# malak29/video-text-detection-system

Hardware: AMD Instinct MI355X
Metric: frames/sec (detect+recognize) @720p, 1/2/4/8 MI355X; box IoU vs CPU ref (higher is better)
Workload: dtype f16

## Files before the change

include/vtd.h:

```cpp
#ifndef VTD_H
#define VTD_H

#include <stddef.h>
#include <stdint.h>

#ifdef __cplusplus
extern "C" {
#endif

typedef struct vtd_detector vtd_detector;
typedef struct vtd_recognizer vtd_recognizer;
typedef struct vtd_postproc vtd_postproc;
typedef void* vtd_stream;

typedef struct vtd_detection {
    int32_t bbox[4];
    int32_t polygon[8];
    float confidence;
    float area;
    int32_t first_x, first_y;
} vtd_detection;

const char* vtd_version(void);
const char* vtd_strerror(int code);
int vtd_device_count(void);

int vtd_detector_create(const char* backbone, int max_batch, vtd_detector** out);
void vtd_detector_destroy(vtd_detector* d);
int vtd_detector_set_tensor(vtd_detector* d, const char* key, const float* host_data, int64_t numel);
int vtd_detector_set_option(vtd_detector* d, const char* name, int value);
int vtd_detector_finalize(vtd_detector* d, vtd_stream stream);
int vtd_detector_preprocess(vtd_detector* d, const uint8_t* frames_dev, int n, int height, int width, vtd_stream stream);
int vtd_detector_set_input_nchw(vtd_detector* d, const float* x_dev, int n, vtd_stream stream);
int vtd_detector_forward(vtd_detector* d, int n, float* prob_dev, float* thresh_dev, vtd_stream stream);
int vtd_detector_read_tap(vtd_detector* d, const char* name, int n, float* host_out, int64_t capacity, vtd_stream stream);
int64_t vtd_detector_macs_per_frame(const vtd_detector* d);
int vtd_detector_set_profiling(vtd_detector* d, int enable);
int vtd_detector_num_ops(const vtd_detector* d);
int vtd_detector_get_profile(vtd_detector* d, int op_index, char* name, int name_cap, double* total_ms, int64_t* calls,
                             double* total_macs, vtd_stream stream);

int vtd_detector_set_tuning(vtd_detector* d, const char* table_text);
int64_t vtd_detector_get_tuning(const vtd_detector* d, char* buf, int64_t capacity);
int vtd_detector_tuning_measured(const vtd_detector* d);

int vtd_postproc_create(int max_batch, int map_h, int map_w, int max_out, vtd_postproc** out);
void vtd_postproc_destroy(vtd_postproc* pp);
int vtd_postproc_run(vtd_postproc* pp, const float* prob_dev, int n, const int32_t* orig_w_host, const int32_t* orig_h_host,
                     float threshold, vtd_detection* out_dev, int32_t* counts_dev, vtd_stream stream);
int vtd_copy_to_pinned_host(const void* src_dev, void* dst_pinned_host, int64_t bytes, vtd_stream stream);

int64_t vtd_dbloss_workspace_bytes(void);
int vtd_dbloss_forward(const float* prob_dev, const float* thresh_dev, const float* prob_target_dev, const float* thresh_target_dev, int64_t numel,
                       float smooth, void* workspace_dev, float* out4_dev, double* sums5_dev, vtd_stream stream);
int vtd_dbloss_backward(const float* prob_dev, const float* thresh_dev, const float* prob_target_dev, const float* thresh_target_dev, int64_t numel,
                        float smooth, const double* sums5_dev, const float* grad_out4_dev, float* grad_prob_dev, float* grad_thresh_dev,
                        vtd_stream stream);
int vtd_binary_counts_accumulate(const float* pred_dev, const float* target_dev, int64_t numel, float threshold, int64_t* counts4_dev,
                                 vtd_stream stream);

typedef struct vtd_dbhead_branch {
    float *conv_w, *conv_b, *bn1_w, *bn1_b, *bn1_mean, *bn1_var, *ct1_w, *ct1_b, *bn2_w, *bn2_b, *bn2_mean, *bn2_var, *ct2_w, *ct2_b;
} vtd_dbhead_branch;
typedef struct vtd_dbhead_params {
    vtd_dbhead_branch branch[2];
} vtd_dbhead_params;
int vtd_detector_forward_features(vtd_detector* d, int n, void* feats_dev, vtd_stream stream);
int vtd_dbhead_pack_features(const void* x_dev, int dtype, int n, int height, int width, void* feats_dev, vtd_stream stream);
int64_t vtd_dbhead_train_workspace_bytes(int n, int height, int width, int backward);
int vtd_dbhead_train_forward(const void* feats_dev, int n, int height, int width, const vtd_dbhead_params* params, int training, float momentum,
                             float eps, void* workspace_dev, float* prob_dev, float* thresh_dev, float* stats_dev, vtd_stream stream);
int vtd_dbhead_train_backward(const void* feats_dev, int n, int height, int width, const vtd_dbhead_params* params, int training,
                              const void* workspace_dev, const float* prob_dev, const float* thresh_dev, const float* grad_prob_dev,
                              const float* grad_thresh_dev, const vtd_dbhead_params* grads, void* scratch_dev, vtd_stream stream);
int vtd_dbhead_train_backward_input(int n, int height, int width, const vtd_dbhead_params* params, void* scratch_dev, float* dfeats_dev,
                                    float* dscale_dev, vtd_stream stream);
int vtd_dbhead_unpack_input_grad(const float* dfeats_dev, const float* dscale_dev, int n, int height, int width, float* grad_nchw_dev,
                                 vtd_stream stream);

typedef struct vtd_fpn_params {
    float *inner_w[4], *inner_b[4];
    float *layer_w, *layer_b;
} vtd_fpn_params;
int vtd_detector_forward_trunk(vtd_detector* d, int n, void* c2_dev, void* c3_dev, void* c4_dev, void* c5_dev, vtd_stream stream);
int vtd_detector_forward_pool(vtd_detector* d, int n, void* pool_dev, vtd_stream stream);
int vtd_fpn_train_pack_tap(const void* x_dev, int dtype, int n, int channels, int height, int width, void* tap_dev, vtd_stream stream);
int64_t vtd_fpn_train_workspace_bytes(int n, int h5, int w5, int c5_channels, int mode);
int vtd_fpn_train_forward(const void* const* taps, int n, int h5, int w5, int c5_channels, const vtd_fpn_params* params, void* workspace_dev,
                          void* p2_dev, vtd_stream stream);
int vtd_fpn_train_unpack_p2(const void* p2_dev, int n, int height, int width, float* p2_nchw_dev, vtd_stream stream);
int vtd_fpn_train_pack_grad(const float* grad_nchw_dev, int n, int height, int width, float* dp2_dev, vtd_stream stream);
int vtd_fpn_train_backward(const void* const* taps, int n, int h5, int w5, int c5_channels, const vtd_fpn_params* params, const void* workspace_dev,
                           const float* dp2_dev, const float* dscale_dev, const vtd_fpn_params* grads, void* scratch_dev, vtd_stream stream);
int64_t vtd_fpn_train_input_workspace_bytes(int n, int h5, int w5, int c5_channels);
int vtd_fpn_train_backward_input(int n, int h5, int w5, int c5_channels, const vtd_fpn_params* params, void* scratch_dev, int level_mask,
                                 float* const* dtaps_dev, float* dscale_dev, vtd_stream stream);
int vtd_fpn_train_unpack_tap_grad(const float* dtap_dev, const float* dscale_dev, int n, int channels, int height, int width, float* grad_nchw_dev,
                                  vtd_stream stream);

typedef struct vtd_basicblock_params {
    float *conv1_w, *bn1_w, *bn1_b, *bn1_mean, *bn1_var;
    float *conv2_w, *bn2_w, *bn2_b, *bn2_mean, *bn2_var;
    float *ds_w, *ds_bn_w, *ds_bn_b, *ds_bn_mean, *ds_bn_var;
} vtd_basicblock_params;
int64_t vtd_basicblock_train_workspace_bytes(int n, int h_in, int w_in, int cin, int width, int stride, int mode);
int vtd_basicblock_train_forward(const void* x_dev, int n, int h_in, int w_in, int cin, int width, int stride, const vtd_basicblock_params* params,
                                 float eps, void* workspace_dev, void* y_dev, vtd_stream stream);
int vtd_basicblock_train_backward(const void* x_dev, int n, int h_in, int w_in, int cin, int width, int stride, const vtd_basicblock_params* params,
                                  float eps, const void* workspace_dev, const void* y_dev, const float* dy_dev, const float* dscale_dev,
                                  const vtd_basicblock_params* grads, void* scratch_dev, float* dx_dev, float* dxscale_dev, vtd_stream stream);

int64_t vtd_resblock_train_workspace_bytes(int n, int h_in, int w_in, int cin, int width, int stride, int mode);
int vtd_resblock_train_forward(const void* x_dev, int n, int h_in, int w_in, int cin, int width, int stride, const vtd_basicblock_params* params,
                               float eps, void* workspace_dev, void* y_dev, vtd_stream stream);
int vtd_resblock_train_backward(const void* x_dev, int n, int h_in, int w_in, int cin, int width, int stride, const vtd_basicblock_params* params,
                                float eps, const void* workspace_dev, const void* y_dev, const float* dy_dev, const float* dscale_dev,
                                const vtd_basicblock_params* grads, void* scratch_dev, float* dx_dev, float* dxscale_dev, vtd_stream stream);
int vtd_resblock_train_combine(float* a_dev, const float* ascale_dev, const float* b_dev, const float* bscale_dev, int64_t numel, float* outscale_dev,
                               vtd_stream stream);

int64_t vtd_block64_train_workspace_bytes(int n, int h_in, int w_in, int cin, int width, int stride, int mode);
int vtd_block64_train_forward(const void* x_dev, int n, int h_in, int w_in, int cin, int width, int stride, const vtd_basicblock_params* params,
                              float eps, void* workspace_dev, void* y_dev, vtd_stream stream);
int vtd_block64_train_backward(const void* x_dev, int n, int h_in, int w_in, int cin, int width, int stride, const vtd_basicblock_params* params,
                               float eps, const void* workspace_dev, const void* y_dev, const float* dy_dev, const float* dscale_dev,
                               const vtd_basicblock_params* grads, void* scratch_dev, float* dx_dev, float* dxscale_dev, vtd_stream stream);

typedef struct vtd_stem_params {
    float *w, *gamma, *beta, *mean, *var;
} vtd_stem_params;
int vtd_stem_train_pack_input(const void* x_dev, int dtype, int n, int height, int width, void* tap_dev, vtd_stream stream);
int64_t vtd_stem_train_workspace_bytes(int n, int height, int width, int mode);
int vtd_stem_train_forward(const void* x_tap_dev, int n, int height, int width, const vtd_stem_params* params, float eps, void* workspace_dev,
                           void* pool_tap_dev, void* idx_dev, vtd_stream stream);
int vtd_stem_train_backward(const void* x_tap_dev, int n, int height, int width, const vtd_stem_params* params, float eps, const void* workspace_dev,
                            const void* pool_tap_dev, const void* idx_dev, const float* dpool_dev, const float* dscale_dev, const vtd_stem_params* grads,
                            void* scratch_dev, vtd_stream stream);

int vtd_recognizer_create(int vocab_size, int max_crops, vtd_recognizer** out);
void vtd_recognizer_destroy(vtd_recognizer* r);
int vtd_recognizer_set_tensor(vtd_recognizer* r, const char* key, const float* host_data, int64_t numel);
int vtd_recognizer_set_option(vtd_recognizer* r, const char* name, int value);
int vtd_recognizer_finalize(vtd_recognizer* r, vtd_stream stream);
int vtd_recognizer_crop_resize(vtd_recognizer* r, const uint8_t* frames_dev, int n_frames, int height, int width,
                               const int32_t* boxes_dev, int ncrops, vtd_stream stream);
int vtd_recognizer_set_input_nchw(vtd_recognizer* r, const float* x_dev, int ncrops, vtd_stream stream);
int vtd_recognizer_forward(vtd_recognizer* r, int ncrops, float* logits_dev, vtd_stream stream);
int vtd_recognizer_read_tap(vtd_recognizer* r, const char* name, int ncrops, float* host_out, int64_t capacity, vtd_stream stream);
int64_t vtd_recognizer_macs_per_crop(const vtd_recognizer* r);
int vtd_recognizer_set_tuning(vtd_recognizer* r, const char* table_text);
int64_t vtd_recognizer_get_tuning(const vtd_recognizer* r, char* buf, int64_t capacity);
int vtd_recognizer_tuning_measured(const vtd_recognizer* r);
int vtd_ctc_greedy_decode(const float* logits_dev, int n, int T, int V, const int32_t* id2char_dev, int blank_id, int apply_softmax,
                          int32_t* out_dev, vtd_stream stream);

typedef struct vtd_trocr vtd_trocr;
typedef struct vtd_trocr_config {
    int32_t image_size, patch_size;
    int32_t enc_hidden, enc_layers, enc_heads, enc_ffn;
    int32_t enc_qkv_bias;
    float enc_ln_eps;
    int32_t dec_hidden, dec_layers, dec_heads, dec_ffn;
    int32_t vocab_size, max_positions;
    float dec_ln_eps;
    int32_t decoder_start_token_id, eos_token_id, pad_token_id;
    int32_t max_length;
} vtd_trocr_config;
int vtd_trocr_create(const vtd_trocr_config* cfg, int max_crops, vtd_trocr** out);
void vtd_trocr_destroy(vtd_trocr* t);
int vtd_trocr_set_option(vtd_trocr* t, const char* name, int value);
int vtd_trocr_get_option(const vtd_trocr* t, const char* name, int* value);
int vtd_trocr_set_tensor(vtd_trocr* t, const char* key, const float* host_data, int64_t numel);
int vtd_trocr_finalize(vtd_trocr* t, vtd_stream stream);
int vtd_trocr_encode_crops(vtd_trocr* t, const uint8_t* frames_dev, int n_frames, int height, int width, const int32_t* boxes_host, int ncrops,
                           vtd_stream stream);
int vtd_trocr_encode_pixels(vtd_trocr* t, const float* pixel_values_dev, int ncrops, vtd_stream stream);
int vtd_trocr_generate(vtd_trocr* t, int ncrops, int max_length, const int32_t* forced_ids_dev, int forced_len, int32_t* ids_dev, float* logits_dev,
                       vtd_stream stream);
int vtd_trocr_num_slots(const vtd_trocr* t);
int vtd_trocr_encode_crops_slot(vtd_trocr* t, int slot, const uint8_t* frames_dev, int n_frames, int height, int width, const int32_t* boxes_host,
                                int ncrops, vtd_stream stream);
int vtd_trocr_encode_pixels_slot(vtd_trocr* t, int slot, const float* pixel_values_dev, int ncrops, vtd_stream stream);
int vtd_trocr_stage_crops_slot(vtd_trocr* t, int slot, const uint8_t* frames_dev, int n_frames, int height, int width, const int32_t* boxes_host,
                               int ncrops, int row_offset, vtd_stream stream);
int vtd_trocr_encode_staged_slot(vtd_trocr* t, int slot, int ncrops, vtd_stream stream);
int vtd_trocr_generate_slot(vtd_trocr* t, int slot, int ncrops, int max_length, const int32_t* forced_ids_dev, int forced_len, int32_t* ids_dev,
                            float* logits_dev, vtd_stream stream);
// ... 17 lines not shown
```

video-text-detection-system_amd/csrc/detector_misc.hip:

```cpp
#include "vtd_common.h"

namespace {

constexpr int PRE_TY = 16;
constexpr int PRE_OUT = 640;
constexpr int PRE_CHUNK = 4;
#ifndef VTD_PRE_NT
#define VTD_PRE_NT 640
#endif
constexpr int PRE_NT = VTD_PRE_NT;
constexpr int PRE_COLS = (PRE_OUT + PRE_NT - 1) / PRE_NT;

struct PreParams {
    const uint8_t* frames;
    half_t* out;
    const int* xb;
    const int* xk;
    const int* yb;
    const int* yk;
    int H, W, ksx, ksy;
    int max_rows;
    unsigned quads_magic;
};

__device__ __forceinline__ uint8_t clip8_22(int v) {
    v >>= 22;
    return (uint8_t)(v < 0 ? 0 : (v > 255 ? 255 : v));
}

__global__ __launch_bounds__(256) void preprocess_kernel(const PreParams p) {
    extern __shared__ __attribute__((aligned(16))) uint8_t rows[];
    const int oy0 = blockIdx.x * PRE_TY;
    const int img = blockIdx.y;
    const int y_first = p.yb[2 * oy0];
    const int oy_last = min(oy0 + PRE_TY, PRE_OUT) - 1;
    const int y_end = p.yb[2 * oy_last] + p.yb[2 * oy_last + 1];
    const int nrows = y_end - y_first;
    const int row_bytes = p.W * 3;
    const int row_pad = (row_bytes + 15) & ~15;
    uint8_t* raw = rows + ((p.max_rows * PRE_OUT * 3 + 15) & ~15);
    const uint8_t* src = p.frames + (int64_t)img * p.H * row_bytes;

    for (int r0 = 0; r0 < nrows; r0 += PRE_CHUNK) {
        const int nr = min(PRE_CHUNK, nrows - r0);
        if ((row_bytes & 15) == 0) {
            const int vec_per_row = row_bytes >> 4;
            for (int i = threadIdx.x; i < nr * vec_per_row; i += 256) {
                const int rr = i / vec_per_row, v = i - rr * vec_per_row;
                *(uint4*)(raw + rr * row_pad + v * 16) = *(const uint4*)(src + (int64_t)(y_first + r0 + rr) * row_bytes + v * 16);
            }
        } else {
            for (int i = threadIdx.x; i < nr * row_bytes; i += 256) {
                const int rr = i / row_bytes, v = i - rr * row_bytes;
                raw[rr * row_pad + v] = src[(int64_t)(y_first + r0 + rr) * row_bytes + v];
            }
        }
        __syncthreads();
        for (int idx = threadIdx.x; idx < nr * PRE_OUT; idx += 256) {
            const int rr = idx / PRE_OUT, ox = idx - rr * PRE_OUT;
            const uint8_t* row = raw + rr * row_pad;
            const int xmin = p.xb[2 * ox], cnt = p.xb[2 * ox + 1];
            const int* k = p.xk + ox * p.ksx;
            int s0 = 1 << 21, s1 = 1 << 21, s2 = 1 << 21;
            for (int t = 0; t < cnt; ++t) {
                const int kv = k[t];
                const uint8_t* px = row + (xmin + t) * 3;
                s0 += px[0] * kv;
                s1 += px[1] * kv;
                s2 += px[2] * kv;
            }
            uint8_t* d = rows + ((r0 + rr) * PRE_OUT + ox) * 3;
            d[0] = clip8_22(s0);
            d[1] = clip8_22(s1);
            d[2] = clip8_22(s2);
        }
        __syncthreads();
    }

    const float mean[3] = {0.485f, 0.456f, 0.406f};
    const float stdv[3] = {0.229f, 0.224f, 0.225f};
    for (int idx = threadIdx.x; idx < PRE_TY * PRE_OUT; idx += 256) {
        const int ty = idx / PRE_OUT, ox = idx - ty * PRE_OUT;
        const int oy = oy0 + ty;
        if (oy >= PRE_OUT) break;
        const int ymin = p.yb[2 * oy] - y_first, cnt = p.yb[2 * oy + 1];
        const int* k = p.yk + oy * p.ksy;
        int s0 = 1 << 21, s1 = 1 << 21, s2 = 1 << 21;
        for (int t = 0; t < cnt; ++t) {
            const int kv = k[t];
            const uint8_t* px = rows + ((ymin + t) * PRE_OUT + ox) * 3;
            s0 += px[0] * kv;
            s1 += px[1] * kv;
            s2 += px[2] * kv;
        }
        const float b = (float)clip8_22(s0), g = (float)clip8_22(s1), r = (float)clip8_22(s2);
        half4 o;
        o[0] = (half_t)((r / 255.0f - mean[0]) / stdv[0]);
        o[1] = (half_t)((g / 255.0f - mean[1]) / stdv[1]);
        o[2] = (half_t)((b / 255.0f - mean[2]) / stdv[2]);
        o[3] = (half_t)0.f;
        *(half4*)(p.out + (((int64_t)img * 646 + oy + 3) * 646 + ox + 3) * 4) = o;
    }
}

template <int KSX, int KSY>
__global__ __launch_bounds__(PRE_NT) void preprocess_fast_kernel(const PreParams p) {
    extern __shared__ __attribute__((aligned(16))) uint8_t lds[];
    uint32_t* const rows = (uint32_t*)lds;
    const int raw_pitch = p.W + KSX;
    uint32_t* const raw = rows + p.max_rows * PRE_OUT;
    int* const ytab = (int*)(raw + PRE_CHUNK * raw_pitch);
    half_t* const lut = (half_t*)(ytab + PRE_TY * (2 + KSY));
    const int oy0 = blockIdx.x * PRE_TY;
    const int img = blockIdx.y;
    const int y_first = p.yb[2 * oy0];
    const int oy_last = min(oy0 + PRE_TY, PRE_OUT) - 1;
    const int y_end = p.yb[2 * oy_last] + p.yb[2 * oy_last + 1];
    const int nrows = y_end - y_first;
    const int row_bytes = p.W * 3;
    const uint8_t* src = p.frames + (int64_t)img * p.H * row_bytes;
    const int tid = threadIdx.x;

    int xmin[PRE_COLS], kx[PRE_COLS][KSX];
#pragma unroll
    for (int s = 0; s < PRE_COLS; ++s) {
        const int ox = min(tid + PRE_NT * s, PRE_OUT - 1);
        xmin[s] = p.xb[2 * ox];
#pragma unroll
        for (int t = 0; t < KSX; ++t) kx[s][t] = p.xk[ox * KSX + t];
    }
    for (int i = tid; i < PRE_TY * (2 + KSY); i += PRE_NT) {
        const int ty = i / (2 + KSY), e = i - ty * (2 + KSY);
        const int oy = min(oy0 + ty, PRE_OUT - 1);
        ytab[i] = e < 2 ? p.yb[2 * oy + e] : p.yk[oy * KSY + (e - 2)];
    }
    for (int i = tid; i < PRE_CHUNK * KSX; i += PRE_NT) raw[(i / KSX) * raw_pitch + p.W + (i % KSX)] = 0u;
    {
        const float mean[3] = {0.485f, 0.456f, 0.406f};
        const float stdv[3] = {0.229f, 0.224f, 0.225f};
        if (tid < 256) {
#pragma unroll
            for (int c = 0; c < 3; ++c) lut[c * 256 + tid] = (half_t)(((float)tid / 255.0f - mean[c]) / stdv[c]);
        }
    }

    const int quads = p.W >> 2;
    constexpr int MAXIT = (PRE_CHUNK * 512 + PRE_NT - 1) / PRE_NT;
    uint32_t stg0[MAXIT][3], stg1[MAXIT][3];
    auto fetch = [&](int r0, uint32_t (&stg)[MAXIT][3]) {
        const int nr = min(PRE_CHUNK, nrows - r0);
#pragma unroll
        for (int it = 0; it < MAXIT; ++it) {
            const int i = tid + it * PRE_NT;
            if (i < nr * quads) {
                const int rr = (int)__umulhi((unsigned)i, p.quads_magic), q = i - rr * quads;
                const uint32_t* g = (const uint32_t*)(src + (int64_t)(y_first + r0 + rr) * row_bytes) + q * 3;
                stg[it][0] = g[0]; stg[it][1] = g[1]; stg[it][2] = g[2];
            }
        }
    };
    auto chunk = [&](int r0, uint32_t (&stg)[MAXIT][3]) {
        const int nr = min(PRE_CHUNK, nrows - r0);
#pragma unroll
        for (int it = 0; it < MAXIT; ++it) {
            const int i = tid + it * PRE_NT;
            if (i < nr * quads) {
                const int rr = (int)__umulhi((unsigned)i, p.quads_magic), q = i - rr * quads;
                const uint32_t d0 = stg[it][0], d1 = stg[it][1], d2 = stg[it][2];
                uint4 px;
                px.x = d0 & 0xffffffu;
                px.y = ((d0 >> 24) | (d1 << 8)) & 0xffffffu;
                px.z = ((d1 >> 16) | (d2 << 16)) & 0xffffffu;
                px.w = d2 >> 8;
                *(uint4*)(raw + rr * raw_pitch + q * 4) = px;
            }
        }
        __syncthreads();
        if (r0 + 2 * PRE_CHUNK < nrows) fetch(r0 + 2 * PRE_CHUNK, stg);
        for (int rr = 0; rr < nr; ++rr) {
            const uint32_t* row = raw + rr * raw_pitch;
#pragma unroll
            for (int s = 0; s < PRE_COLS; ++s) {
                const int ox = tid + PRE_NT * s;
                if (ox < PRE_OUT) {
                    uint32_t s0 = 1u << 21, s1 = 1u << 21, s2 = 1u << 21;
#pragma unroll
                    for (int t = 0; t < KSX; ++t) {
                        const uint32_t px = row[xmin[s] + t];
                        const uint32_t kt = (uint32_t)kx[s][t];
                        s0 = __umul24(px & 0xffu, kt) + s0;
                        s1 = __umul24((px >> 8) & 0xffu, kt) + s1;
                        s2 = __umul24(px >> 16, kt) + s2;
                    }
                    rows[(r0 + rr) * PRE_OUT + ox] = (uint32_t)clip8_22((int)s0) | ((uint32_t)clip8_22((int)s1) << 8) | ((uint32_t)clip8_22((int)s2) << 16);
                }
            }
        }
        __syncthreads();
    };
    fetch(0, stg0);
    if (PRE_CHUNK < nrows) fetch(PRE_CHUNK, stg1);
    for (int r0 = 0; r0 < nrows; r0 += 2 * PRE_CHUNK) {
        chunk(r0, stg0);
        if (r0 + PRE_CHUNK < nrows) chunk(r0 + PRE_CHUNK, stg1);
    }

    for (int idx = tid; idx < PRE_TY * (PRE_OUT / 4); idx += PRE_NT) {
        const int ty = idx / (PRE_OUT / 4), g = idx - ty * (PRE_OUT / 4);
        const int oy = oy0 + ty;
        if (oy >= PRE_OUT) break;
        const int* yt = ytab + ty * (2 + KSY);
        const int ymin = yt[0] - y_first;
        uint32_t acc[4][3];
#pragma unroll
        for (int q = 0; q < 4; ++q)
#pragma unroll
            for (int c = 0; c < 3; ++c) acc[q][c] = 1u << 21;
#pragma unroll
        for (int t = 0; t < KSY; ++t) {
            const uint32_t kv = (uint32_t)yt[2 + t];
            const int r = min(ymin + t, nrows - 1);
            const uint4 px = *(const uint4*)(rows + r * PRE_OUT + g * 4);
            const uint32_t pv[4] = {px.x, px.y, px.z, px.w};
#pragma unroll
            for (int q = 0; q < 4; ++q) {
                acc[q][0] = __umul24(pv[q] & 0xffu, kv) + acc[q][0];
                acc[q][1] = __umul24((pv[q] >> 8) & 0xffu, kv) + acc[q][1];
                acc[q][2] = __umul24(pv[q] >> 16, kv) + acc[q][2];
            }
        }
        half8 o01, o23;
#pragma unroll
        for (int q = 0; q < 4; ++q) {
            const half_t h0 = lut[clip8_22((int)acc[q][2])];
            const half_t h1 = lut[256 + clip8_22((int)acc[q][1])];
            const half_t h2 = lut[512 + clip8_22((int)acc[q][0])];
            if (q < 2) { o01[q * 4] = h0; o01[q * 4 + 1] = h1; o01[q * 4 + 2] = h2; o01[q * 4 + 3] = (half_t)0.f; }
            else { o23[(q - 2) * 4] = h0; o23[(q - 2) * 4 + 1] = h1; o23[(q - 2) * 4 + 2] = h2; o23[(q - 2) * 4 + 3] = (half_t)0.f; }
        }
        half_t* dst = p.out + (((int64_t)img * 646 + oy + 3) * 646 + g * 4 + 3) * 4;
        *(half4*)(dst) = half4{o01[0], o01[1], o01[2], o01[3]};
        *(half4*)(dst + 4) = half4{o01[4], o01[5], o01[6], o01[7]};
        *(half4*)(dst + 8) = half4{o23[0], o23[1], o23[2], o23[3]};
        *(half4*)(dst + 12) = half4{o23[4], o23[5], o23[6], o23[7]};
    }
}

__global__ void nchw_to_input_kernel(const float* __restrict__ x, half_t* __restrict__ out, int n) {
    const int64_t idx = (int64_t)blockIdx.x * blockDim.x + threadIdx.x;
    const int64_t total = (int64_t)n * 640 * 640;
    if (idx >= total) return;
    const int img = (int)(idx / (640 * 640));
    const int rem = (int)(idx - (int64_t)img * 640 * 640);
    const int y = rem / 640, xx = rem - y * 640;
    const float* base = x + (int64_t)img * 3 * 640 * 640 + rem;
    half4 o = {(half_t)base[0], (half_t)base[640 * 640], (half_t)base[2 * 640 * 640], (half_t)0.f};
    *(half4*)(out + (((int64_t)img * 646 + y + 3) * 646 + xx + 3) * 4) = o;
}

struct PoolParams {
    const half_t* in;
    half_t* out;
    int n, c, ho, wo;
    int in_hp, in_wp, in_y0, in_x0;
    int out_hp, out_wp, out_ring;
    int kh, kw, sh, sw;
};

__global__ void maxpool_kernel(const PoolParams p) {
    const int cg = p.c >> 3;
    const int64_t total = (int64_t)p.n * p.ho * p.wo * cg;
    for (int64_t idx = (int64_t)blockIdx.x * blockDim.x + threadIdx.x; idx < total; idx += (int64_t)gridDim.x * blockDim.x) {
        const int g = (int)(idx % cg);
        int64_t t = idx / cg;
        const int ox = (int)(t % p.wo);
        t /= p.wo;
        const int oy = (int)(t % p.ho);
        const int img = (int)(t / p.ho);
        half8 m;
#pragma unroll
        for (int e = 0; e < 8; ++e) m[e] = (half_t)(-65504.f);
        for (int r = 0; r < p.kh; ++r)
            for (int s = 0; s < p.kw; ++s) {
                const half8 v = *(const half8*)(p.in + (((int64_t)img * p.in_hp + oy * p.sh + p.in_y0 + r) * p.in_wp +
                                                         ox * p.sw + p.in_x0 + s) * p.c + g * 8);
#pragma unroll
                for (int e = 0; e < 8; ++e) m[e] = v[e] > m[e] ? v[e] : m[e];
            }
        *(half8*)(p.out + (((int64_t)img * p.out_hp + oy + p.out_ring) * p.out_wp + ox + p.out_ring) * p.c + g * 8) = m;
    }
}

}

int vtd_launch_preprocess(const uint8_t* frames, int n, int H, int W, half_t* out, const int* xb, const int* xk, int ksx,
                          const int* yb, const int* yk, int ksy, int max_rows, hipStream_t stream) {
    PreParams p{frames, out, xb, xk, yb, yk, H, W, ksx, ksy, max_rows, 0u};
    if ((W & 3) == 0 && W <= 2048 && ksy == 5 && (ksx == 5 || ksx == 7)) {
        const int lds_fast = (max_rows * PRE_OUT + PRE_CHUNK * (W + ksx) + PRE_TY * (2 + ksy)) * 4 + 3 * 256 * 2;
        p.quads_magic = (unsigned)(((1ull << 32) + (W / 4) - 1) / (W / 4));
        if (lds_fast <= 160 * 1024) {
            static bool attr5 = false, attr7 = false;
            if (ksx == 5) {
                if (!attr5) {
                    VTD_HIP_CHECK(hipFuncSetAttribute((const void*)preprocess_fast_kernel<5, 5>, hipFuncAttributeMaxDynamicSharedMemorySize, 160 * 1024));
                    attr5 = true;
                }
                hipLaunchKernelGGL((preprocess_fast_kernel<5, 5>), dim3(PRE_OUT / PRE_TY, n), dim3(PRE_NT), lds_fast, stream, p);
            } else {
                if (!attr7) {
                    VTD_HIP_CHECK(hipFuncSetAttribute((const void*)preprocess_fast_kernel<7, 5>, hipFuncAttributeMaxDynamicSharedMemorySize, 160 * 1024));
                    attr7 = true;
                }
                hipLaunchKernelGGL((preprocess_fast_kernel<7, 5>), dim3(PRE_OUT / PRE_TY, n), dim3(PRE_NT), lds_fast, stream, p);
            }
            return -(int)hipGetLastError();
        }
    }
    const int lds = ((max_rows * PRE_OUT * 3 + 15) & ~15) + PRE_CHUNK * ((W * 3 + 15) & ~15);
    if (lds > 160 * 1024) return -1010;
    static bool attr_done = false;
    if (!attr_done) {
        VTD_HIP_CHECK(hipFuncSetAttribute((const void*)preprocess_kernel, hipFuncAttributeMaxDynamicSharedMemorySize, 160 * 1024));
        attr_done = true;
    }
    hipLaunchKernelGGL(preprocess_kernel, dim3(PRE_OUT / PRE_TY, n), dim3(256), lds, stream, p);
    return -(int)hipGetLastError();
}

int vtd_launch_nchw_to_input(const float* x, half_t* out, int n, hipStream_t stream) {
    const int64_t total = (int64_t)n * 640 * 640;
    hipLaunchKernelGGL(nchw_to_input_kernel, dim3((unsigned)((total + 255) / 256)), dim3(256), 0, stream, x, out, n);
    return -(int)hipGetLastError();
}

int vtd_launch_maxpool(const TensorDesc& in, const TensorDesc& out, int n, int kh, int kw, int sh, int sw, int pad_h, int pad_w,
                       hipStream_t stream) {
    if (in.c != out.c || (in.c & 7)) return -1020;
    if (in.ring < pad_h || in.ring < pad_w) return -1021;
    if ((out.h - 1) * sh - pad_h + kh > in.h + (in.hp - in.h - in.ring) || (out.w - 1) * sw - pad_w + kw > in.w + (in.wp - in.w - in.ring))
        return -1022;
    PoolParams p{in.ptr, out.ptr, n, in.c, out.h, out.w, in.hp, in.wp, in.ring - pad_h, in.ring - pad_w,
                 out.hp, out.wp, out.ring, kh, kw, sh, sw};
    const int64_t total = (int64_t)n * out.h * out.w * (in.c >> 3);
    const int blocks = (int)((total + 255) / 256 < 256 * 16 ? (total + 255) / 256 : 256 * 16);
    hipLaunchKernelGGL(maxpool_kernel, dim3(blocks), dim3(256), 0, stream, p);
    return -(int)hipGetLastError();
}
```

video-text-detection-system_amd/csrc/stem_pool.hip:

```cpp
#include <cstdlib>
#include "vtd_common.h"

namespace {

constexpr int SP_PT_ROWS = 7, SP_PT_COLS = 8;
constexpr int SP_CT_COLS = 17;
constexpr int SP_PATCH_COLS = 40;
constexpr int SP_PIECES = 12;
constexpr int SP_PATCH_BYTES = SP_PIECES * 1024;
constexpr int SP_NST = 3;
constexpr int SP_CT_PITCH = 144;
constexpr int SP_LDS = SP_NST * SP_PATCH_BYTES + 256 * SP_CT_PITCH + 256;

struct StemPoolParams {
    const half_t* in;
    const half_t* w;
    const float* bias;
    half_t* out;
    int n, in_hp, in_wp, conv_h, conv_w, pool_h, pool_w, out_hp, out_wp, out_ring;
    int tiles_x, tiles_y, total_tiles;
};

typedef short short4v __attribute__((ext_vector_type(4)));
typedef short short8v __attribute__((ext_vector_type(8)));
__device__ __forceinline__ half8 sp_max(half8 a, half8 b) {
    return __builtin_bit_cast(half8, __builtin_elementwise_max(__builtin_bit_cast(short8v, a), __builtin_bit_cast(short8v, b)));
}

__host__ __device__ constexpr int sp_chan(int tile, int row) { return 32 * (tile >> 1) + 8 * (row >> 2) + 4 * (tile & 1) + (row & 3); }

template <int N>
__device__ __forceinline__ void sp_wait_vmcnt() { asm volatile("s_waitcnt vmcnt(%0)" ::"n"(N) : "memory"); }
__device__ __forceinline__ void sp_lds_barrier() {
    asm volatile("s_waitcnt lgkmcnt(0)" ::: "memory");
    __builtin_amdgcn_s_barrier();
}

__device__ __forceinline__ void sp_tile_coords(const StemPoolParams& p, int tile, int& img, int& py0, int& px0) {
    const int per_img = p.tiles_x * p.tiles_y;
    img = tile / per_img;
    const int r = tile - img * per_img;
    const int ty = r / p.tiles_x;
    py0 = ty * SP_PT_ROWS;
    px0 = (r - ty * p.tiles_x) * SP_PT_COLS;
}

template <int DBG>
__global__ __launch_bounds__(256, 2) void stem_pool_kernel(const StemPoolParams p) {
    extern __shared__ __attribute__((aligned(16))) unsigned char sp_smem[];
    unsigned char* const ring = sp_smem;
    unsigned char* const ctile = sp_smem + SP_NST * SP_PATCH_BYTES;
    float* const bias_lds = (float*)(ctile + 256 * SP_CT_PITCH);
    const int tid = threadIdx.x, lane = tid & 63;
    const int wv = __builtin_amdgcn_readfirstlane(tid >> 6);
    const int fr = lane & 15, fq = lane >> 4;

    int first, stride, last;
    if ((gridDim.x & 7) == 0) {
        const int xcd = blockIdx.x & 7, per = gridDim.x >> 3;
        const int lo = (int)(((int64_t)p.total_tiles * xcd) >> 3);
        last = (int)(((int64_t)p.total_tiles * (xcd + 1)) >> 3);
        first = lo + (blockIdx.x >> 3);
        stride = per;
    } else {
        first = blockIdx.x; stride = gridDim.x; last = p.total_tiles;
    }
    if (first >= last) return;
    const int nt = (last - first + stride - 1) / stride;

    half8 wreg[7][4];
#pragma unroll
    for (int ky = 0; ky < 7; ++ky)
#pragma unroll
        for (int i = 0; i < 4; ++i) wreg[ky][i] = *(const half8*)(p.w + ((ky * 4 + i) * 64 + lane) * 8);
    if (tid < 64) bias_lds[tid] = p.bias[tid];
    int a_off[4];
#pragma unroll
    for (int j = 0; j < 4; ++j) {
        const int pix = wv * 64 + j * 16 + fr;
        const int c_row = pix / SP_CT_COLS, c_col = pix - c_row * SP_CT_COLS;
        a_off[j] = ((2 * c_row) * SP_PATCH_COLS + 2 * c_col + 2 * fq) * 8;
    }
    int u_row[3], u_col[3];
#pragma unroll
    for (int k = 0; k < 3; ++k) {
        int u = (wv + 4 * k) * 64 + lane;
        u = u < 700 ? u : 699;
        u_row[k] = u / 20;
        u_col[k] = 2 * (u - u_row[k] * 20);
    }
    auto issue = [&](int tile, int stage) {
        if constexpr (DBG == 4) return;
        int img, py0, px0;
        sp_tile_coords(p, __builtin_amdgcn_readfirstlane(tile), img, py0, px0);
        const half_t* base = p.in + (int64_t)img * p.in_hp * p.in_wp * 4;
#pragma unroll
        for (int k = 0; k < 3; ++k) {
            int iy = 4 * py0 - 2 + u_row[k], ix = 4 * px0 - 2 + u_col[k];
            iy = iy < 0 ? 0 : iy > p.in_hp - 1 ? p.in_hp - 1 : iy;
            ix = ix < 0 ? 0 : ix > p.in_wp - 2 ? p.in_wp - 2 : ix;
            __builtin_amdgcn_global_load_lds((const VTD_AS1 void*)(base + (iy * p.in_wp + ix) * 4),
                                             (VTD_AS3 void*)(ring + stage * SP_PATCH_BYTES + (wv + 4 * k) * 1024), 16, 0, 0);
        }
    };

    if constexpr (DBG == 7 || DBG == 8) {
        if (((blockIdx.x >> 3) & 32) != 0) { __builtin_amdgcn_s_sleep(60); }
    }
    issue(first, 0);
    if (nt > 1) { issue(first + stride, 1); sp_wait_vmcnt<3>(); } else sp_wait_vmcnt<0>();
    sp_lds_barrier();

    int st = 0;
    for (int k = 0; k < nt; ++k) {
        const int tile = first + k * stride;
        int img, py0, px0;
        sp_tile_coords(p, __builtin_amdgcn_readfirstlane(tile), img, py0, px0);
        if (k + 2 < nt) issue(tile + 2 * stride, st == 0 ? SP_NST - 1 : st - 1);

        floatx4 acc[4][4];
#pragma unroll
        for (int i = 0; i < 4; ++i)
#pragma unroll
            for (int j = 0; j < 4; ++j) acc[i][j] = *(const floatx4*)(bias_lds + sp_chan(i, fq * 4));
        const unsigned char* pb = ring + st * SP_PATCH_BYTES;
        half8 af[2][4];
#pragma unroll
        for (int j = 0; j < 4; ++j) af[0][j] = *(const half8*)(pb + a_off[j]);
        if constexpr (DBG == 6 || DBG == 7) __builtin_amdgcn_s_setprio(3);
#pragma unroll
        for (int ky = 0; ky < 7; ++ky) {
            if (ky < 6) {
#pragma unroll
                for (int j = 0; j < 4; ++j) af[(ky + 1) & 1][j] = *(const half8*)(pb + a_off[j] + (ky + 1) * (SP_PATCH_COLS * 8));
            }
            if (DBG == 3 && ky > 0) { for (int j = 0; j < 4; ++j) asm volatile("" ::"v"(af[ky & 1][j])); continue; }
#pragma unroll
            for (int j = 0; j < 4; ++j)
#pragma unroll
                for (int i = 0; i < 4; ++i) acc[i][j] = __builtin_amdgcn_mfma_f32_16x16x32_f16(wreg[ky][i], af[ky & 1][j], acc[i][j], 0, 0, 0);
            if (ky < 6) __builtin_amdgcn_sched_group_barrier(0x100, 4, 0);
            __builtin_amdgcn_sched_group_barrier(0x008, 16, 0);
            __builtin_amdgcn_sched_barrier(0);
        }

        if constexpr (DBG == 6 || DBG == 7) __builtin_amdgcn_s_setprio(0);
        if constexpr (DBG == 2) {
            float t = 0.f;
            for (int i = 0; i < 4; ++i) for (int j = 0; j < 4; ++j) t += acc[i][j][0] + acc[i][j][1] + acc[i][j][2] + acc[i][j][3];
            if (t == 123.456f) p.out[0] = (half_t)t;
            if (k + 2 < nt) sp_wait_vmcnt<3>(); else sp_wait_vmcnt<0>();
            sp_lds_barrier();
            st = st + 1 == SP_NST ? 0 : st + 1;
            continue;
        }
#pragma unroll
        for (int j = 0; j < 4; ++j) {
            const int pix = wv * 64 + j * 16 + fr;
            const int c_row = pix / SP_CT_COLS, c_col = pix - c_row * SP_CT_COLS;
            const int cy = 2 * py0 - 1 + c_row, cx = 2 * px0 - 1 + c_col;
            const bool valid = cy >= 0 && cy < p.conv_h && cx >= 0 && cx < p.conv_w;
            unsigned char* dst = ctile + pix * SP_CT_PITCH + fq * 16;
#pragma unroll
            for (int k = 0; k < 2; ++k) {
                typedef float float2v __attribute__((ext_vector_type(2)));
                typedef _Float16 half2v __attribute__((ext_vector_type(2)));
                const floatx4 a = acc[2 * k][j], b = acc[2 * k + 1][j];
                const half2v h0 = __builtin_convertvector((float2v{a[0], a[1]}), half2v);
                const half2v h1 = __builtin_convertvector((float2v{a[2], a[3]}), half2v);
                const half2v h2 = __builtin_convertvector((float2v{b[0], b[1]}), half2v);
                const half2v h3 = __builtin_convertvector((float2v{b[2], b[3]}), half2v);
                half8 hv = half8{h0[0], h0[1], h1[0], h1[1], h2[0], h2[1], h3[0], h3[1]};
                hv = __builtin_bit_cast(half8, __builtin_elementwise_max(__builtin_bit_cast(short8v, hv), short8v{0, 0, 0, 0, 0, 0, 0, 0}));
                if (!valid) hv = half8{0, 0, 0, 0, 0, 0, 0, 0};
                *(half8*)(dst + k * 64) = hv;
            }
        }
        sp_lds_barrier();

        if constexpr (DBG != 1) {
            const int cg = (lane >> 2) & 7;
            const int qx = ((lane >> 5) & 1) | ((lane & 3) << 1);
            const bool two = wv < 3;
            const unsigned char* src0 = ctile + ((2 * wv) * SP_CT_COLS + 2 * qx) * SP_CT_PITCH + cg * 16;
            const int px = px0 + qx;
#pragma unroll
            for (int it = 0; it < 2; ++it) {
                if (it == 1 && !two) break;
                const unsigned char* src = src0 + it * (8 * SP_CT_COLS * SP_CT_PITCH);
                half8 v[9];
#pragma unroll
                for (int r = 0; r < 3; ++r)
#pragma unroll
                    for (int c = 0; c < 3; ++c) v[r * 3 + c] = *(const half8*)(src + (r * SP_CT_COLS + c) * SP_CT_PITCH);
                __builtin_amdgcn_sched_group_barrier(0x100, 9, 0);
                half8 m = sp_max(v[0], v[1]);
#pragma unroll
                for (int q = 2; q < 9; ++q) m = sp_max(m, v[q]);
                const int py = py0 + wv + 4 * it;
                if (DBG == 5) asm volatile("" ::"v"(m));
                else if (py < p.pool_h && px < p.pool_w)
                    *(half8*)(p.out + (((int64_t)img * p.out_hp + py + p.out_ring) * p.out_wp + px + p.out_ring) * 64 + cg * 8) = m;
            }
        }
        if (k + 2 < nt) sp_wait_vmcnt<3>(); else sp_wait_vmcnt<0>();
        sp_lds_barrier();
        st = st + 1 == SP_NST ? 0 : st + 1;
    }
}

}

void vtd_stem_pool_pack_weights(const float* w_folded , half_t* packed ) {
    for (int ky = 0; ky < 7; ++ky)
        for (int i = 0; i < 4; ++i)
            for (int lane = 0; lane < 64; ++lane) {
                const int fr = lane & 15, fq = lane >> 4, co = sp_chan(i, fr);
                for (int e = 0; e < 8; ++e) {
                    const int kx = 2 * fq + (e >> 2), c = e & 3;
                    float v = 0.f;
                    if (kx < 7 && c < 3) v = w_folded[((co * 3 + c) * 7 + ky) * 7 + kx];
                    packed[((ky * 4 + i) * 64 + lane) * 8 + e] = (half_t)v;
                }
            }
}

int vtd_launch_stem_pool(const TensorDesc& in, const TensorDesc& out, const half_t* w_packed, const float* bias, int n,
                         hipStream_t stream) {
    if (in.c != 4 || in.ring != 3 || out.c != 64 || (in.h & 3) || (in.w & 3) || out.h != in.h / 4 || out.w != in.w / 4 ||
        in.hp != in.h + 6 || in.wp != in.w + 6 || (in.wp & 1) || n <= 0 || n > in.n || n > out.n)
        return -2001;
    if (out.w % SP_PT_COLS) return -2002;
    StemPoolParams p;
    p.in = in.ptr; p.w = w_packed; p.bias = bias; p.out = out.ptr;
    p.n = n; p.in_hp = in.hp; p.in_wp = in.wp; p.conv_h = in.h / 2; p.conv_w = in.w / 2; p.pool_h = out.h; p.pool_w = out.w;
    p.out_hp = out.hp; p.out_wp = out.wp; p.out_ring = out.ring;
    p.tiles_x = out.w / SP_PT_COLS;
    p.tiles_y = (out.h + SP_PT_ROWS - 1) / SP_PT_ROWS;
    p.total_tiles = n * p.tiles_x * p.tiles_y;
    const int grid = p.total_tiles < 512 ? p.total_tiles : 512;
    void (*kern)(const StemPoolParams) = stem_pool_kernel<0>;
#ifdef VTD_STEM_EXPERIMENT
    if (const char* e = getenv("VTD_STEM_DEBUG")) {
        switch (atoi(e)) {
            case 1: kern = stem_pool_kernel<1>; break;
            case 2: kern = stem_pool_kernel<2>; break;
            case 3: kern = stem_pool_kernel<3>; break;
            case 4: kern = stem_pool_kernel<4>; break;
            case 5: kern = stem_pool_kernel<5>; break;
            case 6: kern = stem_pool_kernel<6>; break;
            case 7: kern = stem_pool_kernel<7>; break;
            case 8: kern = stem_pool_kernel<8>; break;
            default: break;
        }
    }
    {
        hipError_t ea = hipFuncSetAttribute((const void*)kern, hipFuncAttributeMaxDynamicSharedMemorySize, SP_LDS);
        if (ea != hipSuccess) return -(int)ea;
    }
#else
    static bool attr_set = false;
    if (!attr_set) {
        hipError_t ea = hipFuncSetAttribute((const void*)kern, hipFuncAttributeMaxDynamicSharedMemorySize, SP_LDS);
        if (ea != hipSuccess) return -(int)ea;
        attr_set = true;
    }
#endif
    hipLaunchKernelGGL(kern, dim3(grid), dim3(256), SP_LDS, stream, p);
    hipError_t e = hipGetLastError();
    return e == hipSuccess ? 0 : -(int)e;
}
```

video-text-detection-system_amd/csrc/vtd_api.cpp:

```cpp
#include <algorithm>
#include <cmath>
#include <cstdio>
#include <cstdlib>
#include <cstring>
#include <map>
#include <memory>
#include <string>
#include <vector>

#include "../../include/vtd.h"
#include "vtd_common.h"

int vtd_launch_conv(const ConvParams& p, int cfg, hipStream_t stream);
int vtd_conv_num_configs();
bool vtd_conv_config_valid(const ConvParams& p, int cfg);
int vtd_launch_preprocess(const uint8_t* frames, int n, int H, int W, half_t* out, const int* xb, const int* xk, int ksx,
                          const int* yb, const int* yk, int ksy, int max_rows, hipStream_t stream);
int vtd_launch_nchw_to_input(const float* x, half_t* out, int n, hipStream_t stream);
int vtd_launch_maxpool(const TensorDesc& in, const TensorDesc& out, int n, int kh, int kw, int sh, int sw, int pad_h, int pad_w,
                       hipStream_t stream);
void vtd_stem_pool_pack_weights(const float* w_folded, half_t* packed);
int vtd_launch_stem_pool(const TensorDesc& in, const TensorDesc& out, const half_t* w_packed, const float* bias, int n, hipStream_t stream);
extern "C" int vtd_head_entry_halo_steps(int py, int px, int nch1, int* out);
int vtd_launch_head_entry_halo(const ConvParams& c, const int* steps_dev, int nsteps, int big_tiles, hipStream_t stream);
#ifdef VTD_EXPERIMENTAL_CANDIDATES
extern "C" int vtd_head_entry_half_schedule(const int* steps, int nsteps, int* out);
int vtd_launch_head_entry_half(const ConvParams& c, const int* sched_dev, int nsteps, hipStream_t stream);
int vtd_head_entry_pair_tables(int py, int px, int c2ch, int* half_steps, int* plan);
int vtd_launch_head_entry_pair(const ConvParams& c, const int* half_steps_dev, const int* plan_dev, int nh, hipStream_t stream);
#endif
bool vtd_conv_halo_supported(const ConvParams& c, int* bn_out, int* tw_out);
bool vtd_conv_halo_c64_supported(const ConvParams& c, int tw);
int vtd_launch_conv_halo(const ConvParams& c, int bn, int tw, hipStream_t stream);
bool vtd_pointwise128_supported(const ConvParams& c);
int vtd_launch_pointwise128(const ConvParams& c, hipStream_t stream);
void vtd_head_tail_pack_w1(const half_t* w1_gemm, half_t* packed);
void vtd_head_tail_pack_w2(const float* w2, half_t* packed);
int vtd_launch_head_tail(const TensorDesc& in, const half_t* w1, const float* bias1, const half_t* w2, float b2, float* out, int n,
                         hipStream_t stream);

int vtd_launch_crop_resize(const uint8_t* frames, int H, int W, const int32_t* boxes, int ncrops, uint8_t* out, hipStream_t s);
int vtd_launch_crnn_conv1(const uint8_t* in_u8, const float* in_f32, const half_t* w, const float* bias, half_t* out, int n, hipStream_t s);
int vtd_launch_lstm(const half_t* xs, const half_t* whh, half_t* hout, int D, int T, hipStream_t s);
int vtd_launch_ctc_greedy(const float* logits, int n, int T, int V, int ld, const int32_t* id2char, int blank, int apply_softmax,
                          int32_t* out, hipStream_t s);
int vtd_launch_compact_rows(const float* in, float* out, int64_t rows, int V, int ld, hipStream_t s);
int vtd_dbloss_ws_bytes();
int vtd_launch_dbloss(const float* prob, const float* thresh, const float* prob_t, const float* thresh_t, int64_t n, float smooth, double* workspace,
                      float* out4, double* sums5, hipStream_t stream);
int vtd_launch_dbloss_backward(const float* prob, const float* thresh, const float* prob_t, const float* thresh_t, int64_t n, float smooth,
                               const double* sums5, const float* grad_out4, float* grad_prob, float* grad_thresh, hipStream_t stream);
int vtd_launch_binary_counts(const float* pred, const float* target, int64_t n, float threshold, int64_t* counts4, hipStream_t stream);
int64_t vtd_dbhead_ws_bytes(int n, int H, int W, int backward);
int vtd_launch_dbhead_pack(const void* x, int dtype, int n, int H, int W, void* feats, hipStream_t s);
int vtd_launch_dbhead_forward(const void* feats, int n, int H, int W, const vtd_dbhead_params* params, int training, float momentum, float eps,
                              void* ws, float* prob, float* thresh, float* stats_out, hipStream_t s);
int vtd_launch_dbhead_backward_input(int n, int H, int W, const vtd_dbhead_params* params, void* scratch, float* dfeats, float* dscale, hipStream_t s);
int vtd_launch_dbhead_unpack_input_grad(const float* dfeats, const float* dscale, int n, int H, int W, float* out, hipStream_t s);
int64_t vtd_fpn_ws_bytes(int n, int h5, int w5, int c5, int mode);
int vtd_launch_fpn_pack_tap(const void* x, int dtype, int n, int channels, int H, int W, void* out, hipStream_t s);
int vtd_launch_fpn_unpack_p2(const void* p2, int n, int H, int W, float* out, hipStream_t s);
int vtd_launch_fpn_pack_grad(const float* g, int n, int H, int W, float* out, hipStream_t s);
int vtd_launch_fpn_forward(const void* const* taps, int n, int h5, int w5, int c5, const vtd_fpn_params* params, void* ws, void* p2_out, hipStream_t s);
int vtd_launch_fpn_backward(const void* const* taps, int n, int h5, int w5, int c5, const vtd_fpn_params* params, const void* ws, const float* dp2,
                            const float* dscale, const vtd_fpn_params* grads, void* scratch, hipStream_t s);
int64_t vtd_fpn_input_ws_bytes(int n, int h5, int w5, int c5);
int vtd_launch_fpn_backward_input(int n, int h5, int w5, int c5, const vtd_fpn_params* params, void* scratch, int mask, float* const* dtaps,
                                  float* dscale, hipStream_t s);
int64_t vtd_basicblock_ws_bytes(int n, int hin, int win, int cin, int width, int stride, int mode);
int vtd_launch_basicblock_forward(const void* x, int n, int hin, int win, int cin, int width, int stride, const vtd_basicblock_params* P, float eps,
                                  void* ws, void* y, hipStream_t s);
int vtd_launch_basicblock_backward(const void* x, int n, int hin, int win, int cin, int width, int stride, const vtd_basicblock_params* P, float eps,
                                   const void* ws, const void* y, const float* dy, const float* dscale, const vtd_basicblock_params* Gp, void* scratch,
                                   float* dx, float* dxscale, hipStream_t s);
int64_t vtd_resblock_ws_bytes(int n, int hin, int win, int cin, int width, int stride, int mode);
int64_t vtd_block64_ws_bytes(int n, int hin, int win, int cin, int width, int stride, int mode);
int vtd_launch_block64_forward(const void* x, int n, int hin, int win, int cin, int width, int stride, const vtd_basicblock_params* P, float eps, void* ws,
                               void* y, hipStream_t s);
int vtd_launch_block64_backward(const void* x, int n, int hin, int win, int cin, int width, int stride, const vtd_basicblock_params* P, float eps,
                                const void* ws, const void* y, const float* dy, const float* dscale, const vtd_basicblock_params* Gp, void* scratch,
                                float* dx, float* dxscale, hipStream_t s);
int vtd_launch_resblock_combine(float* a, const float* asc, const float* b, const float* bsc, int64_t numel, float* osc, hipStream_t s);
int vtd_launch_stem_pack_input(const void* x, int dtype, int n, int H, int W, void* tap, hipStream_t s);
int64_t vtd_stem_ws_bytes(int n, int H, int W, int mode);
int vtd_launch_stem_forward(const void* x, int n, int H, int W, const vtd_stem_params* P, float eps, void* ws, void* pool, void* idx, hipStream_t s);
int vtd_launch_stem_backward(const void* x, int n, int H, int W, const vtd_stem_params* P, float eps, const void* ws, const void* pool, const void* idx,
                             const float* dpool, const float* dscale, const vtd_stem_params* Gp, void* scratch, hipStream_t s);
int vtd_launch_resblock_forward(const void* x, int n, int hin, int win, int cin, int width, int stride, const vtd_basicblock_params* P, float eps, void* ws,
                                void* y, hipStream_t s);
int vtd_launch_resblock_backward(const void* x, int n, int hin, int win, int cin, int width, int stride, const vtd_basicblock_params* P, float eps,
                                 const void* ws, const void* y, const float* dy, const float* dscale, const vtd_basicblock_params* Gp, void* scratch,
                                 float* dx, float* dxscale, hipStream_t s);
int vtd_launch_fpn_unpack_tap_grad(const float* g, const float* sc, int n, int channels, int H, int W, float* out, hipStream_t s);
int vtd_launch_dbhead_backward(const void* feats, int n, int H, int W, const vtd_dbhead_params* params, int training, const void* ws,
                               const float* prob, const float* thresh, const float* gprob, const float* gthresh, const vtd_dbhead_params* grads,
                               void* scratch, hipStream_t s);

namespace vtd {

enum : int {
    ERR_ARG = -1100,
    ERR_UNKNOWN_KEY = -1101,
    ERR_SHAPE = -1102,
    ERR_MISSING_KEY = -1103,
    ERR_NOT_FINALIZED = -1104,
    ERR_BATCH = -1105,
    ERR_GEOMETRY = -1106,
    ERR_CAPACITY = -1107,
};

using StateDict = std::map<std::string, std::vector<float>>;

struct DeviceArena {
    std::vector<void*> blocks;
    size_t total = 0;
    int alloc(void** out, size_t bytes, bool zero) {
        void* p = nullptr;
        bytes = (bytes + 255) & ~size_t(255);
        hipError_t e = hipMalloc(&p, bytes);
        if (e != hipSuccess) return -(int)e;
        if (zero) {
            e = hipMemset(p, 0, bytes);
            if (e != hipSuccess) return -(int)e;
        }
        blocks.push_back(p);
        total += bytes;
        *out = p;
        return 0;
    }
    ~DeviceArena() {
        for (void* p : blocks) (void)hipFree(p);
    }
};

static TensorDesc make_desc(int n, int h, int w, int c, int ring, int ring_br) {
    TensorDesc t;
    t.ptr = nullptr;
    t.n = n; t.h = h; t.w = w; t.c = c; t.ring = ring;
    t.hp = h + ring + ring_br;
    t.wp = w + ring + ring_br;
    return t;
}

struct ConvOp {
    TensorDesc in, out, res;
    bool has_res = false;
    half_t* w = nullptr;
    half_t* w_panel = nullptr;
    float* bias = nullptr;
    int k_hi_step = 32, cin_steps = 1, kw = 1, s_step = 0, r_step = 0;
    int K = 0, cout = 0, cout_pad = 0, stride = 1, in_y0 = 0, in_x0 = 0, flags = 0, ps_cout = 0, res_shift = 0;
    int ho = 0, wo = 0;
    int64_t macs_per_image = 0;
    void* out_f32 = nullptr;
    int ldc = 0;
    int seg_cols = 0;
    void* seg_out[3] = {nullptr, nullptr, nullptr};
    int seg_ldc[3] = {0, 0, 0};
    const float* head_w = nullptr;
    float head_b = 0.f;
    const uint32_t* plist = nullptr;
    const int* tile_combo = nullptr;
    const uint32_t* plist_b = nullptr;
    const int* tile_combo_border = nullptr;
    int tiles_border = 0;
    const int* he_steps = nullptr;
    int he_nsteps = 0;
    const int* hh_sched = nullptr;
    const int* hp_half_steps = nullptr;
    const int* hp_plan = nullptr;
    int hp_nh = 0;
    const int* tile_combo_b = nullptr;
    int tiles_per_img_b = 0;
    int tiles_per_img = 0, seg1_steps = 0, cin_steps2 = 0, kw2 = 0, s_step2 = 0, r_step2 = 0, img_h = 0, img_w = 0;
    TensorDesc in2;
    const float* bias_tab = nullptr;
    bool dual = false;
    int in2_mul = 1, in2_shr = 0;
    int pool_pw = 0;
};

struct Op {
    enum Kind { CONV, POOL, FINAL, STEMPOOL, HEADTAIL, BORDER } kind;
    ConvOp conv;
    TensorDesc pin, pout;
    int pk[6] = {0, 0, 0, 0, 0, 0};
    const float* fw = nullptr;
    float fbias = 0.f;
    int final_slot = 0;
    const half_t* spw = nullptr;
    const float* spb = nullptr;
    const half_t* htw1 = nullptr;
    const half_t* htw2 = nullptr;
};

static void fill_conv_params(const ConvOp& c, int n, ConvParams& p) {
    std::memset(&p, 0, sizeof(p));
    p.in = c.in.ptr; p.wgt = c.w; p.k_hi_step = c.k_hi_step; p.cin_steps = c.cin_steps; p.kw = c.kw; p.s_step = c.s_step; p.r_step = c.r_step; p.bias = c.bias;
    p.res = c.has_res ? c.res.ptr : nullptr;
    p.out = (c.flags & (EPI_OUT_F32 | EPI_OUT_F16)) ? c.out_f32 : (void*)c.out.ptr;
    p.M = n * c.ho * c.wo; p.K = c.K; p.cout = c.cout; p.cout_pad = c.cout_pad;
    p.ho = c.ho; p.wo = c.wo;
    p.in_hp = c.in.hp; p.in_wp = c.in.wp; p.in_c = c.in.c; p.in_y0 = c.in_y0; p.in_x0 = c.in_x0; p.stride = c.stride;
    p.out_hp = c.out.hp; p.out_wp = c.out.wp; p.out_c = c.out.c; p.out_ring = c.out.ring;
    p.res_hp = c.res.hp; p.res_wp = c.res.wp; p.res_ring = c.res.ring; p.res_shift = c.res_shift;
    p.ps_cout = c.ps_cout; p.flags = c.flags; p.ldc = c.ldc;
    p.seg_cols = c.seg_cols;
    for (int i = 0; i < 3; ++i) { p.seg_out[i] = c.seg_out[i]; p.seg_ldc[i] = c.seg_ldc[i]; }
    p.head_w = c.head_w; p.head_b = c.head_b; p.prob_out = (float*)c.out_f32;
    if (c.plist) {
        p.plist = c.plist; p.tile_combo = c.tile_combo; p.tiles_per_img = c.tiles_per_img;
        p.plist_b = c.plist_b; p.tile_combo_b = c.tile_combo_b; p.tiles_per_img_b = c.tiles_per_img_b;
        p.in2 = c.in2.ptr; p.in2_hp = c.in2.hp; p.in2_wp = c.in2.wp; p.in2_c = c.in2.c; p.in2_ring = c.in2.ring;
        p.seg1_steps = c.seg1_steps; p.cin_steps2 = c.cin_steps2; p.kw2 = c.kw2; p.s_step2 = c.s_step2; p.r_step2 = c.r_step2;
        p.bias_tab = c.bias_tab; p.img_h = c.img_h; p.img_w = c.img_w;
        p.M = n * c.tiles_per_img * 128;
    }
    p.pool_pw = c.pool_pw;
    if (c.dual) {
        p.in2 = c.in2.ptr; p.in2_hp = c.in2.hp; p.in2_wp = c.in2.wp; p.in2_c = c.in2.c; p.in2_ring = c.in2.ring;
        p.in2_mul = c.in2_mul; p.in2_shr = c.in2_shr;
        p.seg1_steps = c.seg1_steps; p.cin_steps2 = c.cin_steps2; p.kw2 = 1; p.s_step2 = 0; p.r_step2 = 0;
    }
}

static const int kHaloCfg = 100;
static const int kHaloC64Cfg = 101;
static const int kHalo64Cfg = 104;
static const int kHeadEntryHalo256Cfg = 103;
static const int kHeadEntryPairCfg = 105;
static const int kPointwiseCfg = 106;
static const int kHeadEntryHalfCfg = 107;
static const int kHeadEntryHaloCfg = 102;
static bool halo_enabled() {
    const char* e = std::getenv("VTD_HALO_CONV");
    return !(e && e[0] == '0');
}

static int pick_tile_height(const ConvParams& p, int table_cfg) {
    if (const char* e = std::getenv("VTD_TILE_HEIGHT_MODEL"); e && e[0] == '0') return table_cfg;
    if (std::getenv("VTD_FORCE_CONV_CFG")) return table_cfg;
    static const struct { int cfg, bm, bn; double eff; } family[5] = {{0, 256, 128, 1.0}, {14, 256, 128, 1.04}, {13, 272, 128, 0.92}, {12, 208, 128, 0.80},
                                                                      {15, 256, 256, 1.07}};
    auto cost_of = [&](int cfg) -> double {
        for (const auto& k : family)
            if (k.cfg == cfg) {
                if (!vtd_conv_config_valid(p, k.cfg)) return 0.0;
                const int64_t tiles = (int64_t)((p.M + k.bm - 1) / k.bm) * (p.cout_pad / k.bn);
                return (double)((tiles + 255) / 256) * k.bm * k.bn / k.eff;
            }
        return 0.0;
    };
    int best = table_cfg;
    double best_cost = cost_of(table_cfg);
    if (best_cost == 0.0) return table_cfg;
    const double keep = best_cost * 0.94;
    double other_cost = keep;
    for (const auto& k : family) {
        if (k.cfg == table_cfg) continue;
        const double c = cost_of(k.cfg);
        if (c > 0.0 && c < other_cost) { other_cost = c; best = k.cfg; }
// ... 32 lines not shown
    return vtd_launch_conv(p, cfg, s);
}

static int launch_border_tiles(const ConvOp& c, int n, hipStream_t s) {
    if (!c.tile_combo_border || c.tiles_border <= 0) return ERR_GEOMETRY;
    ConvParams pb;
    fill_conv_params(c, n, pb);
    pb.tile_combo = c.tile_combo_border; pb.tiles_per_img = c.tiles_border; pb.M = n * c.tiles_border * 128;
    pb.plist_b = nullptr; pb.tile_combo_b = nullptr; pb.tiles_per_img_b = 0;
    return vtd_launch_conv(pb, 9, s);
}

static int autotune_conv(const ConvOp& c, int n, hipStream_t s, int* best_cfg) {
    ConvParams p;
    fill_conv_params(c, n, p);
    hipEvent_t e0, e1;
    VTD_HIP_CHECK(hipEventCreate(&e0));
    VTD_HIP_CHECK(hipEventCreate(&e1));
    float best = 1e30f;
    int best_id = -1, rc = 0;
    if (p.plist) {
        const char* fc = std::getenv("VTD_FORCE_CLASSED_CFG");
        if (fc && (vtd_conv_config_valid(p, std::atoi(fc)) || ((std::atoi(fc) == kHeadEntryHaloCfg || std::atoi(fc) == kHeadEntryHalo256Cfg) && c.he_steps) ||
                   (std::atoi(fc) == kHeadEntryHalfCfg && c.hh_sched) ||
                   (std::atoi(fc) == kHeadEntryPairCfg && c.hp_half_steps))) {
            (void)hipEventDestroy(e0);
            (void)hipEventDestroy(e1);
            *best_cfg = std::atoi(fc);
            return 0;
        }
    }
    for (int cfg = 0; cfg < vtd_conv_num_configs() && !rc; ++cfg) {
        if (!vtd_conv_config_valid(p, cfg)) continue;
        if ((rc = vtd_launch_conv(p, cfg, s))) break;
        (void)hipEventRecord(e0, s);
        for (int rep = 0; rep < 3 && !rc; ++rep) rc = vtd_launch_conv(p, cfg, s);
        (void)hipEventRecord(e1, s);
        if (hipEventSynchronize(e1) != hipSuccess) { rc = ERR_ARG; break; }
        float ms = 0.f;
        (void)hipEventElapsedTime(&ms, e0, e1);
        if (ms < best) { best = ms; best_id = cfg; }
    }
    if (!rc && p.plist && c.he_steps && halo_enabled()) {
        const float best_gathered = best;
        for (int variant = 0; variant < 4 && !rc; ++variant) {
            if (variant == 2 && !c.hp_half_steps) continue;
            if (variant == 3 && !c.hh_sched) continue;
            const int vcfg = variant == 3 ? kHeadEntryHalfCfg : variant == 2 ? kHeadEntryPairCfg : variant ? kHeadEntryHalo256Cfg : kHeadEntryHaloCfg;
            auto both = [&]() { int r = launch_conv_op(c, n, s, vcfg); return r ? r : launch_border_tiles(c, n, s); };
            if ((rc = both())) break;
            float ms = 1e30f;
            for (int round = 0; round < 2 && !rc; ++round) {
                (void)hipEventRecord(e0, s);
                for (int rep = 0; rep < 4 && !rc; ++rep) rc = both();
                (void)hipEventRecord(e1, s);
                if (hipEventSynchronize(e1) != hipSuccess) rc = ERR_ARG;
                float t = 0.f;
                (void)hipEventElapsedTime(&t, e0, e1);
                ms = t * 0.75f < ms ? t * 0.75f : ms;
            }
            if (const char* v = std::getenv("VTD_AUTOTUNE_VERBOSE"); v && v[0] == '1')
                std::fprintf(stderr, "[autotune] head entry variant %d: %.1f us per launch incl. border tiles (best so far %.1f, cfg %d)\n", vcfg,
                             ms / 3.f * 1e3f, best / 3.f * 1e3f, best_id);
            (void)best_gathered;
            if (!rc && ms < best) { best = ms; best_id = vcfg; }
        }
    }
    if (!rc && vtd_pointwise128_supported(p)) {
        if (!(rc = vtd_launch_pointwise128(p, s))) {
            (void)hipEventRecord(e0, s);
            for (int rep = 0; rep < 3 && !rc; ++rep) rc = vtd_launch_pointwise128(p, s);
            (void)hipEventRecord(e1, s);
            if (hipEventSynchronize(e1) != hipSuccess) rc = ERR_ARG;
            float ms = 0.f;
            (void)hipEventElapsedTime(&ms, e0, e1);
            if (!rc && ms < best) { best = ms; best_id = kPointwiseCfg; }
        }
    }
    int hbn = 0, htw = 0;
    if (!rc && halo_enabled() && vtd_conv_halo_supported(p, &hbn, &htw)) {
        const char* force = std::getenv("VTD_FORCE_HALO");
        if (force && (force[0] == '1' || force[0] == '2' || force[0] == '3')) best = 1e30f;
        bool pinned = false;
        for (int variant = 0; variant < 3 && !rc; ++variant) {
            if (variant == 1 && !vtd_conv_halo_c64_supported(p, htw)) continue;
            const int bn = variant == 1 ? 1 : variant == 2 ? 2 : hbn;
            if ((rc = vtd_launch_conv_halo(p, bn, htw, s))) break;
            (void)hipEventRecord(e0, s);
            for (int rep = 0; rep < 3 && !rc; ++rep) rc = vtd_launch_conv_halo(p, bn, htw, s);
            (void)hipEventRecord(e1, s);
            if (hipEventSynchronize(e1) != hipSuccess) rc = ERR_ARG;
            float ms = 0.f;
            (void)hipEventElapsedTime(&ms, e0, e1);
            const int vid = variant == 1 ? kHaloC64Cfg : variant == 2 ? kHalo64Cfg : kHaloCfg;
            const bool pin = (variant == 1 && force && force[0] == '2') || (variant == 2 && force && force[0] == '3');
            if (!rc && !pinned && (ms < best || pin)) { best = ms; best_id = vid; pinned = pin; }
        }
    }
    (void)hipEventDestroy(e0);
    (void)hipEventDestroy(e1);
    *best_cfg = best_id;
    if (const char* v = std::getenv("VTD_AUTOTUNE_VERBOSE"); v && v[0] == '1')
        std::fprintf(stderr, "[autotune] M=%d N=%d K=%d%s -> cfg %d (%.1f us per launch)\n", p.M, p.cout, p.K, p.plist ? " classed" : "", best_id,
                     best / 3.f * 1e3f);
    return rc;
}

static bool autotune_enabled() {
    const char* e = std::getenv("VTD_AUTOTUNE");
    return !(e && e[0] == '0');
}

struct ResampleAxis {
    int ksize = 0;
    std::vector<int> bounds, kk;
};
static ResampleAxis pillow_axis(int in_size, int out_size) {
    ResampleAxis a;
    const double scale = (double)in_size / out_size;
    const double fscale = scale < 1.0 ? 1.0 : scale;
    const double support = fscale;
    a.ksize = (int)std::ceil(support) * 2 + 1;
    a.bounds.assign(2 * (size_t)out_size, 0);
    a.kk.assign((size_t)out_size * a.ksize, 0);
    std::vector<double> pre(a.ksize);
    for (int xx = 0; xx < out_size; ++xx) {
        const double center = (xx + 0.5) * scale, ss = 1.0 / fscale;
        int xmin = (int)(center - support + 0.5);
        if (xmin < 0) xmin = 0;
        int xmax = (int)(center + support + 0.5);
        if (xmax > in_size) xmax = in_size;
        xmax -= xmin;
        double ww = 0.0;
        for (int x = 0; x < xmax; ++x) {
            double t = (x + xmin - center + 0.5) * ss;
            if (t < 0) t = -t;
            const double wv = t < 1.0 ? 1.0 - t : 0.0;
            pre[x] = wv;
            ww += wv;
        }
        for (int x = 0; x < xmax; ++x) {
            const double v = ww != 0.0 ? pre[x] / ww : pre[x];
            a.kk[(size_t)xx * a.ksize + x] = v < 0 ? (int)(-0.5 + v * (1 << 22)) : (int)(0.5 + v * (1 << 22));
        }
        a.bounds[2 * xx] = xmin;
        a.bounds[2 * xx + 1] = xmax;
    }
    return a;
}

struct PreTables {
    int *xb = nullptr, *xk = nullptr, *yb = nullptr, *yk = nullptr;
    int ksx = 0, ksy = 0, max_rows = 0;
};

}

using namespace vtd;

namespace vtd {
struct ModelBase {
    StateDict sd;
    DeviceArena arena;
    std::map<std::string, int> tuning;
    bool tuning_measured = false;
    int alloc_tensor(TensorDesc& t) {
        void* p = nullptr;
        int rc = arena.alloc(&p, (size_t)tensor_elems(t) * sizeof(half_t), true);
        t.ptr = (half_t*)p;
        return rc;
    }
    const std::vector<float>* get(const std::string& k, size_t numel) const {
        auto it = sd.find(k);
        if (it == sd.end() || it->second.size() != numel) return nullptr;
        return &it->second;
    }
};

static std::string conv_signature(const ConvOp& c) {
    char buf[192];
    int len = std::snprintf(buf, sizeof buf, "conv|in%dx%dx%d|out%dx%d|co%d|K%d|s%d|f%x|r%d|c%d", c.in.h, c.in.w, c.in.c, c.ho, c.wo, c.cout, c.K,
                            c.stride, (unsigned)c.flags, c.has_res ? 1 + c.res_shift : 0, c.plist ? 1 : 0);
    if (c.dual) len += std::snprintf(buf + len, sizeof buf - len, "|x%dm%ds%d", c.in2.c, c.in2_mul, c.in2_shr);
    if (c.pool_pw) std::snprintf(buf + len, sizeof buf - len, "|p2x%d", c.pool_pw);
    return buf;
}

static bool config_valid_for(const ConvOp& c, int n, int cfg) {
    ConvParams p;
    fill_conv_params(c, n, p);
    if (cfg == kHeadEntryPairCfg) return p.plist && c.hp_half_steps && c.tile_combo_border;
    if (cfg == kHeadEntryHalfCfg) return p.plist && c.hh_sched && c.tile_combo_border;
    if (cfg == kHeadEntryHaloCfg || cfg == kHeadEntryHalo256Cfg) return p.plist && c.he_steps && c.tile_combo_border;
    if (cfg == kHaloCfg || cfg == kHaloC64Cfg || cfg == kHalo64Cfg) {
        int bn = 0, tw = 0;
        if (!vtd_conv_halo_supported(p, &bn, &tw)) return false;
        return cfg != kHaloC64Cfg || vtd_conv_halo_c64_supported(p, tw);
    }
    if (cfg == kPointwiseCfg) return vtd_pointwise128_supported(p);
    return cfg >= 0 && cfg < vtd_conv_num_configs() && vtd_conv_config_valid(p, cfg);
}

static int choose_config(ModelBase* m, const ConvOp& c, int n, hipStream_t s, int* cfg) {
    const std::string key = conv_signature(c) + "|n" + std::to_string(n);
    auto it = m->tuning.find(key);
    const bool forced = std::getenv("VTD_FORCE_CLASSED_CFG") || std::getenv("VTD_FORCE_HALO");
    if (const char* fc = std::getenv("VTD_FORCE_CONV_CFG"); fc && !c.plist && config_valid_for(c, n, std::atoi(fc))) {
        *cfg = std::atoi(fc);
        return 0;
    }
    if (const char* fp = std::getenv("VTD_FORCE_POINTWISE"); fp && fp[0] == '1' && config_valid_for(c, n, kPointwiseCfg)) {
        *cfg = kPointwiseCfg;
        return 0;
    }
    if (!forced && it != m->tuning.end() && config_valid_for(c, n, it->second)) {
        *cfg = it->second;
        return 0;
    }
    *cfg = -1;
    if (!autotune_enabled()) return 0;
    int rc = autotune_conv(c, n, s, cfg);
    if (!rc && *cfg >= 0) {
        m->tuning[key] = *cfg;
        m->tuning_measured = true;
    }
    return rc;
}

static int set_tuning_text(ModelBase* m, const char* text) {
    if (!m || !text) return ERR_ARG;
    const char* p = text;
    while (*p) {
        const char* eol = std::strchr(p, '\n');
        std::string line = eol ? std::string(p, eol) : std::string(p);
        p = eol ? eol + 1 : p + line.size();
        if (line.empty() || line[0] == '#') continue;
        const size_t sp = line.find_last_of(" \t");
        if (sp == std::string::npos || sp + 1 >= line.size()) return ERR_ARG;
        char* end = nullptr;
        const long v = std::strtol(line.c_str() + sp + 1, &end, 10);
        if (!end || *end != 0) return ERR_ARG;
        size_t ke = sp;
        while (ke > 0 && (line[ke - 1] == ' ' || line[ke - 1] == '\t')) --ke;
        m->tuning[line.substr(0, ke)] = (int)v;
    }
    return 0;
}

static int64_t get_tuning_text(const ModelBase* m, char* buf, int64_t cap) {
    if (!m) return ERR_ARG;
    std::string out;
    for (const auto& kv : m->tuning) out += kv.first + " " + std::to_string(kv.second) + "\n";
    if (buf && cap > 0) {
        const size_t ncopy = std::min((size_t)cap - 1, out.size());
        std::memcpy(buf, out.data(), ncopy);
        buf[ncopy] = 0;
    }
    return (int64_t)out.size() + 1;
}

static int batch_bucket(int n, int cap) {
    int b = 1;
    while (b < n) b <<= 1;
    return std::min(b, cap);
}

}

struct vtd_detector : vtd::ModelBase {
    std::string backbone;
    int max_batch = 0;
    bool finalized = false;
    std::vector<Op> ops;
    TensorDesc input;
    std::map<std::string, TensorDesc> taps;
    std::map<std::pair<int, int>, PreTables> pre;
    int64_t macs = 0;
    float* final_out[2] = {nullptr, nullptr};
    std::map<int, std::vector<int>> tuned;
    bool head_tail_kernel = true;
    bool fuse_stem_pool = true;
    bool fuse_fpn_head = true;
    bool fuse_downsample = true;
    size_t pool_ops = 0;
    size_t trunk_ops = 0;
    size_t p2_ops = 0;
    bool profiling = false;
    int prof_only = -1;
    std::vector<hipEvent_t> ev_pool;
    size_t ev_used = 0;
    std::vector<std::pair<int, std::pair<hipEvent_t, hipEvent_t>>> ev_spans;
    std::vector<double> prof_ms;
    std::vector<int64_t> prof_calls;
    std::vector<double> prof_macs;
    hipEvent_t take_event() {
        if (ev_used == ev_pool.size()) {
            hipEvent_t e;
            if (hipEventCreate(&e) != hipSuccess) return nullptr;
            ev_pool.push_back(e);
        }
        return ev_pool[ev_used++];
    }
    ~vtd_detector() {
        for (hipEvent_t e : ev_pool) (void)hipEventDestroy(e);
    }
};


struct vtd_recognizer : vtd::ModelBase {
    int vocab = 0, max_crops = 0;
    bool finalized = false;
    bool fuse_pools = true;
    uint8_t* resized = nullptr;
    half_t* w1 = nullptr;
    float* b1 = nullptr;
    TensorDesc t1;
    std::vector<Op> ops;
    TensorDesc t7, h0, h1;
    ConvOp xs_gemm[2], cls_gemm;
    half_t* whh[2] = {nullptr, nullptr};
    half_t* xs = nullptr;
    float* logits_pad = nullptr;
    std::map<std::string, TensorDesc> taps;
    int64_t macs = 0;
    std::map<int, std::vector<int>> tuned;
};

namespace vtd {

struct Fold {
    std::vector<double> scale, shift;
};

static inline half_t half_of(double v) {
    volatile float f = (float)v;
    return (half_t)f;
}

static int fold_bn(const ModelBase* d, const std::string& bn, const std::string& bias_key, int cout, Fold& f) {
    f.scale.assign(cout, 1.0);
    f.shift.assign(cout, 0.0);
    const std::vector<float>* b = nullptr;
    if (!bias_key.empty()) {
        b = d->get(bias_key, cout);
        if (!b) return ERR_MISSING_KEY;
    }
    if (!bn.empty()) {
        auto g = d->get(bn + ".weight", cout), be = d->get(bn + ".bias", cout), mu = d->get(bn + ".running_mean", cout),
             var = d->get(bn + ".running_var", cout);
        if (!g || !be || !mu || !var) return ERR_MISSING_KEY;
        for (int c = 0; c < cout; ++c) {
            const double s = (double)(*g)[c] / std::sqrt((double)(*var)[c] + 1e-5);
            f.scale[c] = s;
            f.shift[c] = (double)(*be)[c] + ((b ? (double)(*b)[c] : 0.0) - (double)(*mu)[c]) * s;
        }
    } else if (b) {
        for (int c = 0; c < cout; ++c) f.shift[c] = (*b)[c];
    }
    return 0;
}

static int upload(DeviceArena& arena, const void* host, size_t bytes, void** dev) {
    int rc = arena.alloc(dev, bytes, false);
    if (rc) return rc;
    hipError_t e = hipMemcpy(*dev, host, bytes, hipMemcpyHostToDevice);
    return e == hipSuccess ? 0 : -(int)e;
}

struct HostConv {
    std::vector<half_t> w;
    std::vector<float> bias;
    int K = 0, cout_pad = 0;
    bool host_only = false;
};

static int build_conv(ModelBase* d, ConvOp& op, const TensorDesc& in, TensorDesc& out, const std::string& wkey,
                      const Fold& f, int cin, int cout, int kh, int kw, int stride, int pad, int flags, HostConv* keep = nullptr) {
    auto w = d->get(wkey, (size_t)cout * cin * kh * kw);
    if (!w) return ERR_MISSING_KEY;
    if (in.c != cin || (cin & 63) || in.ring < pad) return ERR_GEOMETRY;
    const int ho = (in.h + 2 * pad - kh) / stride + 1, wo = (in.w + 2 * pad - kw) / stride + 1;
    if (out.h != ho || out.w != wo || out.c != cout) return ERR_GEOMETRY;
    const int K = kh * kw * cin;
    const int cout_pad = (cout + 63) / 64 * 64;
    std::vector<half_t> wp((size_t)cout_pad * K, (half_t)0.f);
    for (int co = 0; co < cout; ++co)
        for (int c = 0; c < cin; ++c)
            for (int r = 0; r < kh; ++r)
                for (int s = 0; s < kw; ++s)
                    wp[(size_t)co * K + (size_t)(r * kw + s) * cin + c] =
                        half_of((double)(*w)[(((size_t)co * cin + c) * kh + r) * kw + s] * f.scale[co]);
    std::vector<float> bias(cout_pad, 0.f);
    for (int co = 0; co < cout; ++co) bias[co] = (float)f.shift[co];
    op.cin_steps = cin / 64; op.kw = kw; op.s_step = in.c; op.r_step = in.wp * in.c; op.k_hi_step = 32;
    int rc;
    if (!keep || !keep->host_only) {
        if ((rc = upload(d->arena, wp.data(), wp.size() * sizeof(half_t), (void**)&op.w))) return rc;
        if ((rc = upload(d->arena, bias.data(), bias.size() * sizeof(float), (void**)&op.bias))) return rc;
    }
    if (keep) { keep->w = wp; keep->bias = bias; keep->K = K; keep->cout_pad = cout_pad; }
    op.in = in; op.out = out; op.K = K; op.cout = cout; op.cout_pad = cout_pad; op.stride = stride;
    op.in_y0 = in.ring - pad; op.in_x0 = in.ring - pad; op.flags = flags; op.ho = ho; op.wo = wo;
    op.macs_per_image = (int64_t)ho * wo * cout * K;
    if ((ho - 1) * stride + op.in_y0 + kh - 1 >= in.hp || (wo - 1) * stride + op.in_x0 + kw - 1 >= in.wp) return ERR_GEOMETRY;
    return 0;
}

static int attach_second_segment(ModelBase* d, ConvOp& op, const HostConv& first, const ConvOp& sec_op, const HostConv& second,
                                 int mul, int shr) {
    if (first.cout_pad != second.cout_pad || first.K != op.K || second.K != sec_op.K || sec_op.kw != 1 || sec_op.K != sec_op.cin_steps * 64 ||
        sec_op.cout != op.cout || sec_op.ho != op.ho || sec_op.wo != op.wo || (first.K & 63) || (second.K & 63))
        return ERR_GEOMETRY;
    if (((op.ho - 1) * mul >> shr) >= sec_op.in.h || ((op.wo - 1) * mul >> shr) >= sec_op.in.w) return ERR_GEOMETRY;
    const int K = first.K + second.K;
    std::vector<half_t> wp((size_t)first.cout_pad * K);
    std::vector<float> bias(first.cout_pad);
    for (int co = 0; co < first.cout_pad; ++co) {
        std::memcpy(&wp[(size_t)co * K], &first.w[(size_t)co * first.K], (size_t)first.K * sizeof(half_t));
        std::memcpy(&wp[(size_t)co * K + first.K], &second.w[(size_t)co * second.K], (size_t)second.K * sizeof(half_t));
        bias[co] = (float)((double)first.bias[co] + (double)second.bias[co]);
    }
    int rc;
    if ((rc = upload(d->arena, wp.data(), wp.size() * sizeof(half_t), (void**)&op.w))) return rc;
    if ((rc = upload(d->arena, bias.data(), bias.size() * sizeof(float), (void**)&op.bias))) return rc;
    op.dual = true;
    op.in2 = sec_op.in; op.in2_mul = mul; op.in2_shr = shr;
    op.seg1_steps = first.K / 64; op.cin_steps2 = second.K / 64;
    op.K = K;
    op.macs_per_image += sec_op.macs_per_image;
    return 0;
}

static int build_stem(ModelBase* d, ConvOp& op, const TensorDesc& in, TensorDesc& out, const std::string& wkey, const Fold& f) {
    auto w = d->get(wkey, (size_t)64 * 3 * 7 * 7);
    if (!w) return ERR_MISSING_KEY;
// ... 436 lines not shown
                push_conv(c3);
            }
            x = y;
            cin = cout;
        }
        tapsC[st] = x;
        d->taps["c" + std::to_string(st + 2)] = x;
    }
    d->trunk_ops = d->ops.size();

    TensorDesc last;
    for (int i = 0; i < (fuse ? 3 : 4); ++i) {
        const TensorDesc& feat = tapsC[3 - i];
        TensorDesc lat;
        if ((rc = new_tensor(feat.h, feat.w, 256, lat))) return rc;
        Fold f;
        const std::string k = "fpn.inner_blocks." + std::to_string(i);
        if ((rc = fold_bn(d, "", k + ".bias", 256, f))) return rc;
        ConvOp c;
        if ((rc = build_conv(d, c, feat, lat, k + ".weight", f, feat.c, 256, 1, 1, 1, 0, i ? EPI_RESIDUAL : 0))) return rc;
        if (i) { c.has_res = true; c.res = last; c.res_shift = 1; }
        push_conv(c);
        last = lat;
    }
    TensorDesc p2;
    if (!fuse) {
        if ((rc = new_tensor(160, 160, 256, p2))) return rc;
        Fold f;
        if ((rc = fold_bn(d, "", "fpn.layer_blocks.3.bias", 256, f))) return rc;
        ConvOp c;
        if ((rc = build_conv(d, c, last, p2, "fpn.layer_blocks.3.weight", f, 256, 256, 3, 3, 1, 1, 0))) return rc;
        push_conv(c);
        d->taps["p2"] = p2;
        d->p2_ops = d->ops.size();
    } else if (!d->get("fpn.inner_blocks.3.weight", (size_t)256 * tapsC[0].c) || !d->get("fpn.layer_blocks.3.weight", (size_t)256 * 256 * 9)) {
        return ERR_MISSING_KEY;
    }
    for (int i = 0; i < 3; ++i) {
        const std::string k = "fpn.layer_blocks." + std::to_string(i);
        if (!d->get(k + ".weight", (size_t)256 * 256 * 9) || !d->get(k + ".bias", 256)) return ERR_MISSING_KEY;
    }

    const char* branch[2] = {"head.probability_head.", "head.threshold_head."};
    for (int br = 0; br < 2; ++br) {
        const std::string hp = branch[br];
        TensorDesc h1;
        if ((rc = new_tensor(160, 160, 64, h1))) return rc;
        Fold f1, f2;
        ConvOp c1;
        if (fuse) {
            if ((rc = build_classed_head_entry(d, c1, tapsC[0], last, h1, hp))) return rc;
        } else {
            if ((rc = fold_bn(d, hp + "1", hp + "0.bias", 64, f1))) return rc;
            if ((rc = build_conv(d, c1, p2, h1, hp + "0.weight", f1, 256, 64, 3, 3, 1, 1, EPI_RELU))) return rc;
        }
        if ((rc = fold_bn(d, hp + "4", hp + "3.bias", 64, f2))) return rc;
        ConvOp c2;
        TensorDesc h2 = make_desc(B, 320, 320, 64, 1, 1);
        std::vector<half_t> w1_host;
        if ((rc = build_convt(d, c2, h1, h2, hp + "3.weight", f2, 64, 64, EPI_RELU, &w1_host))) return rc;
        auto w6 = d->get(hp + "6.weight", 64 * 4), b6 = d->get(hp + "6.bias", 1);
        if (!w6 || !b6) return ERR_MISSING_KEY;
        std::vector<float> wf(4 * 64);
        for (int blk = 0; blk < 4; ++blk)
            for (int ci = 0; ci < 64; ++ci) wf[blk * 64 + ci] = (*w6)[ci * 4 + blk];
        float* wdev = nullptr;
        if ((rc = upload(d->arena, wf.data(), wf.size() * sizeof(float), (void**)&wdev))) return rc;
        c2.flags = EPI_HEAD_FINAL;
        c2.head_w = wdev;
        c2.head_b = (*b6)[0];
        Op o1, o2;
        o1.kind = Op::CONV; o1.conv = c1; o1.final_slot = br;
        o2.kind = Op::FINAL; o2.conv = c2; o2.final_slot = br;
        if (d->head_tail_kernel) {
            std::vector<half_t> p1((size_t)4 * 4 * 2 * 64 * 8), p2((size_t)2 * 64 * 8);
            vtd_head_tail_pack_w1(w1_host.data(), p1.data());
            vtd_head_tail_pack_w2(wf.data(), p2.data());
            if ((rc = upload(d->arena, p1.data(), p1.size() * sizeof(half_t), (void**)&o2.htw1))) return rc;
            if ((rc = upload(d->arena, p2.data(), p2.size() * sizeof(half_t), (void**)&o2.htw2))) return rc;
            o2.kind = Op::HEADTAIL;
        }
        d->ops.push_back(o1);
        if (fuse) {
            Op ob;
            ob.kind = Op::BORDER; ob.conv = c1; ob.final_slot = br;
            ob.conv.macs_per_image = (int64_t)c1.tiles_border * 128 * 64 * c1.K;
            d->ops.push_back(ob);
        }
        d->ops.push_back(o2);
        if (br == 0) {
            const int64_t px = (int64_t)160 * 160;
            const int64_t ref_entry = fuse ? px * 256 * tapsC[0].c + px * 256 * 2304 + px * 64 * 2304 : c1.macs_per_image;
            d->macs += ref_entry + c2.macs_per_image + (int64_t)320 * 320 * 4 * 64;
            d->taps["head1"] = h1;
        }
    }
    return 0;
}

static int read_tensor_nchw(const TensorDesc& t, int n, int creal, float* host_out, hipStream_t stream) {
    hipError_t e = hipStreamSynchronize(stream);
    if (e != hipSuccess) return -(int)e;
    std::vector<half_t> tmp((size_t)n * t.hp * t.wp * t.c);
    e = hipMemcpy(tmp.data(), t.ptr, tmp.size() * sizeof(half_t), hipMemcpyDeviceToHost);
    if (e != hipSuccess) return -(int)e;
    for (int img = 0; img < n; ++img)
        for (int c = 0; c < creal; ++c)
            for (int y = 0; y < t.h; ++y)
                for (int x = 0; x < t.w; ++x)
                    host_out[(((size_t)img * creal + c) * t.h + y) * t.w + x] =
                        (float)tmp[(((size_t)img * t.hp + y + t.ring) * t.wp + x + t.ring) * t.c + c];
    return 0;
}

static int build_linear(ModelBase* d, ConvOp& op, const TensorDesc& in, const std::vector<float>& W, const std::vector<float>& bias,
                        int N, int K, void* out_f32, int ldc, int out_flag = EPI_OUT_F32) {
    if (in.c != K || (K & 63) || (int)W.size() != N * K || (int)bias.size() != N || (ldc & 3) || ldc < N) return ERR_GEOMETRY;
    const int cout_pad = (N + 63) / 64 * 64;
    std::vector<half_t> wp((size_t)cout_pad * K, (half_t)0.f);
    for (size_t i = 0; i < (size_t)N * K; ++i) wp[i] = (half_t)W[i];
    std::vector<float> b(cout_pad, 0.f);
    for (int i = 0; i < N; ++i) b[i] = bias[i];
    op.cin_steps = K / 64; op.kw = 1; op.s_step = 0; op.r_step = 0; op.k_hi_step = 32;
    int rc;
    if ((rc = upload(d->arena, wp.data(), wp.size() * sizeof(half_t), (void**)&op.w))) return rc;
    if ((rc = upload(d->arena, b.data(), b.size() * sizeof(float), (void**)&op.bias))) return rc;
    op.in = in; op.out = in; op.K = K; op.cout = N; op.cout_pad = cout_pad; op.stride = 1;
    op.in_y0 = in.ring; op.in_x0 = in.ring; op.flags = out_flag; op.ho = in.h; op.wo = in.w;
    op.out_f32 = out_f32; op.ldc = ldc;
    op.macs_per_image = (int64_t)in.h * in.w * N * K;
    return 0;
}

static bool known_detector_key(const std::string& k) {
    return k.rfind("backbone.", 0) == 0 || k.rfind("fpn.", 0) == 0 || k.rfind("head.", 0) == 0;
}

static int get_pre_tables(vtd_detector* d, int H, int W, PreTables& out) {
    auto key = std::make_pair(H, W);
    auto it = d->pre.find(key);
    if (it != d->pre.end()) {
        out = it->second;
        return 0;
    }
    ResampleAxis ax = pillow_axis(W, 640), ay = pillow_axis(H, 640);
    PreTables t;
    t.ksx = ax.ksize; t.ksy = ay.ksize;
    int max_rows = 0;
    for (int oy0 = 0; oy0 < 640; oy0 += 16) {
        const int last = std::min(oy0 + 16, 640) - 1;
        max_rows = std::max(max_rows, ay.bounds[2 * last] + ay.bounds[2 * last + 1] - ay.bounds[2 * oy0]);
    }
    t.max_rows = max_rows;
    int rc;
    if ((rc = upload(d->arena, ax.bounds.data(), ax.bounds.size() * sizeof(int), (void**)&t.xb))) return rc;
    if ((rc = upload(d->arena, ax.kk.data(), ax.kk.size() * sizeof(int), (void**)&t.xk))) return rc;
    if ((rc = upload(d->arena, ay.bounds.data(), ay.bounds.size() * sizeof(int), (void**)&t.yb))) return rc;
    if ((rc = upload(d->arena, ay.kk.data(), ay.kk.size() * sizeof(int), (void**)&t.yk))) return rc;
    d->pre[key] = t;
    out = t;
    return 0;
}

}

extern "C" {

const char* vtd_version(void) {
#ifdef VTD_EXPERIMENTAL_CANDIDATES
    return "vtd_hip 0.3 (gfx950) +experimental";
#else
    return "vtd_hip 0.3 (gfx950)";
#endif
}

const char* vtd_strerror(int code) {
    static thread_local char buf[128];
    switch (code) {
        case 0: return "ok";
        case ERR_ARG: return "invalid argument";
        case ERR_UNKNOWN_KEY: return "unknown state-dict key";
        case ERR_SHAPE: return "tensor has the wrong number of elements";
        case ERR_MISSING_KEY: return "state dict incomplete (missing or mis-sized key)";
        case ERR_NOT_FINALIZED: return "handle not finalized";
        case ERR_BATCH: return "batch exceeds the handle's max_batch";
        case ERR_GEOMETRY: return "layer geometry check failed";
        case ERR_CAPACITY: return "output capacity too small";
        case -2801: return "feature export needs a detector finalized with fuse_fpn_head=0 (the fused head entry never forms P2)";
        case -2802: return "DB head training: invalid argument or shape";
        case -2803: return "DB head training: misaligned buffer";
        case -2901: return "trunk export needs a detector finalized with fuse_fpn_head=0 (the fused graph pads C2 for the composed head entry)";
        case -2902: return "FPN training: invalid argument or shape";
        case -2903: return "FPN training: misaligned buffer";
        case -3001: return "BasicBlock training: invalid argument or unsupported geometry (built: 256 -> 512 stride 2 with even extents, 512 -> 512 stride 1)";
        case -3002: return "BasicBlock training: misaligned buffer";
        case -3003: return "BasicBlock training: the input gradient of the stride-2 block is not built (it needs a strided dgrad)";
        case -3101: return "ResNet block training: invalid argument or unsupported geometry (built: 128 -> 256 and 256 -> 512 stride 2 with even "
                           "extents, 256 -> 256 and 512 -> 512 stride 1)";
        case -3102: return "ResNet block training: misaligned buffer";
        case -3201: return "64-wide block training: invalid argument or unsupported geometry (built: 64 -> 64 stride 1, ResNet-18's layer1)";
        case -3202: return "64-wide block training: misaligned buffer";
        case -3301: return "stem training: invalid argument or unsupported geometry (built: n >= 1, even image height and width >= 2)";
        case -3302: return "stem training: misaligned buffer";
        default: break;
    }
    if (code <= -1000) {
        std::snprintf(buf, sizeof(buf), "vtd validation error %d", code);
        return buf;
    }
    if (code < 0) return hipGetErrorString((hipError_t)(-code));
    return "unknown";
}

int64_t vtd_dbloss_workspace_bytes(void) { return vtd_dbloss_ws_bytes(); }

int vtd_dbloss_forward(const float* prob_dev, const float* thresh_dev, const float* prob_target_dev, const float* thresh_target_dev, int64_t numel,
                       float smooth, void* workspace_dev, float* out4_dev, double* sums5_dev, vtd_stream stream) {
    if (!prob_dev || !prob_target_dev || !workspace_dev || !out4_dev || numel <= 0) return ERR_ARG;
    if ((thresh_dev == nullptr) != (thresh_target_dev == nullptr)) return ERR_ARG;
    return vtd_launch_dbloss(prob_dev, thresh_dev, prob_target_dev, thresh_target_dev, numel, smooth, (double*)workspace_dev, out4_dev, sums5_dev,
                             (hipStream_t)stream);
}

int vtd_dbloss_backward(const float* prob_dev, const float* thresh_dev, const float* prob_target_dev, const float* thresh_target_dev, int64_t numel,
                        float smooth, const double* sums5_dev, const float* grad_out4_dev, float* grad_prob_dev, float* grad_thresh_dev,
                        vtd_stream stream) {
    return vtd_launch_dbloss_backward(prob_dev, thresh_dev, prob_target_dev, thresh_target_dev, numel, smooth, sums5_dev, grad_out4_dev,
                                      grad_prob_dev, grad_thresh_dev, (hipStream_t)stream);
}

int vtd_binary_counts_accumulate(const float* pred_dev, const float* target_dev, int64_t numel, float threshold, int64_t* counts4_dev,
                                 vtd_stream stream) {
    return vtd_launch_binary_counts(pred_dev, target_dev, numel, threshold, counts4_dev, (hipStream_t)stream);
}

int vtd_dbhead_pack_features(const void* x_dev, int dtype, int n, int height, int width, void* feats_dev, vtd_stream stream) {
    return vtd_launch_dbhead_pack(x_dev, dtype, n, height, width, feats_dev, (hipStream_t)stream);
}

int64_t vtd_dbhead_train_workspace_bytes(int n, int height, int width, int backward) { return vtd_dbhead_ws_bytes(n, height, width, backward); }

int vtd_dbhead_train_forward(const void* feats_dev, int n, int height, int width, const vtd_dbhead_params* params, int training, float momentum,
                             float eps, void* workspace_dev, float* prob_dev, float* thresh_dev, float* stats_dev, vtd_stream stream) {
    return vtd_launch_dbhead_forward(feats_dev, n, height, width, params, training, momentum, eps, workspace_dev, prob_dev, thresh_dev, stats_dev,
                                     (hipStream_t)stream);
}

int vtd_dbhead_train_backward(const void* feats_dev, int n, int height, int width, const vtd_dbhead_params* params, int training,
                              const void* workspace_dev, const float* prob_dev, const float* thresh_dev, const float* grad_prob_dev,
                              const float* grad_thresh_dev, const vtd_dbhead_params* grads, void* scratch_dev, vtd_stream stream) {
    return vtd_launch_dbhead_backward(feats_dev, n, height, width, params, training, workspace_dev, prob_dev, thresh_dev, grad_prob_dev,
                                      grad_thresh_dev, grads, scratch_dev, (hipStream_t)stream);
}

int vtd_dbhead_train_backward_input(int n, int height, int width, const vtd_dbhead_params* params, void* scratch_dev, float* dfeats_dev,
                                    float* dscale_dev, vtd_stream stream) {
    return vtd_launch_dbhead_backward_input(n, height, width, params, scratch_dev, dfeats_dev, dscale_dev, (hipStream_t)stream);
}

int vtd_fpn_train_pack_tap(const void* x_dev, int dtype, int n, int channels, int height, int width, void* tap_dev, vtd_stream stream) {
    return vtd_launch_fpn_pack_tap(x_dev, dtype, n, channels, height, width, tap_dev, (hipStream_t)stream);
}

int64_t vtd_fpn_train_workspace_bytes(int n, int h5, int w5, int c5_channels, int mode) { return vtd_fpn_ws_bytes(n, h5, w5, c5_channels, mode); }

int vtd_fpn_train_forward(const void* const* taps, int n, int h5, int w5, int c5_channels, const vtd_fpn_params* params, void* workspace_dev,
                          void* p2_dev, vtd_stream stream) {
    return vtd_launch_fpn_forward(taps, n, h5, w5, c5_channels, params, workspace_dev, p2_dev, (hipStream_t)stream);
}

int vtd_fpn_train_unpack_p2(const void* p2_dev, int n, int height, int width, float* p2_nchw_dev, vtd_stream stream) {
    return vtd_launch_fpn_unpack_p2(p2_dev, n, height, width, p2_nchw_dev, (hipStream_t)stream);
}

int vtd_fpn_train_pack_grad(const float* grad_nchw_dev, int n, int height, int width, float* dp2_dev, vtd_stream stream) {
    return vtd_launch_fpn_pack_grad(grad_nchw_dev, n, height, width, dp2_dev, (hipStream_t)stream);
}

int vtd_fpn_train_backward(const void* const* taps, int n, int h5, int w5, int c5_channels, const vtd_fpn_params* params, const void* workspace_dev,
                           const float* dp2_dev, const float* dscale_dev, const vtd_fpn_params* grads, void* scratch_dev, vtd_stream stream) {
    return vtd_launch_fpn_backward(taps, n, h5, w5, c5_channels, params, workspace_dev, dp2_dev, dscale_dev, grads, scratch_dev, (hipStream_t)stream);
}

int64_t vtd_basicblock_train_workspace_bytes(int n, int h_in, int w_in, int cin, int width, int stride, int mode) {
    return vtd_basicblock_ws_bytes(n, h_in, w_in, cin, width, stride, mode);
}

int vtd_basicblock_train_forward(const void* x_dev, int n, int h_in, int w_in, int cin, int width, int stride, const vtd_basicblock_params* params,
                                 float eps, void* workspace_dev, void* y_dev, vtd_stream stream) {
    return vtd_launch_basicblock_forward(x_dev, n, h_in, w_in, cin, width, stride, params, eps, workspace_dev, y_dev, (hipStream_t)stream);
}

int vtd_basicblock_train_backward(const void* x_dev, int n, int h_in, int w_in, int cin, int width, int stride, const vtd_basicblock_params* params,
                                  float eps, const void* workspace_dev, const void* y_dev, const float* dy_dev, const float* dscale_dev,
                                  const vtd_basicblock_params* grads, void* scratch_dev, float* dx_dev, float* dxscale_dev, vtd_stream stream) {
    return vtd_launch_basicblock_backward(x_dev, n, h_in, w_in, cin, width, stride, params, eps, workspace_dev, y_dev, dy_dev, dscale_dev, grads,
                                          scratch_dev, dx_dev, dxscale_dev, (hipStream_t)stream);
}

int64_t vtd_resblock_train_workspace_bytes(int n, int h_in, int w_in, int cin, int width, int stride, int mode) {
    return vtd_resblock_ws_bytes(n, h_in, w_in, cin, width, stride, mode);
}

int vtd_resblock_train_forward(const void* x_dev, int n, int h_in, int w_in, int cin, int width, int stride, const vtd_basicblock_params* params,
                               float eps, void* workspace_dev, void* y_dev, vtd_stream stream) {
    return vtd_launch_resblock_forward(x_dev, n, h_in, w_in, cin, width, stride, params, eps, workspace_dev, y_dev, (hipStream_t)stream);
}

int vtd_resblock_train_backward(const void* x_dev, int n, int h_in, int w_in, int cin, int width, int stride, const vtd_basicblock_params* params,
                                float eps, const void* workspace_dev, const void* y_dev, const float* dy_dev, const float* dscale_dev,
                                const vtd_basicblock_params* grads, void* scratch_dev, float* dx_dev, float* dxscale_dev, vtd_stream stream) {
    return vtd_launch_resblock_backward(x_dev, n, h_in, w_in, cin, width, stride, params, eps, workspace_dev, y_dev, dy_dev, dscale_dev, grads,
                                        scratch_dev, dx_dev, dxscale_dev, (hipStream_t)stream);
}

int vtd_resblock_train_combine(float* a_dev, const float* ascale_dev, const float* b_dev, const float* bscale_dev, int64_t numel, float* outscale_dev,
                               vtd_stream stream) {
    return vtd_launch_resblock_combine(a_dev, ascale_dev, b_dev, bscale_dev, numel, outscale_dev, (hipStream_t)stream);
}

int64_t vtd_block64_train_workspace_bytes(int n, int h_in, int w_in, int cin, int width, int stride, int mode) {
    return vtd_block64_ws_bytes(n, h_in, w_in, cin, width, stride, mode);
}

int vtd_block64_train_forward(const void* x_dev, int n, int h_in, int w_in, int cin, int width, int stride, const vtd_basicblock_params* params,
                              float eps, void* workspace_dev, void* y_dev, vtd_stream stream) {
    return vtd_launch_block64_forward(x_dev, n, h_in, w_in, cin, width, stride, params, eps, workspace_dev, y_dev, (hipStream_t)stream);
}

int vtd_block64_train_backward(const void* x_dev, int n, int h_in, int w_in, int cin, int width, int stride, const vtd_basicblock_params* params,
                               float eps, const void* workspace_dev, const void* y_dev, const float* dy_dev, const float* dscale_dev,
                               const vtd_basicblock_params* grads, void* scratch_dev, float* dx_dev, float* dxscale_dev, vtd_stream stream) {
    return vtd_launch_block64_backward(x_dev, n, h_in, w_in, cin, width, stride, params, eps, workspace_dev, y_dev, dy_dev, dscale_dev, grads,
                                       scratch_dev, dx_dev, dxscale_dev, (hipStream_t)stream);
}

int vtd_stem_train_pack_input(const void* x_dev, int dtype, int n, int height, int width, void* tap_dev, vtd_stream stream) {
    return vtd_launch_stem_pack_input(x_dev, dtype, n, height, width, tap_dev, (hipStream_t)stream);
}

int64_t vtd_stem_train_workspace_bytes(int n, int height, int width, int mode) { return vtd_stem_ws_bytes(n, height, width, mode); }

int vtd_stem_train_forward(const void* x_tap_dev, int n, int height, int width, const vtd_stem_params* params, float eps, void* workspace_dev,
                           void* pool_tap_dev, void* idx_dev, vtd_stream stream) {
    return vtd_launch_stem_forward(x_tap_dev, n, height, width, params, eps, workspace_dev, pool_tap_dev, idx_dev, (hipStream_t)stream);
}

int vtd_stem_train_backward(const void* x_tap_dev, int n, int height, int width, const vtd_stem_params* params, float eps, const void* workspace_dev,
                            const void* pool_tap_dev, const void* idx_dev, const float* dpool_dev, const float* dscale_dev, const vtd_stem_params* grads,
                            void* scratch_dev, vtd_stream stream) {
    return vtd_launch_stem_backward(x_tap_dev, n, height, width, params, eps, workspace_dev, pool_tap_dev, idx_dev, dpool_dev, dscale_dev, grads,
                                    scratch_dev, (hipStream_t)stream);
}

int64_t vtd_fpn_train_input_workspace_bytes(int n, int h5, int w5, int c5_channels) { return vtd_fpn_input_ws_bytes(n, h5, w5, c5_channels); }

int vtd_fpn_train_backward_input(int n, int h5, int w5, int c5_channels, const vtd_fpn_params* params, void* scratch_dev, int level_mask,
                                 float* const* dtaps_dev, float* dscale_dev, vtd_stream stream) {
    return vtd_launch_fpn_backward_input(n, h5, w5, c5_channels, params, scratch_dev, level_mask, dtaps_dev, dscale_dev, (hipStream_t)stream);
}

int vtd_fpn_train_unpack_tap_grad(const float* dtap_dev, const float* dscale_dev, int n, int channels, int height, int width, float* grad_nchw_dev,
                                  vtd_stream stream) {
    return vtd_launch_fpn_unpack_tap_grad(dtap_dev, dscale_dev, n, channels, height, width, grad_nchw_dev, (hipStream_t)stream);
}

int vtd_dbhead_unpack_input_grad(const float* dfeats_dev, const float* dscale_dev, int n, int height, int width, float* grad_nchw_dev,
                                 vtd_stream stream) {
    return vtd_launch_dbhead_unpack_input_grad(dfeats_dev, dscale_dev, n, height, width, grad_nchw_dev, (hipStream_t)stream);
}

int vtd_device_count(void) {
    int n = 0;
    hipError_t e = hipGetDeviceCount(&n);
    return e == hipSuccess ? n : -(int)e;
}

int vtd_detector_create(const char* backbone, int max_batch, vtd_detector** out) {
    if (!backbone || !out || max_batch <= 0) return ERR_ARG;
    const std::string b = backbone;
    if (b != "resnet18" && b != "resnet50") return ERR_ARG;
    auto* d = new vtd_detector();
    d->backbone = b;
    d->max_batch = max_batch;
    *out = d;
    return 0;
}

void vtd_detector_destroy(vtd_detector* d) { delete d; }

int vtd_detector_set_tensor(vtd_detector* d, const char* key, const float* host_data, int64_t numel) {
    if (!d || !key || !host_data || numel < 0) return ERR_ARG;
    const std::string k = key;
    if (!known_detector_key(k)) return ERR_UNKNOWN_KEY;
    if (k.size() > 19 && k.compare(k.size() - 19, 19, "num_batches_tracked") == 0) return 0;
    d->sd[k].assign(host_data, host_data + numel);
    return 0;
}

int vtd_detector_set_option(vtd_detector* d, const char* name, int value) {
    if (!d || !name || d->finalized) return ERR_ARG;
    if (std::string(name) == "fuse_fpn_head") { d->fuse_fpn_head = value != 0; return 0; }
    if (std::string(name) == "fuse_stem_pool") { d->fuse_stem_pool = value != 0; return 0; }
    if (std::string(name) == "head_tail_kernel") { d->head_tail_kernel = value != 0; return 0; }
    if (std::string(name) == "fuse_downsample") { d->fuse_downsample = value != 0; return 0; }
    return ERR_UNKNOWN_KEY;
}

int vtd_detector_finalize(vtd_detector* d, vtd_stream stream) {
    if (!d) return ERR_ARG;
    if (d->finalized) return ERR_ARG;
    int rc = build_detector_graph(d);
    if (rc) return rc;
    hipError_t e = hipStreamSynchronize((hipStream_t)stream);
    if (e != hipSuccess) return -(int)e;
    d->sd.clear();
    d->finalized = true;
    return 0;
}

int vtd_detector_preprocess(vtd_detector* d, const uint8_t* frames_dev, int n, int height, int width, vtd_stream stream) {
    if (!d || !frames_dev || height <= 0 || width <= 0) return ERR_ARG;
    if (!d->finalized) return ERR_NOT_FINALIZED;
    if (n <= 0 || n > d->max_batch) return ERR_BATCH;
    PreTables t;
    int rc = get_pre_tables(d, height, width, t);
    if (rc) return rc;
    return vtd_launch_preprocess(frames_dev, n, height, width, d->input.ptr, t.xb, t.xk, t.ksx, t.yb, t.yk, t.ksy, t.max_rows,
                                 (hipStream_t)stream);
}

int vtd_detector_set_input_nchw(vtd_detector* d, const float* x_dev, int n, vtd_stream stream) {
    if (!d || !x_dev) return ERR_ARG;
    if (!d->finalized) return ERR_NOT_FINALIZED;
    if (n <= 0 || n > d->max_batch) return ERR_BATCH;
    return vtd_launch_nchw_to_input(x_dev, d->input.ptr, n, (hipStream_t)stream);
}

static int run_detector_ops(vtd_detector* d, int n, float* prob_dev, float* thresh_dev, hipStream_t s, size_t op_end) {
    float* outs[2] = {prob_dev, thresh_dev};
    const int bucket = batch_bucket(n, d->max_batch);
    auto tit = d->tuned.find(bucket);
    if (tit == d->tuned.end()) {
        std::vector<int> cfgs(d->ops.size(), -1);
        for (size_t oi = 0; oi < d->ops.size(); ++oi)
            if (d->ops[oi].kind == Op::CONV) {
                int rc = choose_config(d, d->ops[oi].conv, bucket, s, &cfgs[oi]);
                if (rc) return rc;
            }
        tit = d->tuned.emplace(bucket, std::move(cfgs)).first;
    }
    const std::vector<int>& cfgs = tit->second;
    for (size_t oi = 0; oi < op_end; ++oi) {
        const Op& o = d->ops[oi];
        int rc = 0;
        if (o.final_slot == 1 && !thresh_dev) continue;
        if (o.kind == Op::BORDER && (oi == 0 || (cfgs[oi - 1] != kHeadEntryHaloCfg && cfgs[oi - 1] != kHeadEntryHalo256Cfg && cfgs[oi - 1] != kHeadEntryPairCfg && cfgs[oi - 1] != kHeadEntryHalfCfg)))
            continue;
        hipEvent_t e0 = nullptr, e1 = nullptr;
        const bool prof = d->profiling && (d->prof_only < 0 || d->prof_only == (int)oi);
        if (prof) {
            e0 = d->take_event();
            e1 = d->take_event();
            if (!e0 || !e1) return ERR_ARG;
            VTD_HIP_CHECK(hipEventRecord(e0, s));
        }
        switch (o.kind) {
            case Op::CONV: rc = launch_conv_op(o.conv, n, s, cfgs[oi]); break;
            case Op::POOL: rc = vtd_launch_maxpool(o.pin, o.pout, n, o.pk[0], o.pk[1], o.pk[2], o.pk[3], o.pk[4], o.pk[5], s); break;
            case Op::FINAL: rc = launch_conv_op(o.conv, n, s, 7, outs[o.final_slot]); break;
            case Op::HEADTAIL:
                rc = vtd_launch_head_tail(o.conv.in, o.htw1, o.conv.bias, o.htw2, o.conv.head_b, outs[o.final_slot], n, s);
                break;
            case Op::BORDER: rc = launch_border_tiles(o.conv, n, s); break;
            case Op::STEMPOOL: rc = vtd_launch_stem_pool(o.pin, o.pout, o.spw, o.spb, n, s); break;
        }
        if (rc) return rc;
        if (prof) {
            VTD_HIP_CHECK(hipEventRecord(e1, s));
            d->ev_spans.push_back({(int)oi, {e0, e1}});
            d->prof_macs[oi] += (o.kind != Op::POOL) ? (double)o.conv.macs_per_image * n : 0.0;
        }
    }
    return 0;
}

int vtd_detector_forward(vtd_detector* d, int n, float* prob_dev, float* thresh_dev, vtd_stream stream) {
    if (!d || !prob_dev) return ERR_ARG;
    if (!d->finalized) return ERR_NOT_FINALIZED;
    if (n <= 0 || n > d->max_batch) return ERR_BATCH;
    return run_detector_ops(d, n, prob_dev, thresh_dev, (hipStream_t)stream, d->ops.size());
}

int vtd_detector_forward_features(vtd_detector* d, int n, void* feats_dev, vtd_stream stream) {
    if (!d || !feats_dev) return ERR_ARG;
    if (!d->finalized) return ERR_NOT_FINALIZED;
    if (n <= 0 || n > d->max_batch) return ERR_BATCH;
    if (d->fuse_fpn_head || !d->p2_ops || !d->taps.count("p2")) return -2801;
    if ((uintptr_t)feats_dev & 15) return -2803;
    hipStream_t s = (hipStream_t)stream;
    int rc = run_detector_ops(d, n, nullptr, nullptr, s, d->p2_ops);
    if (rc) return rc;
    const TensorDesc& p2 = d->taps["p2"];
    VTD_HIP_CHECK(hipMemcpyAsync(feats_dev, p2.ptr, (size_t)n * p2.hp * p2.wp * p2.c * sizeof(half_t), hipMemcpyDeviceToDevice, s));
    return 0;
}

int vtd_detector_forward_trunk(vtd_detector* d, int n, void* c2_dev, void* c3_dev, void* c4_dev, void* c5_dev, vtd_stream stream) {
    void* dst[4] = {c2_dev, c3_dev, c4_dev, c5_dev};
    if (!d || !c2_dev || !c3_dev || !c4_dev || !c5_dev) return ERR_ARG;
    if (!d->finalized) return ERR_NOT_FINALIZED;
    if (n <= 0 || n > d->max_batch) return ERR_BATCH;
    if (d->fuse_fpn_head || !d->trunk_ops) return -2901;
    const char* names[4] = {"c2", "c3", "c4", "c5"};
    for (int i = 0; i < 4; ++i) {
        if ((uintptr_t)dst[i] & 15) return -2903;
        auto it = d->taps.find(names[i]);
        if (it == d->taps.end() || it->second.ring != 1) return -2901;
    }
    hipStream_t s = (hipStream_t)stream;
    int rc = run_detector_ops(d, n, nullptr, nullptr, s, d->trunk_ops);
    if (rc) return rc;
    for (int i = 0; i < 4; ++i) {
        const TensorDesc& t = d->taps[names[i]];
        VTD_HIP_CHECK(hipMemcpyAsync(dst[i], t.ptr, (size_t)n * t.hp * t.wp * t.c * sizeof(half_t), hipMemcpyDeviceToDevice, s));
    }
    return 0;
}

int vtd_detector_forward_pool(vtd_detector* d, int n, void* pool_dev, vtd_stream stream) {
    if (!d || !pool_dev) return ERR_ARG;
    if (!d->finalized) return ERR_NOT_FINALIZED;
    if (n <= 0 || n > d->max_batch) return ERR_BATCH;
    auto it = d->taps.find("pool");
    if (!d->pool_ops || it == d->taps.end() || it->second.ring != 1) return -2901;
    if ((uintptr_t)pool_dev & 15) return -2903;
    hipStream_t s = (hipStream_t)stream;
    int rc = run_detector_ops(d, n, nullptr, nullptr, s, d->pool_ops);
    if (rc) return rc;
    const TensorDesc& t = it->second;
    VTD_HIP_CHECK(hipMemcpyAsync(pool_dev, t.ptr, (size_t)n * t.hp * t.wp * t.c * sizeof(half_t), hipMemcpyDeviceToDevice, s));
    return 0;
}

int vtd_detector_set_profiling(vtd_detector* d, int enable) {
    if (!d || !d->finalized) return ERR_ARG;
    d->profiling = enable != 0;
    d->prof_only = enable >= 2 ? enable - 2 : -1;
    if (d->prof_only >= (int)d->ops.size()) return ERR_ARG;
    d->ev_spans.clear();
    d->ev_used = 0;
    d->prof_ms.assign(d->ops.size(), 0.0);
    d->prof_calls.assign(d->ops.size(), 0);
    d->prof_macs.assign(d->ops.size(), 0.0);
    return 0;
}

int vtd_detector_num_ops(const vtd_detector* d) { return d ? (int)d->ops.size() : 0; }

int vtd_detector_set_tuning(vtd_detector* d, const char* table_text) {
    if (!d) return ERR_ARG;
    int rc = set_tuning_text(d, table_text);
    if (!rc) d->tuned.clear();
    return rc;
}

int64_t vtd_detector_get_tuning(const vtd_detector* d, char* buf, int64_t capacity) { return get_tuning_text(d, buf, capacity); }

int vtd_detector_tuning_measured(const vtd_detector* d) { return d && d->tuning_measured ? 1 : 0; }

int vtd_detector_get_profile(vtd_detector* d, int op_index, char* name, int name_cap, double* total_ms, int64_t* calls,
                             double* total_macs, vtd_stream stream) {
    if (!d || op_index < 0 || op_index >= (int)d->ops.size() || !name || name_cap < 32 || !total_ms || !calls || !total_macs)
        return ERR_ARG;
    if (!d->ev_spans.empty()) {
        hipError_t e = hipStreamSynchronize((hipStream_t)stream);
        if (e != hipSuccess) return -(int)e;
        for (auto& sp : d->ev_spans) {
            float ms = 0.f;
            e = hipEventElapsedTime(&ms, sp.second.first, sp.second.second);
            if (e != hipSuccess) return -(int)e;
            d->prof_ms[sp.first] += ms;
            d->prof_calls[sp.first] += 1;
        }
        d->ev_spans.clear();
        d->ev_used = 0;
    }
    const Op& o = d->ops[op_index];
    if (o.kind == Op::CONV) {
        const ConvOp& c = o.conv;
        static const char* kTile[] = {"256,128,s3", "128,128,s2", "128,128,s3", "256,64,s2", "256,64,s3", "128,64,s2", "128,64,s3",
                                      "64,256,s2", "128,64,s2,classed", "128,64,s3,classed", "256,64,s2,classed", "256,64,s3,classed", "208,128,s3", "272,128,s3", "256,128,s3,16w", "256,256,s2", "128,64,s6"};
        int cfg = -1;
        if (!d->tuned.empty()) cfg = d->tuned.rbegin()->second[op_index];
        if (cfg == kHeadEntryPairCfg)
            std::snprintf(name, name_cap, "head_entry_pair M/img=%d N=%d K=%d (lateral+smooth+head conv composed; border classes in the "
                          "next slot)", c.ho * c.wo, c.cout, c.K);
        else if (cfg == kHeadEntryHalfCfg)
            std::snprintf(name, name_cap, "head_entry_half M/img=%d N=%d K=%d (lateral+smooth+head conv composed, half halos two steps ahead; border classes in the "
                          "next slot)", c.ho * c.wo, c.cout, c.K);
        else if (cfg == kHeadEntryHalo256Cfg)
            std::snprintf(name, name_cap, "head_entry_halo256 M/img=%d N=%d K=%d (lateral+smooth+head conv composed; border classes in the "
                          "next slot)", c.ho * c.wo, c.cout, c.K);
        else if (cfg == kHeadEntryHaloCfg)
            std::snprintf(name, name_cap, "head_entry_halo M/img=%d N=%d K=%d (lateral+smooth+head conv composed; border classes in the "
                          "next slot)", c.ho * c.wo, c.cout, c.K);
        else if (cfg == kPointwiseCfg)
            std::snprintf(name, name_cap, "pointwise128 1x1%s streaming M/img=%d N=%d K=%d", c.has_res ? "+top-down add" : "", c.ho * c.wo, c.cout, c.K);
        else if (cfg == kHaloCfg || cfg == kHaloC64Cfg || cfg == kHalo64Cfg)
            std::snprintf(name, name_cap, "conv_halo%s 3x3 M/img=%d N=%d K=%d", cfg == kHaloC64Cfg ? "_c64_persistent" : cfg == kHalo64Cfg ? "64" : "",
                          c.ho * c.wo, c.cout, c.K);
        else
            std::snprintf(name, name_cap, "conv_igemm<%s> M/img=%d N=%d K=%d%s", (cfg >= 0 && cfg < 17) ? kTile[cfg] : "default",
                          c.ho * c.wo, c.cout, c.K, c.plist ? " (lateral+smooth+head conv composed)" : "");
    } else if (o.kind == Op::POOL) {
        std::snprintf(name, name_cap, "maxpool %dx%d/s%d", o.pk[0], o.pk[1], o.pk[2]);
    } else if (o.kind == Op::BORDER) {
        std::snprintf(name, name_cap, "conv_igemm<128,64,s3,classed> border classes of the composed head entry (%d tiles/img)", o.conv.tiles_border);
    } else if (o.kind == Op::HEADTAIL) {
        std::snprintf(name, name_cap, "head_tail ConvT1+BN+ReLU+ConvT2+sigmoid fused M/img=%d N=256 K=64", o.conv.ho * o.conv.wo);
    } else if (o.kind == Op::STEMPOOL) {
        std::snprintf(name, name_cap, "stem_pool conv7x7/s2+BN+ReLU+maxpool3x3/s2 fused M/img=%d N=64 K=147", 320 * 320);
    } else {
        std::snprintf(name, name_cap, "conv_igemm<64,256,s2> ConvT1+ConvT2+sigmoid fused M/img=%d", o.conv.ho * o.conv.wo);
    }
    const bool have = d->prof_ms.size() == d->ops.size();
    *total_ms = have ? d->prof_ms[op_index] : 0.0;
    *calls = have ? d->prof_calls[op_index] : 0;
    *total_macs = have ? d->prof_macs[op_index] : 0.0;
    return 0;
}

int vtd_detector_read_tap(vtd_detector* d, const char* name, int n, float* host_out, int64_t capacity, vtd_stream stream) {
    if (!d || !name || !host_out) return ERR_ARG;
    if (!d->finalized) return ERR_NOT_FINALIZED;
    auto it = d->taps.find(name);
    if (it == d->taps.end()) return ERR_UNKNOWN_KEY;
    const TensorDesc& t = it->second;
    if (n <= 0 || n > t.n) return ERR_BATCH;
    const int creal = (std::string(name) == "input") ? 3 : t.c;
    if (capacity < (int64_t)n * creal * t.h * t.w) return ERR_CAPACITY;
    return read_tensor_nchw(t, n, creal, host_out, (hipStream_t)stream);
}

int64_t vtd_detector_macs_per_frame(const vtd_detector* d) { return d ? d->macs : 0; }

}

namespace vtd {

static int build_recognizer_graph(vtd_recognizer* r) {
    const int D = r->max_crops;
    int rc;
    auto new_tensor = [&](int h, int w, int c, int ring, TensorDesc& t) {
        t = make_desc(D, h, w, c, ring, ring);
        return r->alloc_tensor(t);
    };
    void* p = nullptr;
    if ((rc = r->arena.alloc(&p, (size_t)D * 32 * 128 * 3, true))) return rc;
    r->resized = (uint8_t*)p;
    {
        Fold f;
        if ((rc = fold_bn(r, "cnn.1", "cnn.0.bias", 64, f))) return rc;
        auto w = r->get("cnn.0.weight", 64 * 3 * 3 * 3);
        if (!w) return ERR_MISSING_KEY;
        std::vector<half_t> wp(64 * 32, (half_t)0.f);
        std::vector<float> bp(64);
        for (int co = 0; co < 64; ++co) {
            bp[co] = (float)f.shift[co];
            for (int c = 0; c < 3; ++c)
                for (int rr = 0; rr < 3; ++rr)
                    for (int ss = 0; ss < 3; ++ss)
                        wp[co * 32 + (rr * 3 + ss) * 3 + c] = half_of((double)(*w)[((co * 3 + c) * 3 + rr) * 3 + ss] * f.scale[co]);
        }
        if ((rc = upload(r->arena, wp.data(), wp.size() * sizeof(half_t), (void**)&r->w1))) return rc;
        if ((rc = upload(r->arena, bp.data(), bp.size() * 4, (void**)&r->b1))) return rc;
        if ((rc = new_tensor(16, 64, 64, 1, r->t1))) return rc;
        r->macs += (int64_t)32 * 128 * 64 * 27;
    }
    struct Spec { int conv, bn, cin, cout, k, pad, ph, pw; };
    const Spec specs[6] = {{4, 5, 64, 128, 3, 1, 2, 2},  {8, 9, 128, 256, 3, 1, 0, 0},   {11, 12, 256, 256, 3, 1, 2, 1},
                           {15, 16, 256, 512, 3, 1, 0, 0}, {18, 19, 512, 512, 3, 1, 2, 1}, {22, 23, 512, 512, 2, 0, 0, 0}};
    TensorDesc x = r->t1;
    for (const Spec& sp : specs) {
        const int ho = x.h + 2 * sp.pad - sp.k + 1, wo = x.w + 2 * sp.pad - sp.k + 1;
        TensorDesc y;
        const bool pooled = sp.ph == 2 && r->fuse_pools && !(ho & 1) && wo % sp.pw == 0;
        if (pooled) y = make_desc(D, ho, wo, sp.cout, 1, 1);
        else if ((rc = new_tensor(ho, wo, sp.cout, 1, y))) return rc;
        Fold f;
        const std::string ck = "cnn." + std::to_string(sp.conv), bk = "cnn." + std::to_string(sp.bn);
        if ((rc = fold_bn(r, bk, ck + ".bias", sp.cout, f))) return rc;
        Op o;
        o.kind = Op::CONV;
        if ((rc = build_conv(r, o.conv, x, y, ck + ".weight", f, sp.cin, sp.cout, sp.k, sp.k, 1, sp.pad, EPI_RELU))) return rc;
        if (pooled) {
            TensorDesc z;
            if ((rc = new_tensor(ho / 2, wo / sp.pw, sp.cout, 1, z))) return rc;
            o.conv.out = z;
            o.conv.pool_pw = sp.pw;
            y = z;
        }
        r->ops.push_back(o);
        r->macs += o.conv.macs_per_image;
        x = y;
        if (sp.ph && !pooled) {
            TensorDesc z;
            if ((rc = new_tensor(x.h / sp.ph, x.w / sp.pw, x.c, 1, z))) return rc;
            Op po;
            po.kind = Op::POOL;
            po.pin = x; po.pout = z;
            const int pk[6] = {sp.ph, sp.pw, sp.ph, sp.pw, 0, 0};
            std::memcpy(po.pk, pk, sizeof(pk));
            r->ops.push_back(po);
            x = z;
        }
    }
    if (x.h != 1 || x.w != 31 || x.c != 512) return ERR_GEOMETRY;
    r->t7 = x;
    r->taps["cnn"] = x;
    const int T = 31;
    if ((rc = r->arena.alloc(&p, (size_t)D * T * 2048 * sizeof(half_t), true))) return rc;
    r->xs = (half_t*)p;
    if ((rc = r->arena.alloc(&p, (size_t)D * T * 128 * 4, true))) return rc;
    r->logits_pad = (float*)p;
    r->h0 = make_desc(D, 1, T, 512, 0, 0);
    r->h1 = make_desc(D, 1, T, 512, 0, 0);
    if ((rc = r->alloc_tensor(r->h0)) || (rc = r->alloc_tensor(r->h1))) return rc;
    r->taps["h0"] = r->h0;
    r->taps["h1"] = r->h1;
    for (int layer = 0; layer < 2; ++layer) {
        std::vector<float> W((size_t)2048 * 512), B(2048);
        std::vector<half_t> whh((size_t)2 * 1024 * 256);
        for (int dir = 0; dir < 2; ++dir) {
            const std::string suf = "_l" + std::to_string(layer) + (dir ? "_reverse" : "");
            auto wih = r->get("rnn.weight_ih" + suf, (size_t)1024 * 512), wh = r->get("rnn.weight_hh" + suf, (size_t)1024 * 256);
            auto bih = r->get("rnn.bias_ih" + suf, 1024), bhh = r->get("rnn.bias_hh" + suf, 1024);
            if (!wih || !wh || !bih || !bhh) return ERR_MISSING_KEY;
            std::copy(wih->begin(), wih->end(), W.begin() + (size_t)dir * 1024 * 512);
            for (int i = 0; i < 1024; ++i) B[dir * 1024 + i] = (*bih)[i] + (*bhh)[i];
            for (size_t i = 0; i < (size_t)1024 * 256; ++i) whh[(size_t)dir * 1024 * 256 + i] = (half_t)(*wh)[i];
        }
        if ((rc = build_linear(r, r->xs_gemm[layer], layer ? r->h0 : r->t7, W, B, 2048, 512, r->xs, 2048, EPI_OUT_F16))) return rc;
        if ((rc = upload(r->arena, whh.data(), whh.size() * sizeof(half_t), (void**)&r->whh[layer]))) return rc;
        r->macs += r->xs_gemm[layer].macs_per_image + (int64_t)2 * T * 1024 * 256;
    }
    {
        auto w = r->get("classifier.weight", (size_t)r->vocab * 512), b = r->get("classifier.bias", r->vocab);
        if (!w || !b) return ERR_MISSING_KEY;
        if (r->vocab > 128) return ERR_GEOMETRY;
        if ((rc = build_linear(r, r->cls_gemm, r->h1, *w, *b, r->vocab, 512, r->logits_pad, 128))) return rc;
        r->macs += r->cls_gemm.macs_per_image;
    }
    return 0;
}

}

extern "C" {

int vtd_recognizer_create(int vocab_size, int max_crops, vtd_recognizer** out) {
    if (!out || vocab_size <= 0 || vocab_size > 128 || max_crops <= 0) return ERR_ARG;
    auto* r = new vtd_recognizer();
    r->vocab = vocab_size;
    r->max_crops = max_crops;
    *out = r;
    return 0;
}

void vtd_recognizer_destroy(vtd_recognizer* r) { delete r; }

int vtd_recognizer_set_tensor(vtd_recognizer* r, const char* key, const float* host_data, int64_t numel) {
    if (!r || !key || !host_data || numel < 0) return ERR_ARG;
    const std::string k = key;
    if (k.rfind("cnn.", 0) != 0 && k.rfind("rnn.", 0) != 0 && k.rfind("classifier.", 0) != 0) return ERR_UNKNOWN_KEY;
    if (k.size() > 19 && k.compare(k.size() - 19, 19, "num_batches_tracked") == 0) return 0;
    r->sd[k].assign(host_data, host_data + numel);
    return 0;
}

int vtd_recognizer_set_option(vtd_recognizer* r, const char* name, int value) {
    if (!r || !name || r->finalized) return ERR_ARG;
    if (std::string(name) == "fuse_pools") { r->fuse_pools = value != 0; return 0; }
    return ERR_UNKNOWN_KEY;
}

int vtd_recognizer_finalize(vtd_recognizer* r, vtd_stream stream) {
    if (!r || r->finalized) return ERR_ARG;
    int rc = build_recognizer_graph(r);
    if (rc) return rc;
    hipError_t e = hipStreamSynchronize((hipStream_t)stream);
    if (e != hipSuccess) return -(int)e;
// ... 100 lines not shown
```

video-text-detection-system_amd/csrc/vtd_common.h:

```cpp
#pragma once
#include <hip/hip_runtime.h>
#include <stdint.h>

typedef _Float16 half_t;
typedef half_t half8 __attribute__((ext_vector_type(8)));
typedef half_t half4 __attribute__((ext_vector_type(4)));
typedef half_t half2v __attribute__((ext_vector_type(2)));
typedef float floatx4 __attribute__((ext_vector_type(4)));

#define VTD_AS1 __attribute__((address_space(1)))
#define VTD_AS3 __attribute__((address_space(3)))

struct TensorDesc {
    half_t* ptr;
    int n, h, w, c;
    int ring;
    int hp, wp;
};

static inline __host__ __device__ int64_t tensor_elems(const TensorDesc& t) {
    return (int64_t)t.n * t.hp * t.wp * t.c;
}

enum : int {
    EPI_RELU = 1,
    EPI_RESIDUAL = 2,
    EPI_PIXEL_SHUFFLE = 4,
    EPI_OUT_F32 = 8,
    EPI_OUT_F16 = 32,
    EPI_GELU = 64,
    EPI_HEAD_FINAL = 16,
};

struct ConvParams {
    const half_t* in;
    const half_t* wgt;
    int cin_steps, kw, s_step, r_step;
    int k_hi_step;
    const float* bias;
    const half_t* res;
    void* out;
    int M;
    int K;
    int cout;
    int cout_pad;
    int ho, wo;
    int in_hp, in_wp, in_c;
    int in_y0, in_x0;
    int stride;
    int out_hp, out_wp, out_c, out_ring;
    int res_hp, res_wp, res_ring, res_shift;
    int ps_cout;
    int flags;
    int dbg;
    int ldc;
    int seg_cols;
    void* seg_out[3];
    int seg_ldc[3];
    int epi_direct;
    int pool_pw, pool_log2, pool_wq, pool_hqwq;
    uint64_t magic_wo, magic_howo;
    int magic_ok;
    const uint32_t* plist;
    const int* tile_combo;
    const uint32_t* plist_b;
    const int* tile_combo_b;
    int tiles_per_img_b;
    int tiles_per_img;
    const half_t* in2;
    int in2_hp, in2_wp, in2_c, in2_ring;
    int in2_mul, in2_shr;
    int seg1_steps;
    int cin_steps2, kw2, s_step2, r_step2;
    const float* bias_tab;
    int img_h, img_w;
    const float* head_w;
    float head_b;
    float* prob_out;
};

#define VTD_HIP_CHECK(expr)                                   \
    do {                                                      \
        hipError_t _e = (expr);                               \
        if (_e != hipSuccess) return -(int)_e;                \
    } while (0)
```

video-text-detection-system_amd/vtd_amd/_native.py:

```python
import ctypes as C
import os

_HERE = os.path.dirname(os.path.abspath(__file__))
_VARIANT = os.environ.get("VTD_LIB_VARIANT", "")
LIB_PATH = os.path.join(_HERE, "_lib", f"libvtd_hip_{_VARIANT}.so" if _VARIANT else "libvtd_hip.so")

_lib = None


class NativeError(RuntimeError):
    pass


class TrocrConfig(C.Structure):
    _fields_ = [("image_size", C.c_int32), ("patch_size", C.c_int32), ("enc_hidden", C.c_int32), ("enc_layers", C.c_int32),
                ("enc_heads", C.c_int32), ("enc_ffn", C.c_int32), ("enc_qkv_bias", C.c_int32), ("enc_ln_eps", C.c_float),
                ("dec_hidden", C.c_int32), ("dec_layers", C.c_int32), ("dec_heads", C.c_int32), ("dec_ffn", C.c_int32),
                ("vocab_size", C.c_int32), ("max_positions", C.c_int32), ("dec_ln_eps", C.c_float),
                ("decoder_start_token_id", C.c_int32), ("eos_token_id", C.c_int32), ("pad_token_id", C.c_int32), ("max_length", C.c_int32)]


class Detection(C.Structure):
    _fields_ = [("bbox", C.c_int32 * 4), ("polygon", C.c_int32 * 8), ("confidence", C.c_float), ("area", C.c_float),
                ("first_x", C.c_int32), ("first_y", C.c_int32)]


class DbHeadBranch(C.Structure):
    _fields_ = [(k, C.c_void_p) for k in ("conv_w", "conv_b", "bn1_w", "bn1_b", "bn1_mean", "bn1_var", "ct1_w", "ct1_b", "bn2_w", "bn2_b",
                                          "bn2_mean", "bn2_var", "ct2_w", "ct2_b")]


class DbHeadParams(C.Structure):
    _fields_ = [("branch", DbHeadBranch * 2)]


class FpnParams(C.Structure):
    _fields_ = [("inner_w", C.c_void_p * 4), ("inner_b", C.c_void_p * 4), ("layer_w", C.c_void_p), ("layer_b", C.c_void_p)]


BLOCK_FIELDS = ("conv1_w", "bn1_w", "bn1_b", "bn1_mean", "bn1_var", "conv2_w", "bn2_w", "bn2_b", "bn2_mean", "bn2_var",
                "ds_w", "ds_bn_w", "ds_bn_b", "ds_bn_mean", "ds_bn_var")


class BasicBlockParams(C.Structure):
    _fields_ = [(k, C.c_void_p) for k in BLOCK_FIELDS]


class StemParams(C.Structure):
    _fields_ = [(k, C.c_void_p) for k in ("w", "gamma", "beta", "mean", "var")]


FpnTaps = C.c_void_p * 4


SIGNATURES = {
    "vtd_version": (C.c_char_p, []),
    "vtd_strerror": (C.c_char_p, [C.c_int]),
    "vtd_device_count": (C.c_int, []),
    "vtd_detector_create": (C.c_int, [C.c_char_p, C.c_int, C.POINTER(C.c_void_p)]),
    "vtd_detector_destroy": (None, [C.c_void_p]),
    "vtd_detector_set_tensor": (C.c_int, [C.c_void_p, C.c_char_p, C.c_void_p, C.c_int64]),
    "vtd_detector_set_option": (C.c_int, [C.c_void_p, C.c_char_p, C.c_int]),
    "vtd_detector_finalize": (C.c_int, [C.c_void_p, C.c_void_p]),
    "vtd_detector_preprocess": (C.c_int, [C.c_void_p, C.c_void_p, C.c_int, C.c_int, C.c_int, C.c_void_p]),
    "vtd_detector_set_input_nchw": (C.c_int, [C.c_void_p, C.c_void_p, C.c_int, C.c_void_p]),
    "vtd_detector_forward": (C.c_int, [C.c_void_p, C.c_int, C.c_void_p, C.c_void_p, C.c_void_p]),
    "vtd_detector_read_tap": (C.c_int, [C.c_void_p, C.c_char_p, C.c_int, C.c_void_p, C.c_int64, C.c_void_p]),
    "vtd_detector_macs_per_frame": (C.c_int64, [C.c_void_p]),
    "vtd_detector_set_profiling": (C.c_int, [C.c_void_p, C.c_int]),
    "vtd_detector_num_ops": (C.c_int, [C.c_void_p]),
    "vtd_detector_get_profile": (C.c_int, [C.c_void_p, C.c_int, C.c_char_p, C.c_int, C.POINTER(C.c_double), C.POINTER(C.c_int64),
                                           C.POINTER(C.c_double), C.c_void_p]),
    "vtd_detector_set_tuning": (C.c_int, [C.c_void_p, C.c_char_p]),
    "vtd_detector_get_tuning": (C.c_int64, [C.c_void_p, C.c_char_p, C.c_int64]),
    "vtd_detector_tuning_measured": (C.c_int, [C.c_void_p]),
    "vtd_postproc_create": (C.c_int, [C.c_int, C.c_int, C.c_int, C.c_int, C.POINTER(C.c_void_p)]),
    "vtd_postproc_destroy": (None, [C.c_void_p]),
    "vtd_copy_to_pinned_host": (C.c_int, [C.c_void_p, C.c_void_p, C.c_int64, C.c_void_p]),
    "vtd_postproc_run": (C.c_int, [C.c_void_p, C.c_void_p, C.c_int, C.c_void_p, C.c_void_p, C.c_float, C.c_void_p, C.c_void_p,
                                   C.c_void_p]),
    "vtd_recognizer_create": (C.c_int, [C.c_int, C.c_int, C.POINTER(C.c_void_p)]),
    "vtd_recognizer_set_option": (C.c_int, [C.c_void_p, C.c_char_p, C.c_int]),
    "vtd_recognizer_destroy": (None, [C.c_void_p]),
    "vtd_recognizer_set_tensor": (C.c_int, [C.c_void_p, C.c_char_p, C.c_void_p, C.c_int64]),
    "vtd_recognizer_finalize": (C.c_int, [C.c_void_p, C.c_void_p]),
    "vtd_recognizer_crop_resize": (C.c_int, [C.c_void_p, C.c_void_p, C.c_int, C.c_int, C.c_int, C.c_void_p, C.c_int, C.c_void_p]),
    "vtd_recognizer_set_input_nchw": (C.c_int, [C.c_void_p, C.c_void_p, C.c_int, C.c_void_p]),
    "vtd_recognizer_forward": (C.c_int, [C.c_void_p, C.c_int, C.c_void_p, C.c_void_p]),
    "vtd_recognizer_read_tap": (C.c_int, [C.c_void_p, C.c_char_p, C.c_int, C.c_void_p, C.c_int64, C.c_void_p]),
    "vtd_recognizer_macs_per_crop": (C.c_int64, [C.c_void_p]),
    "vtd_recognizer_set_tuning": (C.c_int, [C.c_void_p, C.c_char_p]),
    "vtd_recognizer_get_tuning": (C.c_int64, [C.c_void_p, C.c_char_p, C.c_int64]),
    "vtd_recognizer_tuning_measured": (C.c_int, [C.c_void_p]),
    "vtd_trocr_create": (C.c_int, [C.c_void_p, C.c_int, C.POINTER(C.c_void_p)]),
    "vtd_trocr_destroy": (None, [C.c_void_p]),
    "vtd_trocr_set_tensor": (C.c_int, [C.c_void_p, C.c_char_p, C.c_void_p, C.c_int64]),
    "vtd_trocr_finalize": (C.c_int, [C.c_void_p, C.c_void_p]),
    "vtd_trocr_encode_crops": (C.c_int, [C.c_void_p, C.c_void_p, C.c_int, C.c_int, C.c_int, C.c_void_p, C.c_int, C.c_void_p]),
    "vtd_trocr_encode_pixels": (C.c_int, [C.c_void_p, C.c_void_p, C.c_int, C.c_void_p]),
    "vtd_trocr_generate": (C.c_int, [C.c_void_p, C.c_int, C.c_int, C.c_void_p, C.c_int, C.c_void_p, C.c_void_p, C.c_void_p]),
    "vtd_trocr_num_slots": (C.c_int, [C.c_void_p]),
    "vtd_trocr_encode_crops_slot": (C.c_int, [C.c_void_p, C.c_int, C.c_void_p, C.c_int, C.c_int, C.c_int, C.c_void_p, C.c_int, C.c_void_p]),
    "vtd_trocr_encode_pixels_slot": (C.c_int, [C.c_void_p, C.c_int, C.c_void_p, C.c_int, C.c_void_p]),
    "vtd_trocr_stage_crops_slot": (C.c_int, [C.c_void_p, C.c_int, C.c_void_p, C.c_int, C.c_int, C.c_int, C.c_void_p, C.c_int, C.c_int, C.c_void_p]),
    "vtd_trocr_encode_staged_slot": (C.c_int, [C.c_void_p, C.c_int, C.c_int, C.c_void_p]),
    "vtd_trocr_generate_slot": (C.c_int, [C.c_void_p, C.c_int, C.c_int, C.c_int, C.c_void_p, C.c_int, C.c_void_p, C.c_void_p, C.c_void_p]),
    "vtd_trocr_last_steps": (C.c_int, [C.c_void_p]),
    "vtd_dbloss_workspace_bytes": (C.c_int64, []),
    "vtd_dbloss_forward": (C.c_int, [C.c_void_p, C.c_void_p, C.c_void_p, C.c_void_p, C.c_int64, C.c_float, C.c_void_p, C.c_void_p, C.c_void_p,
                                     C.c_void_p]),
    "vtd_dbloss_backward": (C.c_int, [C.c_void_p, C.c_void_p, C.c_void_p, C.c_void_p, C.c_int64, C.c_float, C.c_void_p, C.c_void_p, C.c_void_p,
                                      C.c_void_p, C.c_void_p]),
    "vtd_detector_forward_features": (C.c_int, [C.c_void_p, C.c_int, C.c_void_p, C.c_void_p]),
    "vtd_dbhead_pack_features": (C.c_int, [C.c_void_p, C.c_int, C.c_int, C.c_int, C.c_int, C.c_void_p, C.c_void_p]),
    "vtd_dbhead_train_workspace_bytes": (C.c_int64, [C.c_int, C.c_int, C.c_int, C.c_int]),
    "vtd_dbhead_train_forward": (C.c_int, [C.c_void_p, C.c_int, C.c_int, C.c_int, C.POINTER(DbHeadParams), C.c_int, C.c_float, C.c_float,
                                           C.c_void_p, C.c_void_p, C.c_void_p, C.c_void_p, C.c_void_p]),
    "vtd_dbhead_train_backward": (C.c_int, [C.c_void_p, C.c_int, C.c_int, C.c_int, C.POINTER(DbHeadParams), C.c_int, C.c_void_p, C.c_void_p,
                                            C.c_void_p, C.c_void_p, C.c_void_p, C.POINTER(DbHeadParams), C.c_void_p, C.c_void_p]),
    "vtd_dbhead_train_backward_input": (C.c_int, [C.c_int, C.c_int, C.c_int, C.POINTER(DbHeadParams), C.c_void_p, C.c_void_p, C.c_void_p, C.c_void_p]),
    "vtd_dbhead_unpack_input_grad": (C.c_int, [C.c_void_p, C.c_void_p, C.c_int, C.c_int, C.c_int, C.c_void_p, C.c_void_p]),
    "vtd_detector_forward_trunk": (C.c_int, [C.c_void_p, C.c_int, C.c_void_p, C.c_void_p, C.c_void_p, C.c_void_p, C.c_void_p]),
    "vtd_fpn_train_pack_tap": (C.c_int, [C.c_void_p, C.c_int, C.c_int, C.c_int, C.c_int, C.c_int, C.c_void_p, C.c_void_p]),
    "vtd_fpn_train_workspace_bytes": (C.c_int64, [C.c_int, C.c_int, C.c_int, C.c_int, C.c_int]),
    "vtd_fpn_train_forward": (C.c_int, [C.POINTER(FpnTaps), C.c_int, C.c_int, C.c_int, C.c_int, C.POINTER(FpnParams), C.c_void_p, C.c_void_p,
                                        C.c_void_p]),
    "vtd_fpn_train_unpack_p2": (C.c_int, [C.c_void_p, C.c_int, C.c_int, C.c_int, C.c_void_p, C.c_void_p]),
    "vtd_fpn_train_pack_grad": (C.c_int, [C.c_void_p, C.c_int, C.c_int, C.c_int, C.c_void_p, C.c_void_p]),
    "vtd_fpn_train_backward": (C.c_int, [C.POINTER(FpnTaps), C.c_int, C.c_int, C.c_int, C.c_int, C.POINTER(FpnParams), C.c_void_p, C.c_void_p,
                                         C.c_void_p, C.POINTER(FpnParams), C.c_void_p, C.c_void_p]),
    "vtd_basicblock_train_workspace_bytes": (C.c_int64, [C.c_int] * 7),
    "vtd_basicblock_train_forward": (C.c_int, [C.c_void_p] + [C.c_int] * 6 + [C.POINTER(BasicBlockParams), C.c_float, C.c_void_p, C.c_void_p, C.c_void_p]),
    "vtd_basicblock_train_backward": (C.c_int, [C.c_void_p] + [C.c_int] * 6 + [C.POINTER(BasicBlockParams), C.c_float, C.c_void_p, C.c_void_p, C.c_void_p,
                                                C.c_void_p, C.POINTER(BasicBlockParams), C.c_void_p, C.c_void_p, C.c_void_p, C.c_void_p]),
    "vtd_resblock_train_workspace_bytes": (C.c_int64, [C.c_int] * 7),
    "vtd_resblock_train_forward": (C.c_int, [C.c_void_p] + [C.c_int] * 6 + [C.POINTER(BasicBlockParams), C.c_float, C.c_void_p, C.c_void_p, C.c_void_p]),
    "vtd_resblock_train_backward": (C.c_int, [C.c_void_p] + [C.c_int] * 6 + [C.POINTER(BasicBlockParams), C.c_float, C.c_void_p, C.c_void_p, C.c_void_p,
                                              C.c_void_p, C.POINTER(BasicBlockParams), C.c_void_p, C.c_void_p, C.c_void_p, C.c_void_p]),
    "vtd_resblock_train_combine": (C.c_int, [C.c_void_p, C.c_void_p, C.c_void_p, C.c_void_p, C.c_int64, C.c_void_p, C.c_void_p]),
    "vtd_block64_train_workspace_bytes": (C.c_int64, [C.c_int] * 7),
    "vtd_block64_train_forward": (C.c_int, [C.c_void_p] + [C.c_int] * 6 + [C.POINTER(BasicBlockParams), C.c_float, C.c_void_p, C.c_void_p, C.c_void_p]),
    "vtd_block64_train_backward": (C.c_int, [C.c_void_p] + [C.c_int] * 6 + [C.POINTER(BasicBlockParams), C.c_float, C.c_void_p, C.c_void_p, C.c_void_p,
                                             C.c_void_p, C.POINTER(BasicBlockParams), C.c_void_p, C.c_void_p, C.c_void_p, C.c_void_p]),
    "vtd_stem_train_pack_input": (C.c_int, [C.c_void_p, C.c_int, C.c_int, C.c_int, C.c_int, C.c_void_p, C.c_void_p]),
    "vtd_stem_train_workspace_bytes": (C.c_int64, [C.c_int] * 4),
    "vtd_stem_train_forward": (C.c_int, [C.c_void_p, C.c_int, C.c_int, C.c_int, C.POINTER(StemParams), C.c_float, C.c_void_p, C.c_void_p, C.c_void_p,
                                         C.c_void_p]),
    "vtd_stem_train_backward": (C.c_int, [C.c_void_p, C.c_int, C.c_int, C.c_int, C.POINTER(StemParams), C.c_float, C.c_void_p, C.c_void_p, C.c_void_p,
                                          C.c_void_p, C.c_void_p, C.POINTER(StemParams), C.c_void_p, C.c_void_p]),
    "vtd_detector_forward_pool": (C.c_int, [C.c_void_p, C.c_int, C.c_void_p, C.c_void_p]),
    "vtd_fpn_train_input_workspace_bytes": (C.c_int64, [C.c_int, C.c_int, C.c_int, C.c_int]),
    "vtd_fpn_train_backward_input": (C.c_int, [C.c_int, C.c_int, C.c_int, C.c_int, C.POINTER(FpnParams), C.c_void_p, C.c_int, C.POINTER(FpnTaps),
                                               C.c_void_p, C.c_void_p]),
    "vtd_fpn_train_unpack_tap_grad": (C.c_int, [C.c_void_p, C.c_void_p, C.c_int, C.c_int, C.c_int, C.c_int, C.c_void_p, C.c_void_p]),
    "vtd_binary_counts_accumulate": (C.c_int, [C.c_void_p, C.c_void_p, C.c_int64, C.c_float, C.c_void_p, C.c_void_p]),
    "vtd_trocr_set_option": (C.c_int, [C.c_void_p, C.c_char_p, C.c_int]),
    "vtd_trocr_get_option": (C.c_int, [C.c_void_p, C.c_char_p, C.POINTER(C.c_int)]),
    "vtd_trocr_set_profiling": (C.c_int, [C.c_void_p, C.c_int]),
    "vtd_trocr_get_profile": (C.c_int, [C.c_void_p, C.POINTER(C.c_double), C.POINTER(C.c_int64), C.POINTER(C.c_int64), C.c_void_p]),
    "vtd_trocr_get_gemm_profile": (C.c_int, [C.c_void_p, C.POINTER(C.c_double), C.POINTER(C.c_int64), C.POINTER(C.c_double), C.c_void_p]),
    "vtd_trocr_read_tap": (C.c_int, [C.c_void_p, C.c_char_p, C.c_int, C.c_void_p, C.c_int64, C.c_void_p]),
    "vtd_trocr_encoder_tokens": (C.c_int, [C.c_void_p]),
    "vtd_trocr_logits_stride": (C.c_int, [C.c_void_p]),
    "vtd_trocr_macs_per_crop": (C.c_int64, [C.c_void_p]),
    "vtd_trocr_set_tuning": (C.c_int, [C.c_void_p, C.c_char_p]),
    "vtd_trocr_get_tuning": (C.c_int64, [C.c_void_p, C.c_char_p, C.c_int64]),
    "vtd_trocr_tuning_measured": (C.c_int, [C.c_void_p]),
    "vtd_ctc_greedy_decode": (C.c_int, [C.c_void_p, C.c_int, C.c_int, C.c_int, C.c_void_p, C.c_int, C.c_int, C.c_void_p, C.c_void_p]),
}


def load():
    global _lib
    if _lib is None:
        import torch
        if not os.path.exists(LIB_PATH):
            raise NativeError(f"{LIB_PATH} is missing: build it with `python __graft_entry__.py` (hipcc, gfx950)")
        lib = C.CDLL(LIB_PATH)
        for name, (res, args) in SIGNATURES.items():
            fn = getattr(lib, name)
            fn.restype = res
            fn.argtypes = args
        _lib = lib
    return _lib


def require():
    lib = load()
    n = lib.vtd_device_count()
    if n <= 0:
        raise NativeError("libvtd_hip.so loaded but no HIP device is visible; this package has no CPU fallback")
    return lib


def check(code, what=""):
    if code != 0:
        msg = load().vtd_strerror(code)
        raise NativeError(f"{what or 'vtd call'} failed: {msg.decode() if msg else code} ({code})")
```

video-text-detection-system_amd/vtd_amd/engine.py:

```python
import ctypes as C
import logging
import os
import queue
import sys
import threading

import numpy as np
import torch

from . import _native

logger = logging.getLogger(__name__)

DEFAULT_MAX_BATCH = int(os.environ.get("VTD_MAX_BATCH", "32"))

TUNING_FILE = os.path.join(os.path.dirname(os.path.abspath(__file__)), "tuning", "gfx950.txt")


def shipped_tuning_text():
    if os.environ.get("VTD_TUNING", "1") == "0":
        return ""
    path = os.environ.get("VTD_TUNING_FILE", TUNING_FILE)
    try:
        with open(path) as f:
# ... 8 lines not shown

    def set_tuning(self, text):
        if text:
            fn = getattr(self.lib, f"vtd_{self._kind}_set_tuning")
            with self.lock:
                _native.check(fn(self.handle, text.encode()), f"vtd_{self._kind}_set_tuning")

    def tuning_text(self):
        fn = getattr(self.lib, f"vtd_{self._kind}_get_tuning")
        need = fn(self.handle, None, 0)
        buf = C.create_string_buffer(int(need))
        fn(self.handle, buf, need)
        return buf.value.decode()

    def tuning(self):
        return {k: int(v) for k, v in (line.rsplit(" ", 1) for line in self.tuning_text().splitlines() if line)}

    @property
    def tuning_measured(self):
        return bool(getattr(self.lib, f"vtd_{self._kind}_tuning_measured")(self.handle))


def _stream_ptr():
    return C.c_void_p(torch.cuda.current_stream().cuda_stream)


class PinnedPool:

    def __init__(self):
        self._free = {}
        self._lock = threading.Lock()

    def take(self, shape, dtype=torch.int32):
        key = (tuple(shape), dtype)
        with self._lock:
            lst = self._free.get(key)
            if lst:
                return lst.pop()
        return torch.empty(shape, dtype=dtype).pin_memory()

    def release(self, t, event):
        if event is not None:
            event.synchronize()
        with self._lock:
            self._free.setdefault((tuple(t.shape), t.dtype), []).append(t)


PINNED = PinnedPool()


def copy_to_pinned(dst, src):
    nbytes = src.numel() * src.element_size()
    if nbytes >= 16 and dst.is_pinned() and src.is_contiguous() and dst.is_contiguous() and dst.numel() * dst.element_size() == nbytes and \
            _native.require().vtd_copy_to_pinned_host(src.data_ptr(), dst.data_ptr(), nbytes, torch.cuda.current_stream().cuda_stream) == 0:
        return
    dst.copy_(src, non_blocking=True)


class DeviceFrames:

    def __init__(self, frames, stream=None):
        if isinstance(frames, np.ndarray):
            frames = torch.from_numpy(np.ascontiguousarray(frames))
        elif isinstance(frames, (list, tuple)):
            frames = torch.from_numpy(np.ascontiguousarray(np.stack(frames)))
        if frames.dim() == 3:
            frames = frames.unsqueeze(0)
        if frames.dtype != torch.uint8 or frames.dim() != 4 or frames.shape[-1] != 3:
            raise ValueError("frames must be uint8 [n,H,W,3] (BGR)")
        self.ready = None
        if stream is None or frames.is_cuda:
            self.tensor = frames.to("cuda", non_blocking=True).contiguous()
        else:
            with torch.cuda.stream(stream):
                self.tensor = frames.contiguous().to("cuda", non_blocking=True)
                self.ready = torch.cuda.Event()
                self.ready.record()

    def wait_ready(self):
        if self.ready is not None:
            torch.cuda.current_stream().wait_event(self.ready)

    @property
    def n(self):
        return self.tensor.shape[0]

    @property
    def height(self):
        return self.tensor.shape[1]

    @property
    def width(self):
        return self.tensor.shape[2]


class DetectorEngine(_Tunable):

    _kind = "detector"

    def __init__(self, backbone, state_dict, max_batch=None, options=None):
        self.lib = _native.require()
        self.max_batch = max_batch or DEFAULT_MAX_BATCH
        self.backbone = backbone
        self.lock = threading.Lock()
        h = C.c_void_p()
        _native.check(self.lib.vtd_detector_create(backbone.encode(), self.max_batch, C.byref(h)), "vtd_detector_create")
        self.handle = h
        try:
            for name, value in (options or {}).items():
                _native.check(self.lib.vtd_detector_set_option(h, name.encode(), int(value)), f"vtd_detector_set_option({name})")
            for key, value in state_dict.items():
                if key.endswith("num_batches_tracked"):
                    continue
                arr = np.ascontiguousarray(value.detach().cpu().float().numpy())
                _native.check(self.lib.vtd_detector_set_tensor(h, key.encode(), arr.ctypes.data, arr.size),
                              f"vtd_detector_set_tensor({key})")
            _native.check(self.lib.vtd_detector_finalize(h, _stream_ptr()), "vtd_detector_finalize")
            self.set_tuning(shipped_tuning_text())
        except Exception:
            self.close()
            raise

    def close(self):
        if getattr(self, "handle", None):
            self.lib.vtd_detector_destroy(self.handle)
            self.handle = None

    def __del__(self):
        try:
            self.close()
        except Exception:
            pass

    @property
    def macs_per_frame(self):
        return int(self.lib.vtd_detector_macs_per_frame(self.handle))

    def _set_input(self, x):
        if isinstance(x, DeviceFrames):
            n = x.n
            x.wait_ready()
            _native.check(self.lib.vtd_detector_preprocess(self.handle, C.c_void_p(x.tensor.data_ptr()), n, x.height, x.width,
                                                           _stream_ptr()), "vtd_detector_preprocess")
            return n, x
        if not torch.is_tensor(x) or x.dim() != 4 or tuple(x.shape[1:]) != (3, 640, 640):
            raise ValueError("DBNet input must be [n,3,640,640] float or a DeviceFrames batch")
        xd = x.to("cuda", torch.float32).contiguous()
        _native.check(self.lib.vtd_detector_set_input_nchw(self.handle, C.c_void_p(xd.data_ptr()), xd.shape[0], _stream_ptr()),
                      "vtd_detector_set_input_nchw")
        return xd.shape[0], xd

    def forward(self, x, want_threshold=False):
        with self.lock:
            n, keep = self._set_input(x)
            prob = torch.empty((n, 1, 640, 640), dtype=torch.float32, device="cuda")
            thr = torch.empty_like(prob) if want_threshold else None
            _native.check(self.lib.vtd_detector_forward(self.handle, n, C.c_void_p(prob.data_ptr()),
                                                        C.c_void_p(thr.data_ptr()) if thr is not None else None, _stream_ptr()),
                          "vtd_detector_forward")
            del keep
            return {"probability": prob, "threshold": thr}

    def forward_features(self, x):
        with self.lock:
            n, keep = self._set_input(x)
            feats = torch.empty((n, 162, 162, 256), dtype=torch.float16, device="cuda")
            _native.check(self.lib.vtd_detector_forward_features(self.handle, n, C.c_void_p(feats.data_ptr()), _stream_ptr()),
                          "vtd_detector_forward_features")
            del keep
            return feats

    def forward_trunk(self, x):
        wide = 4 if self.backbone == "resnet50" else 1
        with self.lock:
            n, keep = self._set_input(x)
            taps = [torch.empty((n, (160 >> i) + 2, (160 >> i) + 2, (64 << i) * wide), dtype=torch.float16, device="cuda") for i in range(4)]
            _native.check(self.lib.vtd_detector_forward_trunk(self.handle, n, *(C.c_void_p(t.data_ptr()) for t in taps), _stream_ptr()),
                          "vtd_detector_forward_trunk")
            del keep
            return taps

    def forward_pool(self, x):
        with self.lock:
            n, keep = self._set_input(x)
            tap = torch.empty((n, 162, 162, 64), dtype=torch.float16, device="cuda")
            _native.check(self.lib.vtd_detector_forward_pool(self.handle, n, C.c_void_p(tap.data_ptr()), _stream_ptr()),
                          "vtd_detector_forward_pool")
            del keep
            return tap

    def read_tap(self, name, n):
        shapes = {"input": (3, 640, 640), "stem": (64, 320, 320), "pool": (64, 160, 160), "p2": (256, 160, 160), "head1": (64, 160, 160),
                  "head2": (64, 320, 320)}
        if name not in shapes:
            wide = self.backbone == "resnet50"
            idx = int(name[1]) - 2
            ch = (64, 128, 256, 512)[idx] * (4 if wide else 1)
            shapes[name] = (ch, 160 >> idx, 160 >> idx)
        c, h, w = shapes[name]
        out = np.empty((n, c, h, w), np.float32)
        with self.lock:
            _native.check(self.lib.vtd_detector_read_tap(self.handle, name.encode(), n, out.ctypes.data, out.size, _stream_ptr()),
                          f"vtd_detector_read_tap({name})")
        return out


class PostProcessor:

    def __init__(self, max_batch, map_h=640, map_w=640, max_out=1024):
        self.lib = _native.require()
        self.max_batch, self.h, self.w, self.max_out = max_batch, map_h, map_w, max_out
        self.lock = threading.Lock()
        h = C.c_void_p()
        _native.check(self.lib.vtd_postproc_create(max_batch, map_h, map_w, max_out, C.byref(h)), "vtd_postproc_create")
        self.handle = h
        self.records = torch.empty((max_batch, max_out, 16), dtype=torch.int32, device="cuda")
        self.counts = torch.empty((max_batch,), dtype=torch.int32, device="cuda")

    def close(self):
        if getattr(self, "handle", None):
            self.lib.vtd_postproc_destroy(self.handle)
            self.handle = None

    def __del__(self):
        try:
            self.close()
        except Exception:
            pass

    def run_device(self, prob, orig_w, orig_h, threshold, records=None, counts=None):
        n = prob.shape[0]
        records = self.records if records is None else records
        counts = self.counts if counts is None else counts
        if prob.dtype != torch.float32 or not prob.is_cuda or tuple(prob.shape[-2:]) != (self.h, self.w):
            raise ValueError("probability maps must be float32 cuda tensors of the workspace's map size")
        prob = prob.reshape(n, self.h, self.w).contiguous()
        ow = np.ascontiguousarray(orig_w, dtype=np.int32)
        oh = np.ascontiguousarray(orig_h, dtype=np.int32)
        _native.check(self.lib.vtd_postproc_run(self.handle, C.c_void_p(prob.data_ptr()), n, ow.ctypes.data, oh.ctypes.data,
                                                float(threshold), C.c_void_p(records.data_ptr()),
                                                C.c_void_p(counts.data_ptr()), _stream_ptr()), "vtd_postproc_run")
        self._keep = (prob, ow, oh)
        return records[:n], counts[:n]

    def run(self, prob, orig_w, orig_h, threshold, debug=False):
        with self.lock:
            rec, cnt = self.run_device(prob, orig_w, orig_h, threshold)
            cnt = cnt.cpu().numpy()
            if int(cnt.max(initial=0)) > self.max_out:
                import logging
                logging.getLogger(__name__).warning(f"frame with {int(cnt.max())} components exceeds max_detections={self.max_out}; "
                                                    "extra detections dropped")
            kmax = int(min(cnt.max(initial=0), self.max_out))
            rec = rec[:, :kmax].cpu().numpy() if kmax else np.zeros((len(cnt), 0, 16), np.int32)
        return [records_to_dicts(rec[i, :min(int(cnt[i]), self.max_out)], debug) for i in range(len(cnt))]


def records_to_dicts(rec, debug=False):
    if len(rec) == 0:
        return []
    bbox = rec[:, 0:4].tolist()
    poly = rec[:, 4:12].reshape(-1, 4, 2).tolist()
    conf = np.ascontiguousarray(rec[:, 12]).view(np.float32).tolist()
    out = [{"bbox": b, "confidence": c, "polygon": p} for b, c, p in zip(bbox, conf, poly)]
    if debug:
        area = np.ascontiguousarray(rec[:, 13]).view(np.float32).tolist()
        first = rec[:, 14:16].tolist()
        for d, a, f in zip(out, area, first):
            d["_area"] = a
            d["_first"] = tuple(f)
    return out


def detector_profile(engine):
    lib, out = engine.lib, []
    name = C.create_string_buffer(160)
    ms, calls, macs = C.c_double(), C.c_int64(), C.c_double()
    for i in range(lib.vtd_detector_num_ops(engine.handle)):
        _native.check(lib.vtd_detector_get_profile(engine.handle, i, name, 160, C.byref(ms), C.byref(calls), C.byref(macs),
                                                   _stream_ptr()), "vtd_detector_get_profile")
        out.append((name.value.decode(), ms.value, calls.value, macs.value))
    return out


class RecognizerEngine(_Tunable):

    _kind = "recognizer"

    T = 31

    def __init__(self, vocab_size, state_dict, max_crops=None, options=None):
        self.lib = _native.require()
        self.vocab_size = vocab_size
        self.max_crops = max_crops or int(os.environ.get("VTD_MAX_CROPS", "512"))
        self.lock = threading.Lock()
        h = C.c_void_p()
        _native.check(self.lib.vtd_recognizer_create(vocab_size, self.max_crops, C.byref(h)), "vtd_recognizer_create")
        self.handle = h
        try:
            env_opts = {k: int(v) for k, v in (kv.split("=") for kv in os.environ.get("VTD_RECOGNIZER_OPTIONS", "").split(",") if kv)}
            for name, value in {**env_opts, **(options or {})}.items():
                _native.check(self.lib.vtd_recognizer_set_option(h, name.encode(), int(value)), f"vtd_recognizer_set_option({name})")
            for key, value in state_dict.items():
                if key.endswith("num_batches_tracked"):
                    continue
                arr = np.ascontiguousarray(value.detach().cpu().float().numpy())
                _native.check(self.lib.vtd_recognizer_set_tensor(h, key.encode(), arr.ctypes.data, arr.size),
                              f"vtd_recognizer_set_tensor({key})")
            _native.check(self.lib.vtd_recognizer_finalize(h, _stream_ptr()), "vtd_recognizer_finalize")
            self.set_tuning(shipped_tuning_text())
        except Exception:
            self.close()
# ... 433 lines not shown
```

Measured before the change: 12520.

## Fuse frame resize/normalise preprocessing into the stem conv+pool kernel

Adds a frames_stem_pool kernel that reads raw uint8 720p frames, does the separable Pillow-style resample and LUT normalisation per tile in LDS, and feeds the result straight into the stem conv+maxpool MFMA path. This removes the separate preprocess kernel and the round trip of the padded 646x646 f16 input tensor through global memory. It reuses the shared helpers, now factored into a header, and falls back to the old two-step path when the frame geometry is not eligible. The cost is heavier LDS use per workgroup and redundant resampling of halo rows between neighbouring tiles.

```diff
diff --git a/include/vtd.h b/include/vtd.h
--- a/include/vtd.h
+++ b/include/vtd.h
@@ -33,6 +33,8 @@
 int vtd_detector_preprocess(vtd_detector* d, const uint8_t* frames_dev, int n, int height, int width, vtd_stream stream);
 int vtd_detector_set_input_nchw(vtd_detector* d, const float* x_dev, int n, vtd_stream stream);
 int vtd_detector_forward(vtd_detector* d, int n, float* prob_dev, float* thresh_dev, vtd_stream stream);
+int vtd_detector_forward_frames(vtd_detector* d, const uint8_t* frames_dev, int n, int height, int width, float* prob_dev,
+                                float* thresh_dev, vtd_stream stream);
 int vtd_detector_read_tap(vtd_detector* d, const char* name, int n, float* host_out, int64_t capacity, vtd_stream stream);
 int64_t vtd_detector_macs_per_frame(const vtd_detector* d);
 int vtd_detector_set_profiling(vtd_detector* d, int enable);
diff --git a/video-text-detection-system_amd/csrc/detector_misc.hip b/video-text-detection-system_amd/csrc/detector_misc.hip
--- a/video-text-detection-system_amd/csrc/detector_misc.hip
+++ b/video-text-detection-system_amd/csrc/detector_misc.hip
@@ -1,6 +1,9 @@
 #include "vtd_common.h"
+#include "preprocess_taps.h"
 
 namespace {
+
+using namespace vtd_pre;
 
 constexpr int PRE_TY = 16;
 constexpr int PRE_OUT = 640;
@@ -22,11 +25,6 @@
     int max_rows;
     unsigned quads_magic;
 };
-
-__device__ __forceinline__ uint8_t clip8_22(int v) {
-    v >>= 22;
-    return (uint8_t)(v < 0 ? 0 : (v > 255 ? 255 : v));
-}
 
 __global__ __launch_bounds__(256) void preprocess_kernel(const PreParams p) {
     extern __shared__ __attribute__((aligned(16))) uint8_t rows[];
@@ -135,14 +133,7 @@
         ytab[i] = e < 2 ? p.yb[2 * oy + e] : p.yk[oy * KSY + (e - 2)];
     }
     for (int i = tid; i < PRE_CHUNK * KSX; i += PRE_NT) raw[(i / KSX) * raw_pitch + p.W + (i % KSX)] = 0u;
-    {
-        const float mean[3] = {0.485f, 0.456f, 0.406f};
-        const float stdv[3] = {0.229f, 0.224f, 0.225f};
-        if (tid < 256) {
-#pragma unroll
-            for (int c = 0; c < 3; ++c) lut[c * 256 + tid] = (half_t)(((float)tid / 255.0f - mean[c]) / stdv[c]);
-        }
-    }
+    fill_lut(lut, tid);
 
     const int quads = p.W >> 2;
     constexpr int MAXIT = (PRE_CHUNK * 512 + PRE_NT - 1) / PRE_NT;
@@ -166,13 +157,7 @@
             const int i = tid + it * PRE_NT;
             if (i < nr * quads) {
                 const int rr = (int)__umulhi((unsigned)i, p.quads_magic), q = i - rr * quads;
-                const uint32_t d0 = stg[it][0], d1 = stg[it][1], d2 = stg[it][2];
-                uint4 px;
-                px.x = d0 & 0xffffffu;
-                px.y = ((d0 >> 24) | (d1 << 8)) & 0xffffffu;
-                px.z = ((d1 >> 16) | (d2 << 16)) & 0xffffffu;
-                px.w = d2 >> 8;
-                *(uint4*)(raw + rr * raw_pitch + q * 4) = px;
+                *(uint4*)(raw + rr * raw_pitch + q * 4) = widen_quad(stg[it][0], stg[it][1], stg[it][2]);
             }
         }
         __syncthreads();
@@ -183,16 +168,10 @@
             for (int s = 0; s < PRE_COLS; ++s) {
                 const int ox = tid + PRE_NT * s;
                 if (ox < PRE_OUT) {
-                    uint32_t s0 = 1u << 21, s1 = 1u << 21, s2 = 1u << 21;
-#pragma unroll
-                    for (int t = 0; t < KSX; ++t) {
-                        const uint32_t px = row[xmin[s] + t];
-                        const uint32_t kt = (uint32_t)kx[s][t];
-                        s0 = __umul24(px & 0xffu, kt) + s0;
-                        s1 = __umul24((px >> 8) & 0xffu, kt) + s1;
-                        s2 = __umul24(px >> 16, kt) + s2;
-                    }
-                    rows[(r0 + rr) * PRE_OUT + ox] = (uint32_t)clip8_22((int)s0) | ((uint32_t)clip8_22((int)s1) << 8) | ((uint32_t)clip8_22((int)s2) << 16);
+                    Acc3 a;
+#pragma unroll
+                    for (int t = 0; t < KSX; ++t) tap(a, row[xmin[s] + t], (uint32_t)kx[s][t]);
+                    rows[(r0 + rr) * PRE_OUT + ox] = pack_levels(a);
                 }
             }
         }
@@ -211,11 +190,7 @@
         if (oy >= PRE_OUT) break;
         const int* yt = ytab + ty * (2 + KSY);
         const int ymin = yt[0] - y_first;
-        uint32_t acc[4][3];
-#pragma unroll
-        for (int q = 0; q < 4; ++q)
-#pragma unroll
-            for (int c = 0; c < 3; ++c) acc[q][c] = 1u << 21;
+        Acc3 acc[4];
 #pragma unroll
         for (int t = 0; t < KSY; ++t) {
             const uint32_t kv = (uint32_t)yt[2 + t];
@@ -223,26 +198,11 @@
             const uint4 px = *(const uint4*)(rows + r * PRE_OUT + g * 4);
             const uint32_t pv[4] = {px.x, px.y, px.z, px.w};
 #pragma unroll
-            for (int q = 0; q < 4; ++q) {
-                acc[q][0] = __umul24(pv[q] & 0xffu, kv) + acc[q][0];
-                acc[q][1] = __umul24((pv[q] >> 8) & 0xffu, kv) + acc[q][1];
-                acc[q][2] = __umul24(pv[q] >> 16, kv) + acc[q][2];
-            }
-        }
-        half8 o01, o23;
-#pragma unroll
-        for (int q = 0; q < 4; ++q) {
-            const half_t h0 = lut[clip8_22((int)acc[q][2])];
-            const half_t h1 = lut[256 + clip8_22((int)acc[q][1])];
-            const half_t h2 = lut[512 + clip8_22((int)acc[q][0])];
-            if (q < 2) { o01[q * 4] = h0; o01[q * 4 + 1] = h1; o01[q * 4 + 2] = h2; o01[q * 4 + 3] = (half_t)0.f; }
-            else { o23[(q - 2) * 4] = h0; o23[(q - 2) * 4 + 1] = h1; o23[(q - 2) * 4 + 2] = h2; o23[(q - 2) * 4 + 3] = (half_t)0.f; }
+            for (int q = 0; q < 4; ++q) tap(acc[q], pv[q], kv);
         }
         half_t* dst = p.out + (((int64_t)img * 646 + oy + 3) * 646 + g * 4 + 3) * 4;
-        *(half4*)(dst) = half4{o01[0], o01[1], o01[2], o01[3]};
-        *(half4*)(dst + 4) = half4{o01[4], o01[5], o01[6], o01[7]};
-        *(half4*)(dst + 8) = half4{o23[0], o23[1], o23[2], o23[3]};
-        *(half4*)(dst + 12) = half4{o23[4], o23[5], o23[6], o23[7]};
+#pragma unroll
+        for (int q = 0; q < 4; ++q) *(half4*)(dst + 4 * q) = normalise(lut, acc[q]);
     }
 }
 
diff --git a/video-text-detection-system_amd/csrc/preprocess_taps.h b/video-text-detection-system_amd/csrc/preprocess_taps.h
--- /dev/null
+++ b/video-text-detection-system_amd/csrc/preprocess_taps.h
@@ -0,0 +1,47 @@
+#pragma once
+#include "vtd_common.h"
+
+namespace vtd_pre {
+
+__device__ __forceinline__ uint8_t clip8_22(int v) {
+    v >>= 22;
+    return (uint8_t)(v < 0 ? 0 : (v > 255 ? 255 : v));
+}
+
+__device__ __forceinline__ uint4 widen_quad(uint32_t d0, uint32_t d1, uint32_t d2) {
+    uint4 px;
+    px.x = d0 & 0xffffffu;
+    px.y = ((d0 >> 24) | (d1 << 8)) & 0xffffffu;
+    px.z = ((d1 >> 16) | (d2 << 16)) & 0xffffffu;
+    px.w = d2 >> 8;
+    return px;
+}
+
+struct Acc3 {
+    uint32_t s0 = 1u << 21, s1 = 1u << 21, s2 = 1u << 21;
+};
+
+__device__ __forceinline__ void tap(Acc3& a, uint32_t px, uint32_t kt) {
+    a.s0 = __umul24(px & 0xffu, kt) + a.s0;
+    a.s1 = __umul24((px >> 8) & 0xffu, kt) + a.s1;
+    a.s2 = __umul24(px >> 16, kt) + a.s2;
+}
+
+__device__ __forceinline__ uint32_t pack_levels(const Acc3& a) {
+    return (uint32_t)clip8_22((int)a.s0) | ((uint32_t)clip8_22((int)a.s1) << 8) | ((uint32_t)clip8_22((int)a.s2) << 16);
+}
+
+__device__ __forceinline__ void fill_lut(half_t* lut, int tid) {
+    const float mean[3] = {0.485f, 0.456f, 0.406f};
+    const float stdv[3] = {0.229f, 0.224f, 0.225f};
+    if (tid < 256) {
+#pragma unroll
+        for (int c = 0; c < 3; ++c) lut[c * 256 + tid] = (half_t)(((float)tid / 255.0f - mean[c]) / stdv[c]);
+    }
+}
+
+__device__ __forceinline__ half4 normalise(const half_t* lut, const Acc3& a) {
+    return half4{lut[clip8_22((int)a.s2)], lut[256 + clip8_22((int)a.s1)], lut[512 + clip8_22((int)a.s0)], (half_t)0.f};
+}
+
+}
diff --git a/video-text-detection-system_amd/csrc/stem_pool.hip b/video-text-detection-system_amd/csrc/stem_pool.hip
--- a/video-text-detection-system_amd/csrc/stem_pool.hip
+++ b/video-text-detection-system_amd/csrc/stem_pool.hip
@@ -1,5 +1,6 @@
 #include <cstdlib>
 #include "vtd_common.h"
+#include "preprocess_taps.h"
 
 namespace {
 
@@ -45,6 +46,38 @@
     px0 = (r - ty * p.tiles_x) * SP_PT_COLS;
 }
 
+__device__ __forceinline__ void sp_tile_range(int total_tiles, int& first, int& stride, int& last) {
+    if ((gridDim.x & 7) == 0) {
+        const int xcd = blockIdx.x & 7, per = gridDim.x >> 3;
+        const int lo = (int)(((int64_t)total_tiles * xcd) >> 3);
+        last = (int)(((int64_t)total_tiles * (xcd + 1)) >> 3);
+        first = lo + (blockIdx.x >> 3);
+        stride = per;
+    } else {
+        first = blockIdx.x; stride = gridDim.x; last = total_tiles;
+    }
+}
+
+__device__ __forceinline__ void sp_setup(const StemPoolParams& p, half8 (&wreg)[7][4], int (&a_off)[4], float* bias_lds, int tid, int wv) {
+    const int lane = tid & 63, fr = lane & 15, fq = lane >> 4;
+#pragma unroll
+    for (int ky = 0; ky < 7; ++ky)
+#pragma unroll
+        for (int i = 0; i < 4; ++i) wreg[ky][i] = *(const half8*)(p.w + ((ky * 4 + i) * 64 + lane) * 8);
+    if (tid < 64) bias_lds[tid] = p.bias[tid];
+#pragma unroll
+    for (int j = 0; j < 4; ++j) {
+        const int pix = wv * 64 + j * 16 + fr;
+        const int c_row = pix / SP_CT_COLS, c_col = pix - c_row * SP_CT_COLS;
+        a_off[j] = ((2 * c_row) * SP_PATCH_COLS + 2 * c_col + 2 * fq) * 8;
+    }
+}
+
+template <int DBG, typename AfterMfma>
+__device__ __forceinline__ void sp_tile_math(const StemPoolParams& p, const half8 (&wreg)[7][4], const int (&a_off)[4], const unsigned char* pb,
+                                             unsigned char* ctile, const float* bias_lds, int img, int py0, int px0, int wv, int lane,
+                                             AfterMfma&& after_mfma);
+
 template <int DBG>
 __global__ __launch_bounds__(256, 2) void stem_pool_kernel(const StemPoolParams p) {
     extern __shared__ __attribute__((aligned(16))) unsigned char sp_smem[];
@@ -53,34 +86,15 @@
     float* const bias_lds = (float*)(ctile + 256 * SP_CT_PITCH);
     const int tid = threadIdx.x, lane = tid & 63;
     const int wv = __builtin_amdgcn_readfirstlane(tid >> 6);
-    const int fr = lane & 15, fq = lane >> 4;
 
     int first, stride, last;
-    if ((gridDim.x & 7) == 0) {
-        const int xcd = blockIdx.x & 7, per = gridDim.x >> 3;
-        const int lo = (int)(((int64_t)p.total_tiles * xcd) >> 3);
-        last = (int)(((int64_t)p.total_tiles * (xcd + 1)) >> 3);
-        first = lo + (blockIdx.x >> 3);
-        stride = per;
-    } else {
-        first = blockIdx.x; stride = gridDim.x; last = p.total_tiles;
-    }
+    sp_tile_range(p.total_tiles, first, stride, last);
     if (first >= last) return;
     const int nt = (last - first + stride - 1) / stride;
 
     half8 wreg[7][4];
-#pragma unroll
-    for (int ky = 0; ky < 7; ++ky)
-#pragma unroll
-        for (int i = 0; i < 4; ++i) wreg[ky][i] = *(const half8*)(p.w + ((ky * 4 + i) * 64 + lane) * 8);
-    if (tid < 64) bias_lds[tid] = p.bias[tid];
     int a_off[4];
-#pragma unroll
-    for (int j = 0; j < 4; ++j) {
-        const int pix = wv * 64 + j * 16 + fr;
-        const int c_row = pix / SP_CT_COLS, c_col = pix - c_row * SP_CT_COLS;
-        a_off[j] = ((2 * c_row) * SP_PATCH_COLS + 2 * c_col + 2 * fq) * 8;
-    }
+    sp_setup(p, wreg, a_off, bias_lds, tid, wv);
     int u_row[3], u_col[3];
 #pragma unroll
     for (int k = 0; k < 3; ++k) {
@@ -118,12 +132,24 @@
         sp_tile_coords(p, __builtin_amdgcn_readfirstlane(tile), img, py0, px0);
         if (k + 2 < nt) issue(tile + 2 * stride, st == 0 ? SP_NST - 1 : st - 1);
 
+        sp_tile_math<DBG>(p, wreg, a_off, ring + st * SP_PATCH_BYTES, ctile, bias_lds, img, py0, px0, wv, lane, [] {});
+        if (k + 2 < nt) sp_wait_vmcnt<3>(); else sp_wait_vmcnt<0>();
+        sp_lds_barrier();
+        st = st + 1 == SP_NST ? 0 : st + 1;
+    }
+}
+
+template <int DBG, typename AfterMfma>
+__device__ __forceinline__ void sp_tile_math(const StemPoolParams& p, const half8 (&wreg)[7][4], const int (&a_off)[4], const unsigned char* pb,
+                                             unsigned char* ctile, const float* bias_lds, int img, int py0, int px0, int wv, int lane,
+                                             AfterMfma&& after_mfma) {
+    const int fr = lane & 15, fq = lane >> 4;
+    {
         floatx4 acc[4][4];
 #pragma unroll
         for (int i = 0; i < 4; ++i)
 #pragma unroll
             for (int j = 0; j < 4; ++j) acc[i][j] = *(const floatx4*)(bias_lds + sp_chan(i, fq * 4));
-        const unsigned char* pb = ring + st * SP_PATCH_BYTES;
         half8 af[2][4];
 #pragma unroll
         for (int j = 0; j < 4; ++j) af[0][j] = *(const half8*)(pb + a_off[j]);
@@ -145,14 +171,12 @@
         }
 
         if constexpr (DBG == 6 || DBG == 7) __builtin_amdgcn_s_setprio(0);
+        after_mfma();
         if constexpr (DBG == 2) {
             float t = 0.f;
             for (int i = 0; i < 4; ++i) for (int j = 0; j < 4; ++j) t += acc[i][j][0] + acc[i][j][1] + acc[i][j][2] + acc[i][j][3];
             if (t == 123.456f) p.out[0] = (half_t)t;
-            if (k + 2 < nt) sp_wait_vmcnt<3>(); else sp_wait_vmcnt<0>();
-            sp_lds_barrier();
-            st = st + 1 == SP_NST ? 0 : st + 1;
-            continue;
+            return;
         }
 #pragma unroll
         for (int j = 0; j < 4; ++j) {
@@ -203,9 +227,167 @@
                     *(half8*)(p.out + (((int64_t)img * p.out_hp + py + p.out_ring) * p.out_wp + px + p.out_ring) * 64 + cg * 8) = m;
             }
         }
-        if (k + 2 < nt) sp_wait_vmcnt<3>(); else sp_wait_vmcnt<0>();
+    }
+}
+
+constexpr int FS_ROWS = 35;
+constexpr int FS_QPR = 22;
+constexpr int FS_RAW_PITCH = FS_QPR * 4;
+constexpr int FS_FETCH = 4;
+constexpr int FS_MAX_RAW_ROWS = (FS_FETCH * 256) / FS_QPR;
+constexpr int FS_RAW_BYTES = (FS_MAX_RAW_ROWS + 1) * FS_RAW_PITCH * 4;
+constexpr int FS_HRES_BYTES = FS_MAX_RAW_ROWS * SP_PATCH_COLS * 4;
+constexpr int FS_TAB = 8;
+static_assert(FS_RAW_BYTES % 16 == 0 && FS_HRES_BYTES <= 256 * SP_CT_PITCH, "hres lives inside the conv tile");
+constexpr int FS_LDS = SP_PATCH_BYTES + 256 * SP_CT_PITCH + FS_RAW_BYTES + 256 + 3 * 256 * 2 + (SP_PATCH_COLS + FS_ROWS) * FS_TAB * 4;
+static_assert(FS_LDS <= 80 * 1024, "two workgroups per CU");
+
+struct FramesStemParams {
+    StemPoolParams sp;
+    const uint8_t* frames;
+    const int *xtab, *ytab;
+    int H, W;
+    FramesStemSpans spans;
+};
+
+template <int KSX, int KSY>
+__global__ __launch_bounds__(256, 2) void frames_stem_pool_kernel(const FramesStemParams q) {
+    static_assert(KSX < FS_TAB && KSY < FS_TAB && SP_PATCH_COLS * (1 + KSX) <= 256 && FS_ROWS * (1 + KSY) <= 256, "one table value per lane");
+    using namespace vtd_pre;
+    const StemPoolParams& p = q.sp;
+    extern __shared__ __attribute__((aligned(16))) unsigned char sp_smem[];
+    unsigned char* const patch = sp_smem;
+    unsigned char* const ctile = sp_smem + SP_PATCH_BYTES;
+    uint32_t* const hres = (uint32_t*)ctile;
+    uint32_t* const raw = (uint32_t*)(ctile + 256 * SP_CT_PITCH);
+    float* const bias_lds = (float*)((unsigned char*)raw + FS_RAW_BYTES);
+    half_t* const lut = (half_t*)(bias_lds + 64);
+    int* const xtab = (int*)(lut + 3 * 256);
+    int* const ytab = xtab + SP_PATCH_COLS * FS_TAB;
+    const int tid = threadIdx.x, lane = tid & 63;
+    const int wv = __builtin_amdgcn_readfirstlane(tid >> 6);
+
+    int first, stride, last;
+    sp_tile_range(p.total_tiles, first, stride, last);
+    if (first >= last) return;
+    const int nt = (last - first + stride - 1) / stride;
+
+    half8 wreg[7][4];
+    int a_off[4];
+    sp_setup(p, wreg, a_off, bias_lds, tid, wv);
+    fill_lut(lut, tid);
+    for (int i = FS_ROWS * SP_PATCH_COLS * 8 + tid * 8; i < SP_PATCH_BYTES; i += 256 * 8) *(uint2*)(patch + i) = uint2{0u, 0u};
+
+    auto fetch_slot = [&](int it, int& row, int& quad) {
+        int t = tid;
+        asm volatile("" : "+v"(t));
+        const int i = t + 256 * it;
+        row = i / FS_QPR;
+        quad = i - row * FS_QPR;
+    };
+    struct Fetched {
+        uint32_t stg[FS_FETCH][3];
+        int xt, yt, x_first, y_first, nrows;
+    };
+    auto fetch = [&](int tile) {
+        Fetched f;
+        int img, py0, px0;
+        sp_tile_coords(p, __builtin_amdgcn_readfirstlane(tile), img, py0, px0);
+        const int ty = py0 / SP_PT_ROWS, tx = px0 / SP_PT_COLS;
+        const int nquads = q.spans.nquads[tx];
+        f.nrows = q.spans.nrows[ty]; f.y_first = q.spans.y_first[ty]; f.x_first = q.spans.x_first[tx];
+        const int ix = min(tid, SP_PATCH_COLS * (1 + KSX) - 1), cx = ix / (1 + KSX);
+        const int iy = min(tid, FS_ROWS * (1 + KSY) - 1), ry = iy / (1 + KSY);
+        const int ox = min(max(4 * px0 - 5 + cx, 0), 639), oy = min(max(4 * py0 - 5 + ry, 0), 639);
+        const int* gx = q.xtab + ox * FS_TAB + (ix - cx * (1 + KSX));
+        const int* gy = q.ytab + oy * FS_TAB + (iy - ry * (1 + KSY));
+        const uint8_t* src = q.frames + ((int64_t)img * q.H + f.y_first) * q.W * 3 + f.x_first * 3;
+        const uint32_t* g[FS_FETCH];
+#pragma unroll
+        for (int it = 0; it < FS_FETCH; ++it) {
+            int f_row, f_quad;
+            fetch_slot(it, f_row, f_quad);
+            f_row = min(f_row, f.nrows - 1);
+            f_quad = min(f_quad, nquads - 1);
+            g[it] = (const uint32_t*)(src + ((int64_t)f_row * q.W + 4 * f_quad) * 3);
+        }
+        __builtin_amdgcn_sched_barrier(0);
+#pragma unroll
+        for (int it = 0; it < FS_FETCH; ++it) { f.stg[it][0] = g[it][0]; f.stg[it][1] = g[it][1]; f.stg[it][2] = g[it][2]; }
+        f.xt = *gx;
+        f.yt = *gy;
+        __builtin_amdgcn_sched_barrier(0);
+        return f;
+    };
+    auto stage = [&](const Fetched& f) {
+#pragma unroll
+        for (int it = 0; it < FS_FETCH; ++it) {
+            int f_row, f_quad;
+            fetch_slot(it, f_row, f_quad);
+            *(uint4*)(raw + f_row * FS_RAW_PITCH + f_quad * 4) = widen_quad(f.stg[it][0], f.stg[it][1], f.stg[it][2]);
+        }
+        if (tid < SP_PATCH_COLS * (1 + KSX)) xtab[(tid / (1 + KSX)) * FS_TAB + tid % (1 + KSX)] = tid % (1 + KSX) == 0 ? f.xt - f.x_first : f.xt;
+        if (tid < FS_ROWS * (1 + KSY)) ytab[(tid / (1 + KSY)) * FS_TAB + tid % (1 + KSY)] = tid % (1 + KSY) == 0 ? f.yt - f.y_first : f.yt;
+    };
+
+    int nrows;
+    {
+        const Fetched f0 = fetch(first);
+        stage(f0);
+        nrows = f0.nrows;
+    }
+    sp_lds_barrier();
+    for (int k = 0; k < nt; ++k) {
+        const int tile = first + k * stride;
+        int img, py0, px0;
+        sp_tile_coords(p, __builtin_amdgcn_readfirstlane(tile), img, py0, px0);
+
+        int tconv = tid;
+        asm volatile("" : "+v"(tconv));
+        const int hg = tconv / SP_PATCH_COLS, hc = tconv - hg * SP_PATCH_COLS;
+        if (hg < 6) {
+            const int xm = xtab[hc * FS_TAB];
+            uint32_t kx[KSX];
+#pragma unroll
+            for (int t = 0; t < KSX; ++t) kx[t] = (uint32_t)xtab[hc * FS_TAB + 1 + t];
+            for (int rr = hg; rr < nrows; rr += 6) {
+                const uint32_t* row = raw + rr * FS_RAW_PITCH + xm;
+                Acc3 a;
+#pragma unroll
+                for (int t = 0; t < KSX; ++t) tap(a, row[t], kx[t]);
+                hres[rr * SP_PATCH_COLS + hc] = pack_levels(a);
+            }
+        }
         sp_lds_barrier();
-        st = st + 1 == SP_NST ? 0 : st + 1;
+        if (hg < 6) {
+            const int ox = 4 * px0 - 5 + hc;
+#pragma unroll
+            for (int i = 0; i < (FS_ROWS + 5) / 6; ++i) {
+                const int r = hg + 6 * i;
+                if (r < FS_ROWS) {
+                    const int oy = 4 * py0 - 5 + r;
+                    const int* yr = ytab + r * FS_TAB;
+                    const int ym = yr[0];
+                    Acc3 a;
+#pragma unroll
+                    for (int t = 0; t < KSY; ++t) {
+                        const int rr = min(ym + t, nrows - 1);
+                        tap(a, hres[rr * SP_PATCH_COLS + hc], (uint32_t)yr[1 + t]);
+                    }
+                    half4 o = normalise(lut, a);
+                    if ((unsigned)oy >= 640u || (unsigned)ox >= 640u) o = half4{0, 0, 0, 0};
+                    *(half4*)(patch + (r * SP_PATCH_COLS + hc) * 8) = o;
+                }
+            }
+        }
+        sp_lds_barrier();
+
+        const Fetched f = fetch(k + 1 < nt ? tile + stride : tile);
+        int lane_k = lane;
+        asm volatile("" : "+v"(lane_k));
+        sp_tile_math<0>(p, wreg, a_off, patch, ctile, bias_lds, img, py0, px0, wv, lane_k, [&] { stage(f); });
+        nrows = f.nrows;
+        sp_lds_barrier();
     }
 }
 
@@ -224,6 +406,8 @@
                 }
             }
 }
+
+extern "C" int vtd_stem_pool_grid(int total_tiles) { return total_tiles < 512 ? total_tiles : 512; }
 
 int vtd_launch_stem_pool(const TensorDesc& in, const TensorDesc& out, const half_t* w_packed, const float* bias, int n,
                          hipStream_t stream) {
@@ -238,7 +422,7 @@
     p.tiles_x = out.w / SP_PT_COLS;
     p.tiles_y = (out.h + SP_PT_ROWS - 1) / SP_PT_ROWS;
     p.total_tiles = n * p.tiles_x * p.tiles_y;
-    const int grid = p.total_tiles < 512 ? p.total_tiles : 512;
+    const int grid = vtd_stem_pool_grid(p.total_tiles);
     void (*kern)(const StemPoolParams) = stem_pool_kernel<0>;
 #ifdef VTD_STEM_EXPERIMENT
     if (const char* e = getenv("VTD_STEM_DEBUG")) {
@@ -270,3 +454,53 @@
     hipError_t e = hipGetLastError();
     return e == hipSuccess ? 0 : -(int)e;
 }
+
+void vtd_frames_stem_limits(int* out ) {
+    out[0] = FS_ROWS; out[1] = FS_QPR; out[2] = FS_MAX_RAW_ROWS; out[3] = FS_LDS; out[4] = SP_LDS; out[5] = FS_TAB;
+}
+
+void vtd_frames_stem_spans(const int* xb, const int* yb, FramesStemSpans* out) {
+    for (int ty = 0; ty < FramesStemSpans::TILES_Y; ++ty) {
+        int oy0 = 4 * SP_PT_ROWS * ty - 5, oy1 = oy0 + FS_ROWS - 1;
+        oy0 = oy0 < 0 ? 0 : oy0; oy1 = oy1 > 639 ? 639 : oy1;
+        out->y_first[ty] = yb[2 * oy0];
+        out->nrows[ty] = yb[2 * oy1] + yb[2 * oy1 + 1] - yb[2 * oy0];
+    }
+    for (int tx = 0; tx < FramesStemSpans::TILES_X; ++tx) {
+        int ox0 = 4 * SP_PT_COLS * tx - 5, ox1 = ox0 + SP_PATCH_COLS - 1;
+        ox0 = ox0 < 0 ? 0 : ox0; ox1 = ox1 > 639 ? 639 : ox1;
+        out->x_first[tx] = xb[2 * ox0] & ~3;
+        out->nquads[tx] = (xb[2 * ox1] + xb[2 * ox1 + 1] - out->x_first[tx] + 3) >> 2;
+    }
+}
+
+int vtd_launch_frames_stem_pool(const uint8_t* frames, int H, int W, const int* xtab, int ksx, const int* ytab, int ksy,
+                                const FramesStemSpans& spans, const TensorDesc& out, const half_t* w_packed, const float* bias, int n,
+                                hipStream_t stream) {
+    if (ksx != 5 || ksy != 5 || (W & 3) || !xtab || !ytab || out.c != 64 || out.h != 160 || out.w != 160 || n <= 0 || n > out.n) return -2003;
+    static_assert(FramesStemSpans::TILES_X * SP_PT_COLS == 160 && (FramesStemSpans::TILES_Y - 1) * SP_PT_ROWS < 160 && FramesStemSpans::TILES_Y * SP_PT_ROWS >= 160, "span tables are per tile row / column of the 160x160 pooled map");
+    for (int ty = 0; ty < FramesStemSpans::TILES_Y; ++ty)
+        if (spans.nrows[ty] < 1 || spans.nrows[ty] > FS_MAX_RAW_ROWS || spans.y_first[ty] < 0 || spans.y_first[ty] + spans.nrows[ty] > H) return -2004;
+    for (int tx = 0; tx < FramesStemSpans::TILES_X; ++tx)
+        if (spans.nquads[tx] < 1 || spans.nquads[tx] > FS_QPR || spans.x_first[tx] < 0 || (spans.x_first[tx] & 3) || spans.x_first[tx] + 4 * spans.nquads[tx] > W) return -2004;
+    FramesStemParams q;
+    StemPoolParams& p = q.sp;
+    p.in = nullptr; p.w = w_packed; p.bias = bias; p.out = out.ptr;
+    p.n = n; p.in_hp = 646; p.in_wp = 646; p.conv_h = 320; p.conv_w = 320; p.pool_h = out.h; p.pool_w = out.w;
+    p.out_hp = out.hp; p.out_wp = out.wp; p.out_ring = out.ring;
+    p.tiles_x = out.w / SP_PT_COLS;
+    p.tiles_y = (out.h + SP_PT_ROWS - 1) / SP_PT_ROWS;
+    p.total_tiles = n * p.tiles_x * p.tiles_y;
+    q.frames = frames; q.xtab = xtab; q.ytab = ytab; q.H = H; q.W = W;
+    q.spans = spans;
+    const int grid = vtd_stem_pool_grid(p.total_tiles);
+    static bool attr_set = false;
+    if (!attr_set) {
+        hipError_t ea = hipFuncSetAttribute((const void*)frames_stem_pool_kernel<5, 5>, hipFuncAttributeMaxDynamicSharedMemorySize, FS_LDS);
+        if (ea != hipSuccess) return -(int)ea;
+        attr_set = true;
+    }
+    hipLaunchKernelGGL((frames_stem_pool_kernel<5, 5>), dim3(grid), dim3(256), FS_LDS, stream, q);
+    hipError_t e = hipGetLastError();
+    return e == hipSuccess ? 0 : -(int)e;
+}
diff --git a/video-text-detection-system_amd/csrc/vtd_api.cpp b/video-text-detection-system_amd/csrc/vtd_api.cpp
--- a/video-text-detection-system_amd/csrc/vtd_api.cpp
+++ b/video-text-detection-system_amd/csrc/vtd_api.cpp
@@ -16,6 +16,11 @@
 bool vtd_conv_config_valid(const ConvParams& p, int cfg);
 int vtd_launch_preprocess(const uint8_t* frames, int n, int H, int W, half_t* out, const int* xb, const int* xk, int ksx,
                           const int* yb, const int* yk, int ksy, int max_rows, hipStream_t stream);
+void vtd_frames_stem_limits(int* out);
+void vtd_frames_stem_spans(const int* xb, const int* yb, FramesStemSpans* out);
+int vtd_launch_frames_stem_pool(const uint8_t* frames, int H, int W, const int* xtab, int ksx, const int* ytab, int ksy,
+                                const FramesStemSpans& spans, const TensorDesc& out, const half_t* w_packed, const float* bias, int n,
+                                hipStream_t stream);
 int vtd_launch_nchw_to_input(const float* x, half_t* out, int n, hipStream_t stream);
 int vtd_launch_maxpool(const TensorDesc& in, const TensorDesc& out, int n, int kh, int kw, int sh, int sw, int pad_h, int pad_w,
                        hipStream_t stream);
@@ -107,6 +112,7 @@
     ERR_BATCH = -1105,
     ERR_GEOMETRY = -1106,
     ERR_CAPACITY = -1107,
+    ERR_TAP_NOT_BUILT = -1108,
 };
 
 using StateDict = std::map<std::string, std::vector<float>>;
@@ -445,7 +451,21 @@
 struct PreTables {
     int *xb = nullptr, *xk = nullptr, *yb = nullptr, *yk = nullptr;
     int ksx = 0, ksy = 0, max_rows = 0;
+    FramesStemSpans spans;
+    int *xtab = nullptr, *ytab = nullptr;
+    bool fused_stem = false;
 };
+
+static bool frames_stem_eligible(int H, int W, int ksx, int ksy, const FramesStemSpans& sp) {
+    if (H != 720 || W != 1280 || ksx != 5 || ksy != 5) return false;
+    int lim[6];
+    vtd_frames_stem_limits(lim);
+    for (int ty = 0; ty < FramesStemSpans::TILES_Y; ++ty)
+        if (sp.nrows[ty] > lim[2]) return false;
+    for (int tx = 0; tx < FramesStemSpans::TILES_X; ++tx)
+        if (sp.nquads[tx] > lim[1]) return false;
+    return lim[3] <= 80 * 1024;
+}
 
 }
 
@@ -574,6 +594,8 @@
     bool head_tail_kernel = true;
     bool fuse_stem_pool = true;
     bool fuse_fpn_head = true;
+    bool fuse_preprocess = false;
+    bool input_current = true;
     bool fuse_downsample = true;
     size_t pool_ops = 0;
     size_t trunk_ops = 0;
@@ -1316,11 +1338,27 @@
         max_rows = std::max(max_rows, ay.bounds[2 * last] + ay.bounds[2 * last + 1] - ay.bounds[2 * oy0]);
     }
     t.max_rows = max_rows;
+    vtd_frames_stem_spans(ax.bounds.data(), ay.bounds.data(), &t.spans);
+    t.fused_stem = frames_stem_eligible(H, W, t.ksx, t.ksy, t.spans);
     int rc;
     if ((rc = upload(d->arena, ax.bounds.data(), ax.bounds.size() * sizeof(int), (void**)&t.xb))) return rc;
     if ((rc = upload(d->arena, ax.kk.data(), ax.kk.size() * sizeof(int), (void**)&t.xk))) return rc;
     if ((rc = upload(d->arena, ay.bounds.data(), ay.bounds.size() * sizeof(int), (void**)&t.yb))) return rc;
     if ((rc = upload(d->arena, ay.kk.data(), ay.kk.size() * sizeof(int), (void**)&t.yk))) return rc;
+    if (t.fused_stem) {
+        int lim[6];
+        vtd_frames_stem_limits(lim);
+        const ResampleAxis* axes[2] = {&ax, &ay};
+        int** dst[2] = {&t.xtab, &t.ytab};
+        for (int a = 0; a < 2; ++a) {
+            std::vector<int> tab((size_t)640 * lim[5], 0);
+            for (int o = 0; o < 640; ++o) {
+                tab[(size_t)o * lim[5]] = axes[a]->bounds[2 * o];
+                for (int k = 0; k < axes[a]->ksize; ++k) tab[(size_t)o * lim[5] + 1 + k] = axes[a]->kk[(size_t)o * axes[a]->ksize + k];
+            }
+            if ((rc = upload(d->arena, tab.data(), tab.size() * sizeof(int), (void**)dst[a]))) return rc;
+        }
+    }
     d->pre[key] = t;
     out = t;
     return 0;
@@ -1350,6 +1388,7 @@
         case ERR_BATCH: return "batch exceeds the handle's max_batch";
         case ERR_GEOMETRY: return "layer geometry check failed";
         case ERR_CAPACITY: return "output capacity too small";
+        case ERR_TAP_NOT_BUILT: return "tap not built by the last forward (vtd_detector_forward_frames fed the stem from the raw frames)";
         case -2801: return "feature export needs a detector finalized with fuse_fpn_head=0 (the fused head entry never forms P2)";
         case -2802: return "DB head training: invalid argument or shape";
         case -2803: return "DB head training: misaligned buffer";
@@ -1568,6 +1607,7 @@
     if (std::string(name) == "fuse_stem_pool") { d->fuse_stem_pool = value != 0; return 0; }
     if (std::string(name) == "head_tail_kernel") { d->head_tail_kernel = value != 0; return 0; }
     if (std::string(name) == "fuse_downsample") { d->fuse_downsample = value != 0; return 0; }
+    if (std::string(name) == "fuse_preprocess") { d->fuse_preprocess = value != 0; return 0; }
     return ERR_UNKNOWN_KEY;
 }
 
@@ -1590,6 +1630,7 @@
     PreTables t;
     int rc = get_pre_tables(d, height, width, t);
     if (rc) return rc;
+    d->input_current = true;
     return vtd_launch_preprocess(frames_dev, n, height, width, d->input.ptr, t.xb, t.xk, t.ksx, t.yb, t.yk, t.ksy, t.max_rows,
                                  (hipStream_t)stream);
 }
@@ -1598,10 +1639,17 @@
     if (!d || !x_dev) return ERR_ARG;
     if (!d->finalized) return ERR_NOT_FINALIZED;
     if (n <= 0 || n > d->max_batch) return ERR_BATCH;
+    d->input_current = true;
     return vtd_launch_nchw_to_input(x_dev, d->input.ptr, n, (hipStream_t)stream);
 }
 
-static int run_detector_ops(vtd_detector* d, int n, float* prob_dev, float* thresh_dev, hipStream_t s, size_t op_end) {
+struct RawFrames {
+    const uint8_t* dev;
+    int H, W;
+    PreTables t;
+};
+
+static int run_detector_ops(vtd_detector* d, int n, float* prob_dev, float* thresh_dev, hipStream_t s, size_t op_end, const RawFrames* raw = nullptr) {
     float* outs[2] = {prob_dev, thresh_dev};
     const int bucket = batch_bucket(n, d->max_batch);
     auto tit = d->tuned.find(bucket);
@@ -1637,7 +1685,11 @@
                 rc = vtd_launch_head_tail(o.conv.in, o.htw1, o.conv.bias, o.htw2, o.conv.head_b, outs[o.final_slot], n, s);
                 break;
             case Op::BORDER: rc = launch_border_tiles(o.conv, n, s); break;
-            case Op::STEMPOOL: rc = vtd_launch_stem_pool(o.pin, o.pout, o.spw, o.spb, n, s); break;
+            case Op::STEMPOOL:
+                rc = raw ? vtd_launch_frames_stem_pool(raw->dev, raw->H, raw->W, raw->t.xtab, raw->t.ksx, raw->t.ytab, raw->t.ksy, raw->t.spans,
+                                                       o.pout, o.spw, o.spb, n, s)
+                         : vtd_launch_stem_pool(o.pin, o.pout, o.spw, o.spb, n, s);
+                break;
         }
         if (rc) return rc;
         if (prof) {
@@ -1654,6 +1706,46 @@
     if (!d->finalized) return ERR_NOT_FINALIZED;
     if (n <= 0 || n > d->max_batch) return ERR_BATCH;
     return run_detector_ops(d, n, prob_dev, thresh_dev, (hipStream_t)stream, d->ops.size());
+}
+
+int vtd_detector_forward_frames(vtd_detector* d, const uint8_t* frames_dev, int n, int height, int width, float* prob_dev, float* thresh_dev,
+                                vtd_stream stream) {
+    if (!d || !frames_dev || !prob_dev || height <= 0 || width <= 0) return ERR_ARG;
+    if (!d->finalized) return ERR_NOT_FINALIZED;
+    if (n <= 0 || n > d->max_batch) return ERR_BATCH;
+    RawFrames raw{frames_dev, height, width, {}};
+    int rc = get_pre_tables(d, height, width, raw.t);
+    if (rc) return rc;
+    const bool stem_first = !d->ops.empty() && d->ops[0].kind == Op::STEMPOOL;
+    if (!d->fuse_preprocess || !stem_first || !raw.t.fused_stem) {
+        if ((rc = vtd_detector_preprocess(d, frames_dev, n, height, width, stream))) return rc;
+        return vtd_detector_forward(d, n, prob_dev, thresh_dev, stream);
+    }
+    d->input_current = false;
+    return run_detector_ops(d, n, prob_dev, thresh_dev, (hipStream_t)stream, d->ops.size(), &raw);
+}
+
+int vtd_frames_stem_plan(int height, int width, int* tiles, int* xb, int* xk, int* yb, int* yk, int* info) {
+    if (height <= 0 || width <= 0 || !tiles || !xb || !xk || !yb || !yk || !info) return ERR_ARG;
+    const ResampleAxis ax = pillow_axis(width, 640), ay = pillow_axis(height, 640);
+    if (ax.ksize > 16 || ay.ksize > 16) return ERR_CAPACITY;
+    std::copy(ax.bounds.begin(), ax.bounds.end(), xb);
+    std::copy(ax.kk.begin(), ax.kk.end(), xk);
+    std::copy(ay.bounds.begin(), ay.bounds.end(), yb);
+    std::copy(ay.kk.begin(), ay.kk.end(), yk);
+    FramesStemSpans sp;
+    vtd_frames_stem_spans(ax.bounds.data(), ay.bounds.data(), &sp);
+    for (int ty = 0; ty < FramesStemSpans::TILES_Y; ++ty)
+        for (int tx = 0; tx < FramesStemSpans::TILES_X; ++tx) {
+            int* t = tiles + (ty * FramesStemSpans::TILES_X + tx) * 4;
+            t[0] = sp.y_first[ty]; t[1] = sp.nrows[ty]; t[2] = sp.x_first[tx]; t[3] = sp.nquads[tx];
+        }
+    int lim[6];
+    vtd_frames_stem_limits(lim);
+    const bool fused = frames_stem_eligible(height, width, ax.ksize, ay.ksize, sp);
+    info[0] = ax.ksize; info[1] = ay.ksize; info[2] = fused ? 1 : 0; info[3] = fused ? lim[3] : lim[4];
+    info[4] = FramesStemSpans::TILES_X; info[5] = FramesStemSpans::TILES_Y; info[6] = lim[2]; info[7] = lim[1];
+    return 0;
 }
 
 int vtd_detector_forward_features(vtd_detector* d, int n, void* feats_dev, vtd_stream stream) {
@@ -1802,6 +1894,7 @@
     if (it == d->taps.end()) return ERR_UNKNOWN_KEY;
     const TensorDesc& t = it->second;
     if (n <= 0 || n > t.n) return ERR_BATCH;
+    if (std::string(name) == "input" && !d->input_current) return ERR_TAP_NOT_BUILT;
     const int creal = (std::string(name) == "input") ? 3 : t.c;
     if (capacity < (int64_t)n * creal * t.h * t.w) return ERR_CAPACITY;
     return read_tensor_nchw(t, n, creal, host_out, (hipStream_t)stream);
diff --git a/video-text-detection-system_amd/csrc/vtd_common.h b/video-text-detection-system_amd/csrc/vtd_common.h
--- a/video-text-detection-system_amd/csrc/vtd_common.h
+++ b/video-text-detection-system_amd/csrc/vtd_common.h
@@ -79,6 +79,11 @@
     float* prob_out;
 };
 
+struct FramesStemSpans {
+    static constexpr int TILES_Y = 23, TILES_X = 20;
+    int y_first[TILES_Y], nrows[TILES_Y], x_first[TILES_X], nquads[TILES_X];
+};
+
 #define VTD_HIP_CHECK(expr)                                   \
     do {                                                      \
         hipError_t _e = (expr);                               \
diff --git a/video-text-detection-system_amd/vtd_amd/_native.py b/video-text-detection-system_amd/vtd_amd/_native.py
--- a/video-text-detection-system_amd/vtd_amd/_native.py
+++ b/video-text-detection-system_amd/vtd_amd/_native.py
@@ -65,6 +65,7 @@
     "vtd_detector_preprocess": (C.c_int, [C.c_void_p, C.c_void_p, C.c_int, C.c_int, C.c_int, C.c_void_p]),
     "vtd_detector_set_input_nchw": (C.c_int, [C.c_void_p, C.c_void_p, C.c_int, C.c_void_p]),
     "vtd_detector_forward": (C.c_int, [C.c_void_p, C.c_int, C.c_void_p, C.c_void_p, C.c_void_p]),
+    "vtd_detector_forward_frames": (C.c_int, [C.c_void_p, C.c_void_p, C.c_int, C.c_int, C.c_int, C.c_void_p, C.c_void_p, C.c_void_p]),
     "vtd_detector_read_tap": (C.c_int, [C.c_void_p, C.c_char_p, C.c_int, C.c_void_p, C.c_int64, C.c_void_p]),
     "vtd_detector_macs_per_frame": (C.c_int64, [C.c_void_p]),
     "vtd_detector_set_profiling": (C.c_int, [C.c_void_p, C.c_int]),
diff --git a/video-text-detection-system_amd/vtd_amd/engine.py b/video-text-detection-system_amd/vtd_amd/engine.py
--- a/video-text-detection-system_amd/vtd_amd/engine.py
+++ b/video-text-detection-system_amd/vtd_amd/engine.py
@@ -184,12 +184,17 @@
 
     def forward(self, x, want_threshold=False):
         with self.lock:
-            n, keep = self._set_input(x)
+            raw = isinstance(x, DeviceFrames)
+            n, keep = (x.n, x) if raw else self._set_input(x)
             prob = torch.empty((n, 1, 640, 640), dtype=torch.float32, device="cuda")
             thr = torch.empty_like(prob) if want_threshold else None
-            _native.check(self.lib.vtd_detector_forward(self.handle, n, C.c_void_p(prob.data_ptr()),
-                                                        C.c_void_p(thr.data_ptr()) if thr is not None else None, _stream_ptr()),
-                          "vtd_detector_forward")
+            outs = (C.c_void_p(prob.data_ptr()), C.c_void_p(thr.data_ptr()) if thr is not None else None, _stream_ptr())
+            if raw:
+                x.wait_ready()
+                _native.check(self.lib.vtd_detector_forward_frames(self.handle, C.c_void_p(x.tensor.data_ptr()), n, x.height, x.width, *outs),
+                              "vtd_detector_forward_frames")
+            else:
+                _native.check(self.lib.vtd_detector_forward(self.handle, n, *outs), "vtd_detector_forward")
             del keep
             return {"probability": prob, "threshold": thr}
 
```

Result: no change. 12600, median of 4 (+0.7%).
